# hello-robot/stretch_mujoco

Measured on AMD Instinct MI355X. Metric: env-steps/sec (whole node), 4096 parallel Stretch envs in total, higher is better.
Workload: dtype f32

## Files before the change

### stretch_mujoco_amd/csrc/smj_kernels.hip

```cpp
#define SMJ_BUILD_TAG step
#include "smj_step_tu.h"

__global__ __launch_bounds__(256) void smj_reset_kernel(const DevModel M, const DevState S, const uint8_t* mask) {
  const int e = blockIdx.x * blockDim.x + threadIdx.x;
  if (e >= S.B) return;
  if (mask && !mask[e]) return;
  for (int k = 0; k < M.nq_all; k++) S.qpos[k * S.ld + e] = M.qpos0[k];
  for (int k = 0; k < M.nv_all; k++) { S.qvel[k * S.ld + e] = 0.f; S.warm[k * S.ld + e] = 0.f; }
  for (int k = 0; k < M.nu; k++) S.ctrl[k * S.ld + e] = 0.f;
  if (S.bctl)
    for (int k = 0; k < SMJ_BC_ROWS; k++) S.bctl[k * S.ld + e] = 0.f;
  S.nstep[e] = 0;
  for (int k = 0; k < 4; k++) S.info[k * S.ld + e] = 0;
  if (S.pgsprev) S.pgsprev[(size_t)e * SMJ_PGSPREV_STRIDE] = 0.f;
  if (S.mcache)
    for (int k = 0; k < SMJ_MC_SLOTS; k++) S.mcache[((size_t)e * SMJ_MC_SLOTS + k) * SMJ_MC_WORDS] = 0.f;
  if (S.sepcache)
    for (int k = 0; k < SMJ_SEP_SLOTS; k++) S.sepcache[((size_t)e * SMJ_SEP_SLOTS + k) * 4 + 3] = 0.f;
}

__global__ __launch_bounds__(256) void smj_stage_kernel(const StagePlan P, float* stage, int stride, int B, long ld, int is_export) {
  __shared__ float tile[128][65];
  const int t = threadIdx.x, w = t >> 6, l = t & 63, env0 = blockIdx.x * 64, sg = blockIdx.y;
  float* arr = static_cast<float*>(P.seg[sg].ptr) + (long)P.row0[sg] * ld;
  const int nr = P.seg[sg].rows, off = P.seg[sg].off;
  if (!is_export) {
    for (int k = w; k < nr; k += 4) tile[k][l] = env0 + l < B ? arr[(long)k * ld + env0 + l] : 0.f;
    __syncthreads();
    for (int idx = t; idx < 64 * nr; idx += 256) {
      const int e = idx / nr, k = idx - e * nr;
      if (env0 + e < B) stage[(size_t)(env0 + e) * stride + off + k] = tile[k][e];
    }
  } else {
    for (int idx = t; idx < 64 * nr; idx += 256) {
      const int e = idx / nr, k = idx - e * nr;
      if (env0 + e < B) tile[k][e] = stage[(size_t)(env0 + e) * stride + off + k];
    }
    __syncthreads();
    for (int k = w; k < nr; k += 4)
      if (env0 + l < B) arr[(long)k * ld + env0 + l] = tile[k][l];
  }
}

__global__ __launch_bounds__(256) void smj_base_tick_kernel(const DevState S) {
  const int e = blockIdx.x * blockDim.x + threadIdx.x;
  if (e >= S.B || !S.bctl) return;
  const long ld = S.ld;
  const int mode = (int)S.bctl[SMJ_BC_MODE * ld + e];
  if (mode == 0) return;
  const float x = S.base[e], y = S.base[ld + e], th = S.base[2 * ld + e];
  const float inc = S.bctl[SMJ_BC_INC * ld + e], sign = inc > 0.f ? 1.f : -1.f;
  float v = 0.f, w = 0.f;
  int next = mode;
  if (mode == 1) {
    const float dx = x - S.bctl[SMJ_BC_X0 * ld + e], dy = y - S.bctl[SMJ_BC_Y0 * ld + e];
    if (!(sqrtf(dx * dx + dy * dy) <= fabsf(inc))) next = 0; else v = SMJ_BASE_X_VEL * sign;
  } else if (mode == 2) {
    if (!(fabsf(S.bctl[SMJ_BC_TH0 * ld + e] - th) <= fabsf(inc))) next = 0; else w = SMJ_BASE_R_VEL * sign;
  } else { v = S.bctl[SMJ_BC_V * ld + e]; w = S.bctl[SMJ_BC_W * ld + e]; }
  S.ctrl[e] = (v - (w * SMJ_WHEEL_SEPARATION / 2.f)) / SMJ_WHEEL_RADIUS;
  S.ctrl[ld + e] = (v + (w * SMJ_WHEEL_SEPARATION / 2.f)) / SMJ_WHEEL_RADIUS;
  S.bctl[SMJ_BC_MODE * ld + e] = (float)next;
}

__global__ __launch_bounds__(1024) void smj_order_kernel(const int* cost, int* order, int B) {
  __shared__ int hist[256], mx;
  const int t = threadIdx.x;
  if (t < 256) hist[t] = 0;
  if (t == 0) mx = 1;
  __syncthreads();
  int m = 1;
  for (int e = t; e < B; e += 1024) m = cost[e] > m ? cost[e] : m;
  atomicMax(&mx, m);
  __syncthreads();
  const float sc = 255.f / (float)mx;
  for (int e = t; e < B; e += 1024) atomicAdd(&hist[255 - (int)((float)(cost[e] > 0 ? cost[e] : 0) * sc)], 1);
  __syncthreads();
  if (t == 0) {
    int acc = 0;
    for (int k = 0; k < 256; k++) { const int n = hist[k]; hist[k] = acc; acc += n; }
  }
  __syncthreads();
  for (int e = t; e < B; e += 1024) order[atomicAdd(&hist[255 - (int)((float)(cost[e] > 0 ? cost[e] : 0) * sc)], 1)] = e;
}
void smj_launch_order(const int* cost, int* order, int B, hipStream_t stream) {
  hipLaunchKernelGGL(smj_order_kernel, dim3(1), dim3(1024), 0, stream, cost, order, B);
}
void smj_launch_stage(const StagePlan& plan, float* stage, int stride, int B, long ld, bool is_export, hipStream_t stream) {
  if (plan.nseg == 0) return;
  hipLaunchKernelGGL(smj_stage_kernel, dim3((B + 63) / 64, plan.nseg), dim3(256), 0, stream, plan, stage, stride, B, ld, is_export ? 1 : 0);
}
void smj_launch_base_tick(const DevState& s, hipStream_t stream) {
  hipLaunchKernelGGL(smj_base_tick_kernel, dim3((s.B + 255) / 256), dim3(256), 0, stream, s);
}
void smj_launch_reset(const DevModel& m, const DevState& s, const uint8_t* mask, hipStream_t stream) {
  hipLaunchKernelGGL(smj_reset_kernel, dim3((s.B + 255) / 256), dim3(256), 0, stream, m, s, mask);
}
```

### stretch_mujoco_amd/csrc/smj_kernels_mid.hip

```cpp
#define SMJ_BUILD_TAG mid
#include "smj_step_tu.h"
```

### stretch_mujoco_amd/csrc/smj_step_impl.h

```cpp
#pragma once
#ifndef SMJ_PROFILING
#define SMJ_PROFILING 1
#endif
#include <cstddef>
#include "smj_model.h"
#include "smj_wave.h"
#include "smj_sat_mem.h"

#define JS (NVS + 1)
#define MS (NVS + 1)
#define SMJ_MINVAL 1e-15f
#define SMJ_MINIMP 0.0001f
#define SMJ_MAXIMP 0.9999f

enum { JT_FREE = 0, JT_BALL = 1, JT_SLIDE = 2, JT_HINGE = 3 };
enum { GT_PLANE = 0, GT_SPHERE = 2, GT_CAPSULE = 3, GT_ELLIPSOID = 4, GT_CYLINDER = 5, GT_BOX = 6, GT_MESH = 7 };
enum { CT_EQUALITY = 0, CT_FRICTION = 1, CT_LIMIT = 3, CT_CONTACT_FRICTIONLESS = 5, CT_CONTACT_ELLIPTIC = 7, CT_NONE = -1 };

#if NSAT > 0
#define NCGS (NCG + 1)
#define NSURV 128
#else
#define NCGS NCG
#endif
// ... 149 lines not shown
#endif

template <int N>
SMJ_DEV int qcqp(float* res, const float* Ain, const float* bin, const float* dd, float r, float& la_io, bool exact, float* iters = nullptr) {
  float A[N * N], b[N], L[N * N], Li[N], la = exact ? 0.f : la_io;
#pragma unroll
  for (int i = 0; i < N; i++) {
    b[i] = bin[i] * dd[i];
#pragma unroll
    for (int j = 0; j <= i; j++) A[i * N + j] = Ain[i * N + j] * dd[i] * dd[j];
  }
  float dmin = A[0];
#pragma unroll
  for (int i = 1; i < N; i++) dmin = fminf(dmin, A[i * N + i]);
  const float r2 = r * r, vtol = exact ? 1e-10f : 1e-10f + 1e-5f * r2, dtol = exact ? 1e-10f : 1e-10f + 1e-5f * dmin, drel = exact ? 0.f : 1e-5f;
  for (int it = 0; it < 20; it++) {
    if (iters) *iters += 1.f;
    bool bad = false;
#pragma unroll
    for (int j = 0; j < N; j++) {
      float sd = A[j * N + j] + la;
#pragma unroll
      for (int k = 0; k < j; k++) sd -= L[j * N + k] * L[j * N + k];
      if (sd < 1e-10f) { bad = true; sd = 1e-10f; }
      const float li = fast_rsqrt(sd);
      Li[j] = li;
#pragma unroll
      for (int i = j + 1; i < N; i++) {
        float t = A[i * N + j];
#pragma unroll
        for (int k = 0; k < j; k++) t -= L[i * N + k] * L[j * N + k];
        L[i * N + j] = t * li;
      }
    }
    if (bad) {
#pragma unroll
      for (int i = 0; i < N; i++) res[i] = 0;
      return 0;
    }
    float x[N], nn = 0;
#pragma unroll
    for (int i = 0; i < N; i++) {
      float sv = -b[i];
#pragma unroll
      for (int k = 0; k < i; k++) sv -= L[i * N + k] * x[k];
      x[i] = sv * Li[i];
    }
#pragma unroll
    for (int i = N - 1; i >= 0; i--) {
      float sv = x[i];
#pragma unroll
      for (int k = i + 1; k < N; k++) sv -= L[k * N + i] * x[k];
      x[i] = sv * Li[i];
    }
#pragma unroll
    for (int i = 0; i < N; i++) { res[i] = x[i]; nn += x[i] * x[i]; }
    const float val = nn - r2;
    if (val < vtol && (exact || la == 0.f || val > -vtol)) break;
    float q = 0;
#pragma unroll
    for (int i = 0; i < N; i++) {
      float sv = res[i];
#pragma unroll
      for (int k = 0; k < i; k++) sv -= L[i * N + k] * x[k];
      x[i] = sv * Li[i];
      q += x[i] * x[i];
    }
    float delta;
    if (exact) {
      delta = val * fast_rcp(2.f * q);
      if (delta < dtol) break;
    } else {
      const float nrm = nn * fast_rsqrt(nn);
      delta = (nrm - r) * nn * fast_rcp(r * q);
      if (fabsf(delta) < dtol + drel * la) break;
      if (fabsf(delta) < 3e-3f * (la + dmin)) {
        const float lan = fmaxf(0.f, la + delta), d = lan - la;
#pragma unroll
        for (int i = N - 1; i >= 0; i--) {
          float sv = x[i];
#pragma unroll
          for (int k = i + 1; k < N; k++) sv -= L[k * N + i] * x[k];
          x[i] = sv * Li[i];
        }
#pragma unroll
        for (int i = 0; i < N; i++) res[i] -= d * x[i];
        la = lan;
        break;
      }
    }
    la = fmaxf(0.f, la + delta);
  }
#pragma unroll
  for (int i = 0; i < N; i++) res[i] *= dd[i];
  la_io = la;
  return la != 0;
}

SMJ_DEV float impedance(const float* solimp, float pos, float margin) {
  float dmin = fminf(SMJ_MAXIMP, fmaxf(SMJ_MINIMP, solimp[0])), dmax = fminf(SMJ_MAXIMP, fmaxf(SMJ_MINIMP, solimp[1]));
  float width = fmaxf(SMJ_MINVAL, solimp[2]), mid = fminf(SMJ_MAXIMP, fmaxf(SMJ_MINIMP, solimp[3])), power = fmaxf(1.0f, solimp[4]);
  if (dmin == dmax) return 0.5f * (dmin + dmax);
  float x = fabsf(pos - margin) / width, y;
  if (x >= 1) return dmax;
  if (x <= 0) return dmin;
  if (power == 1.0f) y = x;
  else if (power == 2.0f) y = (x <= mid) ? x * x / mid : 1 - (1 - x) * (1 - x) / (1 - mid);
  else if (x <= mid) y = powf(x, power) / powf(mid, power - 1);
  else y = 1 - powf(1 - x, power) / powf(1 - mid, power - 1);
  return dmin + y * (dmax - dmin);
}

#ifdef SMJ_EMUL
static long smj_emul_sep_skips = 0;
static long smj_emul_ext_steps = 0;
static long smj_emul_mc_hits = 0;
static long smj_emul_isl_total = 0, smj_emul_isl_swept = 0;
#endif
struct StepKernel {
  const DevModel& M;
  const DevState& S;
  Smem& s;
  int env;

  PL<float[6]> cdof, cdof_dot;
  PL<float> qvel_r, g_r, qacc_r;
  PL<float> f_r[NPS], r_r[NPS], ARinv_r[NPS];
  PL<float> qla_r;
  int nefc, ncon, niter, flags;
  float* ppc = nullptr;
  int step_base = 0;
  int pipe_chunk = 0;
  bool parked = false;
  bool split_on = false, rev = false;
  bool serial_redo = false;

  SMJ_DEV StepKernel(const DevModel& M_, const DevState& S_, Smem& s_, int env_) : M(M_), S(S_), s(s_), env(env_) {}

  SMJ_DEV static uint64_t mk64(int lo, int hi) { return (uint64_t)(uint32_t)lo | ((uint64_t)(uint32_t)hi << 32); }

  struct KinTab {
    PL<int> parent, level;
    PL<int[6]> jump;
    PL<float[3]> pos;
    PL<float[4]> quat;
    PL<int[2]> jtype, jqadr, jdadr;
    PL<float[2]> jq0;
    PL<float[6]> jaxis, jpos;
  };
  SMJ_DEV const int* lanerec(int ol, int off) const {
    return static_cast<const int*>(__builtin_assume_aligned(M.k_lanerec + ol * SMJ_LR_STRIDE + off, 16));
  }
  SMJ_DEV static float asf(int b) { return __builtin_bit_cast(float, b); }
  SMJ_DEV void load(KinTab& t) {
    LANES {
      const int* r = lanerec(opaque(lane), SMJ_LR_KIN);
      int v[35];
      for (int k = 0; k < 35; k++) v[k] = r[k];
      t.parent[lane] = v[0]; t.level[lane] = v[1];
      for (int q = 0; q < 6; q++) t.jump[lane][q] = v[2 + q];
      for (int k = 0; k < 3; k++) t.pos[lane][k] = asf(v[8 + k]);
      for (int k = 0; k < 4; k++) t.quat[lane][k] = asf(v[11 + k]);
      for (int u = 0; u < 2; u++) {
        t.jtype[lane][u] = v[15 + u]; t.jqadr[lane][u] = v[17 + u]; t.jdadr[lane][u] = v[19 + u]; t.jq0[lane][u] = asf(v[21 + u]);
      }
      for (int k = 0; k < 6; k++) { t.jaxis[lane][k] = asf(v[23 + k]); t.jpos[lane][k] = asf(v[29 + k]); }
    }
  }
  struct BodyTab {
    PL<int> root, subsize, parent, dofadr, dofnum;
    PL<int[6]> jump;
    PL<uint64_t> dofmask;
    PL<float[10]> inl;
  };
  SMJ_DEV void load(BodyTab& t) {
    LANES {
      const int* r = lanerec(opaque(lane), SMJ_LR_BODY);
      int v[23];
      for (int k = 0; k < 23; k++) v[k] = r[k];
      t.root[lane] = v[0]; t.subsize[lane] = v[1]; t.parent[lane] = v[2]; t.dofadr[lane] = v[3]; t.dofnum[lane] = v[4];
      for (int q = 0; q < 6; q++) t.jump[lane][q] = v[5 + q];
      t.dofmask[lane] = mk64(v[11], v[12]);
      for (int k = 0; k < 10; k++) t.inl[lane][k] = asf(v[13 + k]);
    }
  }
  struct DofTab {
    PL<int> body, jtype, qadr, first, bsub;
    PL<uint64_t> velmask;
    PL<float> damp, stiff, spring;
    PL<int[2]> act;
    PL<float[2]> actmom;
  };
  SMJ_DEV void load(DofTab& t) {
    LANES {
      const int* r = lanerec(opaque(lane), SMJ_LR_DOF);
      int v[14];
      for (int k = 0; k < 14; k++) v[k] = r[k];
      t.body[lane] = v[0]; t.jtype[lane] = v[1]; t.qadr[lane] = v[2]; t.first[lane] = v[3]; t.bsub[lane] = v[4];
      t.velmask[lane] = mk64(v[5], v[6]);
      t.damp[lane] = asf(v[7]); t.stiff[lane] = asf(v[8]); t.spring[lane] = asf(v[9]);
      for (int u = 0; u < 2; u++) { t.act[lane][u] = v[10 + u]; t.actmom[lane][u] = asf(v[12 + u]); }
    }
  }
  struct EntryTab {
    PL<int[NENT]> i, j, lact;
    PL<float[NENT]> arm, damp, dcoef, lcoef;
  };
  SMJ_DEV void load(EntryTab& t, bool implicit) {
    LANES {
      const int* r = lanerec(opaque(lane), SMJ_LR_ENT);
      for (int u = 0; u < NENT; u++) { t.i[lane][u] = r[u]; t.j[lane][u] = r[NENT + u]; t.arm[lane][u] = asf(r[2 * NENT + u]); }
      if (implicit)
        for (int u = 0; u < NENT; u++) {
          t.lact[lane][u] = r[3 * NENT + u]; t.damp[lane][u] = asf(r[4 * NENT + u]); t.dcoef[lane][u] = asf(r[5 * NENT + u]);
          t.lcoef[lane][u] = asf(r[6 * NENT + u]);
        }
    }
  }
  struct ActTab {
    PL<int[4]> dof, qadr;
    PL<float[4]> mom;
    PL<float[8]> prm;
    PL<int> flags;
    PL<int> gc_body, gc_mlo, gc_mhi;
    PL<float> gc_mass, gc_x, gc_y, gc_z;
  };
  SMJ_DEV void load(ActTab& t) {
    LANES {
      const int* r = lanerec(opaque(lane), SMJ_LR_ACT);
      int v[28];
      for (int k = 0; k < 28; k++) v[k] = r[k];
      for (int u = 0; u < 4; u++) { t.dof[lane][u] = v[u]; t.qadr[lane][u] = v[4 + u]; t.mom[lane][u] = asf(v[8 + u]); }
      for (int k = 0; k < 8; k++) t.prm[lane][k] = asf(v[12 + k]);
      t.flags[lane] = v[20]; t.gc_body[lane] = v[21]; t.gc_mlo[lane] = v[22]; t.gc_mhi[lane] = v[23];
      t.gc_mass[lane] = asf(v[24]); t.gc_x[lane] = asf(v[25]); t.gc_y[lane] = asf(v[26]); t.gc_z[lane] = asf(v[27]);
    }
  }

  SMJ_DEV void setup() {
    LANES {
      for (int k = lane; k < NVS * MS; k += 64) (&s.MM[0][0])[k] = 0.f;
      if (lane == 0) {
        s.xpos[0][0] = s.xpos[0][1] = s.xpos[0][2] = 0;
        s.xquat[0][0] = 1; s.xquat[0][1] = s.xquat[0][2] = s.xquat[0][3] = 0;
        for (int k = 0; k < 9; k++) s.xmat[0][k] = (k % 4 == 0) ? 1.f : 0.f;
      }
    }
    SYNC();
#if NSAT > 0
    LANES {
      for (int k = lane; k < (NDR + 1) * JS; k += 64) (&s.J[0][0])[k] = 0.f;
      if (lane == 0) { s.sat.cand_ok = 0; s.sat.ncand = 0; }
      for (int k = lane; k < NCG * 3; k += 64) (&s.sat.refcen[0][0])[k] = 0.f;
    }
#endif
    LANES { if (lane >= M.nv && lane < NVS) s.MM[lane][lane] = 1.f; }
    SYNC();
  }

  SMJ_DEV float* stage_row() const { return S.stage + (size_t)env * S.lay.stride; }
  SMJ_DEV void escalate(int st) {
#ifndef SMJ_EMUL
    float* row = stage_row();
    int* rowi = reinterpret_cast<int*>(row);
    LANES {
      for (int k = lane; k < M.nq; k += 64) st_coh(&row[S.lay.qpos + k], s.qpos[k]);
      if (lane < M.nv) { st_coh(&row[S.lay.qvel + lane], s.qvel[lane]); st_coh(&row[S.lay.warm + lane], s.warm[lane]); }
      if (lane < M.nu) st_coh(&row[S.lay.ctrl + lane], s.ctrl[lane]);
      if (lane < SMJ_BC_ROWS) st_coh(&row[S.lay.bctl + lane], s.bctl[lane]);
      if (lane == 0) {
        st_coh(&rowi[S.lay.nstep], ld_coh(&rowi[S.lay.nstep]) + st);
        st_coh(&S.done_steps[env], ld_coh(&S.done_steps[env]) + st);
      }
    }
#if NSAT > 0
    sat_store_state();
#endif
    coh_release();
    LANES {
      if (lane == 0) {
        st_coh(&S.progress[env], -(pipe_chunk + 1));
        asm volatile("s_waitcnt vmcnt(0)" ::: "memory");
        const int at = atomicAdd(&S.sched[SMJ_SCHED_COUNT], 1);
        st_coh(&S.redo[at], env);
      }
    }
#endif
    parked = true;
  }
  SMJ_DEV void load_state() {
    const long ld = S.ld;
    if (staged()) {
      const float* st = stage_row();
      LANES {
        for (int k = lane; k < M.nq; k += 64) s.qpos[k] = ld_coh(&st[S.lay.qpos + k]);
        if (lane < M.nv) { s.qvel[lane] = ld_coh(&st[S.lay.qvel + lane]); s.warm[lane] = ld_coh(&st[S.lay.warm + lane]); }
        if (lane < M.nu) s.ctrl[lane] = ld_coh(&st[S.lay.ctrl + lane]);
        if (lane < SMJ_BC_ROWS) s.bctl[lane] = ld_coh(&st[S.lay.bctl + lane]);
      }
    } else {
      LANES {
        for (int k = lane; k < M.nq; k += 64) s.qpos[k] = S.qpos[k * ld + env];
        if (lane < M.nv) { s.qvel[lane] = S.qvel[lane * ld + env]; s.warm[lane] = S.warm[lane * ld + env]; }
        if (lane < M.nu) s.ctrl[lane] = S.ctrl[lane * ld + env];
        if (lane < SMJ_BC_ROWS) s.bctl[lane] = S.bctl ? S.bctl[lane * ld + env] : 0.f;
      }
    }
    SYNC();
#if NSAT > 0
    sat_load_state();
#endif
  }
  SMJ_DEV void store_state(int nsteps) {
    const long ld = S.ld;
#if NSAT > 0
    sat_store_state();
#endif
    const int b = 1;
    const float bx = s.xpos[b][0], by = s.xpos[b][1], bth = atan2f(s.xmat[b][3], s.xmat[b][0]);
    if (staged()) {
      float* st = stage_row();
      int* sti = reinterpret_cast<int*>(st);
      LANES {
        for (int k = lane; k < M.nq; k += 64) st_coh(&st[S.lay.qpos + k], s.qpos[k]);
        if (lane < M.nv) { st_coh(&st[S.lay.qvel + lane], s.qvel[lane]); st_coh(&st[S.lay.warm + lane], s.warm[lane]); }
        if (lane < M.nu) { st_coh(&st[S.lay.ctrl + lane], s.ctrl[lane]); st_coh(&st[S.lay.actlen + lane], s.act_len[lane]); st_coh(&st[S.lay.actvel + lane], s.act_vel[lane]); }
        if (lane < SMJ_BC_ROWS) st_coh(&st[S.lay.bctl + lane], s.bctl[lane]);
        if (lane == 0) {
          st_coh(&sti[S.lay.nstep], ld_coh(&sti[S.lay.nstep]) + nsteps);
          if (S.done_steps) st_coh(&S.done_steps[env], ld_coh(&S.done_steps[env]) + nsteps);
          st_coh(&sti[S.lay.info + SMJ_INFO_NEFC], nefc); st_coh(&sti[S.lay.info + SMJ_INFO_NCON], ncon);
          st_coh(&sti[S.lay.info + SMJ_INFO_NITER], niter); st_coh(&sti[S.lay.info + SMJ_INFO_FLAGS], ld_coh(&sti[S.lay.info + SMJ_INFO_FLAGS]) | flags);
          st_coh(&st[S.lay.base], bx); st_coh(&st[S.lay.base + 1], by); st_coh(&st[S.lay.base + 2], bth);
        }
      }
    } else {
      LANES {
        for (int k = lane; k < M.nq; k += 64) S.qpos[k * ld + env] = s.qpos[k];
        if (lane < M.nv) { S.qvel[lane * ld + env] = s.qvel[lane]; S.warm[lane * ld + env] = s.warm[lane]; }
        if (lane < M.nu) { S.ctrl[lane * ld + env] = s.ctrl[lane]; S.act_len[lane * ld + env] = s.act_len[lane]; S.act_vel[lane * ld + env] = s.act_vel[lane]; }
        if (lane < SMJ_BC_ROWS && S.bctl) S.bctl[lane * ld + env] = s.bctl[lane];
        if (lane == 0) {
          S.nstep[env] += nsteps;
          S.info[SMJ_INFO_NEFC * ld + env] = nefc; S.info[SMJ_INFO_NCON * ld + env] = ncon;
          S.info[SMJ_INFO_NITER * ld + env] = niter; S.info[SMJ_INFO_FLAGS * ld + env] |= flags;
          S.base[0 * ld + env] = bx; S.base[1 * ld + env] = by; S.base[2 * ld + env] = bth;
        }
      }
    }
  }

  SMJ_DEV void base_controller() {
    const int mode = (int)uni(s.bctl[SMJ_BC_MODE]);
    if (mode == 0) return;
    const int b = 1;
    const float x = uni(s.xpos[b][0]), y = uni(s.xpos[b][1]), th = atan2f(uni(s.xmat[b][3]), uni(s.xmat[b][0]));
    const float inc = uni(s.bctl[SMJ_BC_INC]), sign = inc > 0.f ? 1.f : -1.f;
    float v = 0.f, w = 0.f;
    int next = mode;
    if (mode == 1) {
      const float dx = x - uni(s.bctl[SMJ_BC_X0]), dy = y - uni(s.bctl[SMJ_BC_Y0]);
      if (!(sqrtf(dx * dx + dy * dy) <= fabsf(inc))) next = 0; else v = SMJ_BASE_X_VEL * sign;
    } else if (mode == 2) {
      if (!(fabsf(uni(s.bctl[SMJ_BC_TH0]) - th) <= fabsf(inc))) next = 0; else w = SMJ_BASE_R_VEL * sign;
    } else { v = uni(s.bctl[SMJ_BC_V]); w = uni(s.bctl[SMJ_BC_W]); }
    const float wl = (v - (w * SMJ_WHEEL_SEPARATION / 2.f)) / SMJ_WHEEL_RADIUS, wr = (v + (w * SMJ_WHEEL_SEPARATION / 2.f)) / SMJ_WHEEL_RADIUS;
    LANES {
      if (lane == 0) { s.ctrl[0] = wl; s.ctrl[1] = wr; s.bctl[SMJ_BC_MODE] = (float)next; }
    }
    SYNC();
  }

  SMJ_DEV void kinematics() {
    const int nb = M.nbody;
    KinTab kt;
    load(kt);
    PL<float[3]> pl;
    PL<float[4]> ql;
    PL<float[6]> al, xl;
    LANES {
      float pos[3] = {0, 0, 0}, quat[4] = {1, 0, 0, 0};
      for (int k = 0; k < 6; k++) { al[lane][k] = 0.f; xl[lane][k] = 0.f; }
      if (lane > 0 && lane < nb) {
        if (kt.jtype[lane][0] == JT_FREE) {
          const int qa = kt.jqadr[lane][0];
          for (int k = 0; k < 3; k++) pos[k] = s.qpos[qa + k];
          for (int k = 0; k < 4; k++) quat[k] = s.qpos[qa + 3 + k];
        } else {
          for (int k = 0; k < 3; k++) pos[k] = kt.pos[lane][k];
          for (int k = 0; k < 4; k++) quat[k] = kt.quat[lane][k];
#pragma unroll
          for (int t = 0; t < 2; t++) {
            const int jt = kt.jtype[lane][t];
            if (jt < 0) continue;
            const float* ax = &kt.jaxis[lane][3 * t];
            const float* jp = &kt.jpos[lane][3 * t];
            float Rm[9], xa[3], a[3], anchor[3];
            quat2mat(Rm, quat);
            mulmat3vec(xa, Rm, ax);
            mulmat3vec(a, Rm, jp);
            for (int k = 0; k < 3; k++) { anchor[k] = pos[k] + a[k]; xl[lane][3 * t + k] = xa[k]; al[lane][3 * t + k] = anchor[k]; }
            const float q = s.qpos[kt.jqadr[lane][t]] - kt.jq0[lane][t];
            if (jt == JT_SLIDE) {
              for (int k = 0; k < 3; k++) pos[k] += xa[k] * q;
            } else {
              float sn, cs;
              sincosf(0.5f * q, &sn, &cs);
              const float dq[4] = {cs, ax[0] * sn, ax[1] * sn, ax[2] * sn};
              quat_mul(quat, quat, dq);
              quat2mat(Rm, quat);
              mulmat3vec(a, Rm, jp);
              for (int k = 0; k < 3; k++) pos[k] = anchor[k] - a[k];
            }
          }
        }
        quat_normalize(quat);
      }
      const bool mine = lane < NBP && (!SMJ_W2_FORWARD || lane < nb);
      for (int k = 0; k < 3; k++) { pl[lane][k] = pos[k]; if (mine) s.xpos[lane][k] = pos[k]; }
      for (int k = 0; k < 4; k++) { ql[lane][k] = quat[k]; if (mine) s.xquat[lane][k] = quat[k]; }
    }
    SYNC();
#pragma unroll
    for (int r = 0; r < 6; r++) {
      if (r >= M.njump) break;
      PL<float[3]> pa;
      PL<float[4]> qa;
      PL<int> anc;
      LANES {
        const int a = kt.jump[lane][r];
        anc[lane] = a;
        for (int k = 0; k < 3; k++) pa[lane][k] = s.xpos[a][k];
        for (int k = 0; k < 4; k++) qa[lane][k] = s.xquat[a][k];
      }
      SYNC();
      LANES {
        if (anc[lane] > 0) {
          float Rm[9], v[3], q[4];
          quat2mat(Rm, qa[lane]);
          mulmat3vec(v, Rm, pl[lane]);
          quat_mul(q, qa[lane], ql[lane]);
          for (int k = 0; k < 3; k++) { pl[lane][k] = pa[lane][k] + v[k]; s.xpos[lane][k] = pl[lane][k]; }
          for (int k = 0; k < 4; k++) { ql[lane][k] = q[k]; s.xquat[lane][k] = q[k]; }
        }
      }
      SYNC();
    }
    LANES {
      if (lane < nb) {
        float q[4] = {ql[lane][0], ql[lane][1], ql[lane][2], ql[lane][3]}, Rm[9];
        quat_normalize(q);
        quat2mat(Rm, q);
        for (int k = 0; k < 4; k++) s.xquat[lane][k] = q[k];
        for (int k = 0; k < 9; k++) s.xmat[lane][k] = Rm[k];
      }
    }
    SYNC();
    LANES {
      if (lane > 0 && lane < nb) {
        if (kt.jtype[lane][0] == JT_FREE) {
          const int da = kt.jdadr[lane][0];
          for (int d = 0; d < 6; d++)
            for (int k = 0; k < 3; k++) s.xanchor[da + d][k] = s.xpos[lane][k];
          for (int d = 0; d < 3; d++)
            for (int k = 0; k < 3; k++) {
              s.xaxis[da + d][k] = (d == k) ? 1.f : 0.f;
              s.xaxis[da + 3 + d][k] = s.xmat[lane][3 * k + d];
            }
        } else {
          const int p = kt.parent[lane];
#pragma unroll
          for (int t = 0; t < 2; t++) {
            if (kt.jtype[lane][t] < 0) continue;
            const int da = kt.jdadr[lane][t];
            float xa[3], an[3];
            mulmat3vec(xa, s.xmat[p], &xl[lane][3 * t]);
            mulmat3vec(an, s.xmat[p], &al[lane][3 * t]);
            for (int k = 0; k < 3; k++) { s.xaxis[da][k] = xa[k]; s.xanchor[da][k] = s.xpos[p][k] + an[k]; }
          }
        }
      }
    }
    SYNC();
  }

  SMJ_DEV void com_crb() {
    const int nb = M.nbody, nv = M.nv;
    BodyTab bt;
    DofTab dt;
    EntryTab et;
    load(bt); load(dt); load(et, false);
    PL<float> mx, my, mz;
    PL<float[3]> xip;
    LANES {
      const int b = lane;
      float t[3] = {0, 0, 0};
      if (b > 0 && b < nb) {
        mulmat3vec(t, s.xmat[b], &bt.inl[lane][6]);
        for (int k = 0; k < 3; k++) t[k] += s.xpos[b][k];
      }
      for (int k = 0; k < 3; k++) xip[lane][k] = t[k];
    }
    for (int r = 0; r < nroot(); r++) {
      const int root = uni(M.k_root_list[r]);
      LANES {
        const bool in = lane > 0 && lane < nb && bt.root[lane] == root;
        const float m = in ? bt.inl[lane][9] : 0.f;
        mx[lane] = m * xip[lane][0]; my[lane] = m * xip[lane][1]; mz[lane] = m * xip[lane][2];
      }
      const float inv = 1.0f / M.body_subtreemass[root];
      const float cx = wave_sum(mx) * inv, cy = wave_sum(my) * inv, cz = wave_sum(mz) * inv;
      LANES {
        if (lane < nb && bt.root[lane] == root) { s.com[lane][0] = cx; s.com[lane][1] = cy; s.com[lane][2] = cz; }
      }
    }
    SYNC();
    LANES {
      const int b = lane;
      if (b > 0 && b < nb) {
        const float* R = s.xmat[b];
        const float* I = bt.inl[lane];
        float Il[9] = {I[0], I[3], I[4], I[3], I[1], I[5], I[4], I[5], I[2]}, RI[9], T[9], Rt[9];
        mulmat3(RI, R, Il);
        for (int i = 0; i < 3; i++)
          for (int j = 0; j < 3; j++) Rt[3 * i + j] = R[3 * j + i];
        mulmat3(T, RI, Rt);
        float dif[3] = {xip[lane][0] - s.com[b][0], xip[lane][1] - s.com[b][1], xip[lane][2] - s.com[b][2]};
        const float mass = I[9], dd = dot3(dif, dif);
        float* c = s.u.t.cinert[b];
        c[0] = T[0] + mass * (dd - dif[0] * dif[0]); c[1] = T[4] + mass * (dd - dif[1] * dif[1]);
        c[2] = T[8] + mass * (dd - dif[2] * dif[2]); c[3] = T[1] - mass * dif[0] * dif[1];
        c[4] = T[2] - mass * dif[0] * dif[2]; c[5] = T[5] - mass * dif[1] * dif[2];
        c[6] = mass * dif[0]; c[7] = mass * dif[1]; c[8] = mass * dif[2]; c[9] = mass;
      }
      if (lane < nv) {
        const int d = lane, b = dt.body[lane];
        float off[3] = {s.com[b][0] - s.xanchor[d][0], s.com[b][1] - s.xanchor[d][1], s.com[b][2] - s.xanchor[d][2]};
        float* c = cdof[lane];
        const int jt = dt.jtype[lane], k = d - dt.first[lane];
        if (jt == JT_SLIDE || (jt == JT_FREE && k < 3)) {
          c[0] = c[1] = c[2] = 0;
          for (int x = 0; x < 3; x++) c[3 + x] = s.xaxis[d][x];
        } else {
          for (int x = 0; x < 3; x++) c[x] = s.xaxis[d][x];
          cross3(c + 3, s.xaxis[d], off);
        }
        for (int x = 0; x < 6; x++) s.u.t.cdof[d][x] = c[x];
        qvel_r[lane] = s.qvel[d];
      } else {
        for (int x = 0; x < 6; x++) cdof[lane][x] = 0;
        qvel_r[lane] = 0;
      }
    }
    SYNC();
    LANES {
      if (lane < nv)
        for (int x = 0; x < 6; x++) s.u.t.buf[lane][x] = cdof[lane][x] * qvel_r[lane];
    }
    SYNC();
    PL<float[6]> cvb;
    LANES {
      float sv[6] = {0, 0, 0, 0, 0, 0};
      if (lane > 0 && lane < nb) {
        const int da = bt.dofadr[lane], dn = bt.dofnum[lane];
#pragma unroll
        for (int u = 0; u < 6; u++) {
          const float on = u < dn ? 1.f : 0.f;
          const int a = da + (u < dn ? u : 0);
          for (int x = 0; x < 6; x++) sv[x] += on * s.u.t.buf[dn > 0 ? a : 0][x];
        }
      }
      for (int x = 0; x < 6; x++) { cvb[lane][x] = sv[x]; if (lane < NBP) s.u.t.cvel[lane][x] = sv[x]; }
    }
    SYNC();
#pragma unroll
    for (int r = 0; r < 6; r++) {
      if (r >= M.njump) break;
      PL<float[6]> up;
      PL<int> anc;
      LANES {
        const int a = bt.jump[lane][r];
        anc[lane] = a;
        for (int x = 0; x < 6; x++) up[lane][x] = s.u.t.cvel[a][x];
      }
      SYNC();
      LANES {
        if (anc[lane] > 0)
          for (int x = 0; x < 6; x++) { cvb[lane][x] += up[lane][x]; s.u.t.cvel[lane][x] = cvb[lane][x]; }
      }
      SYNC();
    }
    LANES {
      if (lane < nv) {
        const int b = dt.body[lane], pb = M.body_parentid[b], da = M.body_dofadr[b];
        float cv[6];
        for (int x = 0; x < 6; x++) cv[x] = s.u.t.cvel[pb][x];
        const uint64_t mk = dt.velmask[lane];
#pragma unroll
        for (int u = 0; u < 5; u++) {
          const int a = da + u;
          const float on = (a < lane && ((mk >> a) & 1)) ? 1.f : 0.f;
          for (int x = 0; x < 6; x++) cv[x] += on * s.u.t.buf[a < lane ? a : lane][x];
        }
        const int jt = dt.jtype[lane], k = lane - dt.first[lane];
        if (jt == JT_FREE && k < 3) { for (int x = 0; x < 6; x++) cdof_dot[lane][x] = 0; }
        else cross_motion(cdof_dot[lane], cv, cdof[lane]);
        for (int x = 0; x < 6; x++) s.u.t.cdof_dot[lane][x] = cdof_dot[lane][x];
      } else {
        for (int x = 0; x < 6; x++) cdof_dot[lane][x] = 0;
      }
    }
    {
      PL<float[10]> cr;
      LANES { for (int k = 0; k < 10; k++) cr[lane][k] = 0.f; }
      for (int x0 = 0; x0 < M.maxsubtree; x0 += 4) {
        LANES {
          if (lane > 0 && lane < nb) {
            const int sub = bt.subsize[lane];
#pragma unroll
            for (int u = 0; u < 4; u++) {
              const bool in = x0 + u < sub;
              const int x = lane + (in ? x0 + u : 0);
              const float on = in ? 1.f : 0.f;
              for (int k = 0; k < 10; k++) cr[lane][k] += on * s.u.t.cinert[x][k];
            }
          }
        }
      }
      LANES {
        if (lane < nb)
          for (int k = 0; k < 10; k++) s.u.t.crb[lane][k] = cr[lane][k];
      }
    }
    SYNC();
    LANES {
      if (lane < nv) {
        float bf[6];
        mul_inert_vec(bf, s.u.t.crb[dt.body[lane]], cdof[lane]);
        for (int x = 0; x < 6; x++) s.u.t.buf[lane][x] = bf[x];
      }
    }
    SYNC();
    LANES {
      for (int t = 0; t < NENT; t++) {
        const int i = et.i[lane][t], j = et.j[lane][t];
        if (i < 0) continue;
        float v = 0;
        for (int x = 0; x < 6; x++) v += s.u.t.cdof[j][x] * s.u.t.buf[i][x];
        if (i == j) { v += et.arm[lane][t]; s.Mdiag[i] = v; }
        s.MM[i][j] = v;
        if (i != j) s.MM[j][i] = v;
      }
    }
    SYNC();
  }

  SMJ_DEV void factor() {
    const int nv = M.nv;
    EntryTab et;
    load(et, false);
    for (int k = nv - 1; k >= 0; k--) {
      const float dkk = s.MM[k][k], dinv = 1.0f / dkk;
      LANES {
        for (int t = 0; t < NENT; t++) {
          const int i = et.i[lane][t], j = et.j[lane][t];
          if (i < 0 || i >= k) continue;
          const float a = s.MM[k][i];
          if (a != 0.f) s.MM[i][j] -= a * s.MM[k][j] * dinv;
        }
      }
      SYNC();
      LANES {
        if (lane < k) s.MM[k][lane] *= dinv;
        if (lane == k) s.Dinv[k] = dinv;
      }
      SYNC();
    }
  }
  SMJ_DEV void solve_LT(PL<float>& x) {
    for (int i = M.nv - 1; i > 0; i--) {
      const float xi = wave_read(x, i);
      LANES { if (lane < i) x[lane] -= s.MM[i][lane] * xi; }
    }
  }
  SMJ_DEV void solve_L(PL<float>& x) {
    for (int j = 0; j < M.nv - 1; j++) {
      const float xj = wave_read(x, j);
      LANES { if (lane > j && lane < M.nv) x[lane] -= s.MM[lane][j] * xj; }
    }
  }

  SMJ_DEV void smooth_forces(bool dbg) {
    const int nb = M.nbody, nv = M.nv, nu = M.nu;
    PL<float> frc_passive, frc_bias, frc_act;
    DofTab dt;
    ActTab at;
    load(dt); load(at);
    LANES {
      float f = 0;
      if (lane < nv) {
        f = -dt.damp[lane] * s.qvel[lane];
        if (dt.stiff[lane] != 0.f) f -= dt.stiff[lane] * (s.qpos[dt.qadr[lane]] - dt.spring[lane]);
      }
      frc_passive[lane] = f;
    }
    BodyTab bt;
    load(bt);
    LANES {
      if (lane < 16) {
        float off[3] = {0, 0, 0}, F[3] = {0, 0, 0};
        int mlo = 0, mhi = 0;
        if (lane < M.ngc) {
          const int b = at.gc_body[lane];
          const float gm = at.gc_mass[lane];
          const float lp[3] = {at.gc_x[lane], at.gc_y[lane], at.gc_z[lane]};
          float pt[3];
          mulmat3vec(pt, s.xmat[b], lp);
          for (int k = 0; k < 3; k++) { off[k] = pt[k] + s.xpos[b][k] - s.com[b][k]; F[k] = -M.gravity[k] * gm; }
          mlo = at.gc_mlo[lane]; mhi = at.gc_mhi[lane];
        }
        float* o = s.u.t.buf[lane];
        for (int k = 0; k < 3; k++) { o[k] = off[k]; o[3 + k] = F[k]; }
        s.u.t.cfrc[lane][0] = __builtin_bit_cast(float, mlo); s.u.t.cfrc[lane][1] = __builtin_bit_cast(float, mhi);
      }
    }
    SYNC();
    LANES {
      if (lane < nv) {
        float acc = 0;
#pragma unroll
        for (int t = 0; t < 16; t++) {
          const uint64_t mk = mk64(__builtin_bit_cast(int, s.u.t.cfrc[t][0]), __builtin_bit_cast(int, s.u.t.cfrc[t][1]));
          const float* o = s.u.t.buf[t];
          float tv[3];
          cross3(tv, cdof[lane], o);
          const float v = (cdof[lane][3] + tv[0]) * o[3] + (cdof[lane][4] + tv[1]) * o[4] + (cdof[lane][5] + tv[2]) * o[5];
          acc += ((mk >> lane) & 1) ? v : 0.f;
        }
        frc_passive[lane] += acc;
      }
    }
    SYNC();
    LANES {
      if (lane < nv)
        for (int x = 0; x < 6; x++) s.u.t.buf[lane][x] = s.u.t.cdof_dot[lane][x] * s.qvel[lane];
    }
    SYNC();
    PL<float[6]> ca;
    LANES {
      float sv[6] = {0, 0, 0, 0, 0, 0};
      if (lane > 0 && lane < nb) {
        const int da = bt.dofadr[lane], dn = bt.dofnum[lane];
#pragma unroll
        for (int u = 0; u < 6; u++) {
          const float on = u < dn ? 1.f : 0.f;
          const int a = dn > 0 ? da + (u < dn ? u : 0) : 0;
          for (int x = 0; x < 6; x++) sv[x] += on * s.u.t.buf[a][x];
        }
      }
      for (int x = 0; x < 6; x++) { ca[lane][x] = sv[x]; if (lane < NBP) s.u.t.cfrc[lane][x] = sv[x]; }
    }
    SYNC();
#pragma unroll
    for (int r = 0; r < 6; r++) {
      if (r >= M.njump) break;
      PL<float[6]> up;
      PL<int> anc;
      LANES {
        const int a = bt.jump[lane][r];
        anc[lane] = a;
        for (int x = 0; x < 6; x++) up[lane][x] = s.u.t.cfrc[a][x];
      }
      SYNC();
      LANES {
        if (anc[lane] > 0)
          for (int x = 0; x < 6; x++) { ca[lane][x] += up[lane][x]; s.u.t.cfrc[lane][x] = ca[lane][x]; }
      }
      SYNC();
    }
    LANES {
      if (lane < nb) {
        const int b = lane;
        float t1[6] = {0, 0, 0, 0, 0, 0}, cf[6] = {0, 0, 0, 0, 0, 0};
        if (b > 0) {
          const float a[6] = {ca[lane][0], ca[lane][1], ca[lane][2], ca[lane][3] - M.gravity[0], ca[lane][4] - M.gravity[1], ca[lane][5] - M.gravity[2]};
          float t2[6];
          mul_inert_vec(t1, s.u.t.cinert[b], a);
          mul_inert_vec(t2, s.u.t.cinert[b], s.u.t.cvel[b]);
          cross_force(cf, s.u.t.cvel[b], t2);
        }
        for (int x = 0; x < 6; x++) s.u.t.cfrc[b][x] = t1[x] + cf[x];
      }
    }
    SYNC();
    {
      PL<float[6]> cfs;
      LANES { for (int k = 0; k < 6; k++) cfs[lane][k] = 0.f; }
      for (int x0 = 0; x0 < M.maxsubtree; x0 += 4) {
        LANES {
          if (lane < nv) {
            const int b = dt.body[lane], sub = dt.bsub[lane];
#pragma unroll
            for (int u = 0; u < 4; u++) {
              const bool in = x0 + u < sub;
              const int x = b + (in ? x0 + u : 0);
              const float on = in ? 1.f : 0.f;
              for (int k = 0; k < 6; k++) cfs[lane][k] += on * s.u.t.cfrc[x][k];
            }
          }
        }
      }
      LANES {
        float v = 0;
        if (lane < nv)
          for (int k = 0; k < 6; k++) v += cdof[lane][k] * cfs[lane][k];
        frc_bias[lane] = v;
      }
    }
    LANES {
      if (lane < nu) {
        const int a = lane;
        float len = 0, vel = 0;
#pragma unroll
        for (int t = 0; t < 4; t++) {
          const int dd = at.dof[lane][t];
          if (dd >= 0) { vel += at.mom[lane][t] * s.qvel[dd]; len += at.mom[lane][t] * s.qpos[at.qadr[lane][t]]; }
        }
        const float* pr = at.prm[lane];
        const int fl = at.flags[lane];
        float ctrl = s.ctrl[a];
        if (fl & 1) ctrl = fminf(pr[5], fmaxf(pr[4], ctrl));
        float f = pr[0] * ctrl;
        if (fl & 4) f += pr[1] + pr[2] * len + pr[3] * vel;
        bool clamped = false;
        if (fl & 2) { clamped = (f <= pr[6] || f >= pr[7]); f = fminf(pr[7], fmaxf(pr[6], f)); }
        s.act_force[a] = f; s.act_len[a] = len; s.act_vel[a] = vel;
        s.act_free[a] = clamped ? 0.f : 1.f;
      }
    }
    SYNC();
    LANES {
      float v = 0;
      if (lane < nv) {
#pragma unroll
        for (int t = 0; t < 2; t++) {
          const int a = dt.act[lane][t];
          if (a >= 0) v += dt.actmom[lane][t] * s.act_force[a];
        }
      }
      frc_act[lane] = v;
      g_r[lane] = frc_passive[lane] - frc_bias[lane] + frc_act[lane];
      if (lane < nv) s.g[lane] = g_r[lane];
      if (dbg && debug_bound() && lane < nv) {
        S.debug[(SMJ_DBG_QFRC_BIAS + lane) * S.ld + env] = frc_bias[lane];
        S.debug[(SMJ_DBG_QFRC_PASSIVE + lane) * S.ld + env] = frc_passive[lane];
        S.debug[(SMJ_DBG_QFRC_ACT + lane) * S.ld + env] = frc_act[lane];
        S.debug[(SMJ_DBG_G + lane) * S.ld + env] = g_r[lane];
      }
    }
    SYNC();
  }

  SMJ_DEV void geom_pose(int g, float* pos, float* mat) const {
    const int b = M.geom_bodyid[g];
    float lp[3] = {M.geom_pos[3 * g], M.geom_pos[3 * g + 1], M.geom_pos[3 * g + 2]};
    mulmat3vec(pos, s.xmat[b], lp);
    for (int k = 0; k < 3; k++) pos[k] += s.xpos[b][k];
    float lm[9];
    for (int k = 0; k < 9; k++) lm[k] = M.k_geom_mat[9 * g + k];
    mulmat3(mat, s.xmat[b], lm);
  }
  SMJ_DEV void pose_from(int b, const float* lp, const float* lm, float* pos, float* mat) const {
    mulmat3vec(pos, s.xmat[b], lp);
    for (int k = 0; k < 3; k++) pos[k] += s.xpos[b][k];
    mulmat3(mat, s.xmat[b], lm);
  }
  SMJ_DEV static void make_frame(float* fr) {
    normalize3(fr);
    if (fr[1] > -0.5f && fr[1] < 0.5f) { fr[3] = 0; fr[4] = 1; fr[5] = 0; } else { fr[3] = 0; fr[4] = 0; fr[5] = 1; }
    const float t = dot3(fr, fr + 3);
    for (int k = 0; k < 3; k++) fr[3 + k] -= t * fr[k];
    normalize3(fr + 3);
    cross3(fr + 6, fr, fr + 3);
  }
  SMJ_DEV int cslot(int c) const { return (SMJ_SPLIT_COLLIDE && rev) ? NCON - 1 - c : c; }
  SMJ_DEV float (*mcs())[3] {
#if SMJ_SPLIT_COLLIDE
    return rev ? s.u.c.mc2 : s.u.c.mc;
#else
    return s.u.c.mc;
#endif
  }
  SMJ_DEV bool con_claim(int n) {
#if SMJ_SPLIT_COLLIDE
    if (split_on) {
      if (ncon + n > NCON) return false;
      int old = 0;
      LANES { if (lane == 0) old = lds_atomic_add(&s.u.c.contotal, n); }
      return uni(old) + n <= NCON;
    }
#endif
    return ncon + n <= NCON;
  }
  SMJ_DEV void write_contact(int c_, const int* r, float dist, const float* pos, const float* n) {
    const int c = cslot(c_);
    s.cdist[c] = dist;
    float fr[9] = {n[0], n[1], n[2], 0, 0, 0, 0, 0, 0};
    make_frame(fr);
    for (int k = 0; k < 9; k++) s.cframe[c][k] = fr[k];
    for (int k = 0; k < 3; k++) s.cpos[c][k] = pos[k];
    for (int k = 0; k < 5; k++) { s.cfric[c][k] = asf(r[SMJ_CP_FRIC + k]); s.csolimp[c][k] = asf(r[SMJ_CP_SOLIMP + k]); }
    s.csolref[c][0] = asf(r[SMJ_CP_SOLREF]); s.csolref[c][1] = asf(r[SMJ_CP_SOLREF + 1]);
    s.cmargin[c] = asf(r[SMJ_CP_MG]);
    s.cdim[c] = r[SMJ_CP_CONDIM]; s.cgeom1[c] = r[SMJ_CP_G1]; s.cgeom2[c] = r[SMJ_CP_G2]; s.cefc[c] = -1;
#if NSAT > 0
    s.cpair[c] = r[SMJ_CP_PAIR];
#endif
  }
  SMJ_DEV void add_contact(const int* r, float dist, const float* pos, const float* n) {
    if (!con_claim(1)) { flags |= SMJ_FLAG_CON_OVERFLOW | 0x4000; return; }
    const int c = ncon++;
    LANES { if (lane == 0) write_contact(c, r, dist, pos, n); }
  }

  SMJ_DEV void collision() {
    ncon = 0;
    for (int base = 0; base < M.nplanepair; base += 64) {
      PL<int> hull, cv;
      LANES {
        int cnt = 0, hl = 0;
        const int t = base + lane;
        if (t < M.nplanepair) {
          const int* r = static_cast<const int*>(__builtin_assume_aligned(M.k_pprec + opaque(t) * SMJ_PP_STRIDE, 16));
          int v[SMJ_PP_CONDIM];
          for (int k = 0; k < SMJ_PP_CONDIM; k++) v[k] = r[k];
          const int b1 = v[SMJ_PP_B1], b2 = v[SMJ_PP_B2];
          float lp1[3], lm1[9], pp[3], pm[9];
          for (int k = 0; k < 3; k++) lp1[k] = asf(v[SMJ_PP_POS1 + k]);
          for (int k = 0; k < 9; k++) lm1[k] = asf(v[SMJ_PP_MAT1 + k]);
          pose_from(b1, lp1, lm1, pp, pm);
          float c2[3], lc[3] = {asf(v[SMJ_PP_BCEN2]), asf(v[SMJ_PP_BCEN2 + 1]), asf(v[SMJ_PP_BCEN2 + 2])};
          mulmat3vec(c2, s.xmat[b2], lc);
          const float n[3] = {pm[2], pm[5], pm[8]};
          const float dif[3] = {c2[0] + s.xpos[b2][0] - pp[0], c2[1] + s.xpos[b2][1] - pp[1], c2[2] + s.xpos[b2][2] - pp[2]};
          const float margin = asf(v[SMJ_PP_MARGIN]);
          if (dot3(dif, n) - asf(v[SMJ_PP_RBOUND2]) <= margin) {
            const int t2 = v[SMJ_PP_T2];
            if (t2 == GT_MESH) {
              float lp2[3], lm2[9], gp[3], gm[9], bc[3], wc[3];
              for (int k = 0; k < 3; k++) { lp2[k] = asf(v[SMJ_PP_POS2 + k]); bc[k] = asf(r[SMJ_PP_BOX2 + k]); }
              for (int k = 0; k < 9; k++) lm2[k] = asf(v[SMJ_PP_MAT2 + k]);
              pose_from(b2, lp2, lm2, gp, gm);
              mulmat3vec(wc, gm, bc);
              float low = (gp[0] + wc[0] - pp[0]) * n[0] + (gp[1] + wc[1] - pp[1]) * n[1] + (gp[2] + wc[2] - pp[2]) * n[2];
              for (int k = 0; k < 3; k++) low -= fabsf(n[0] * gm[k] + n[1] * gm[3 + k] + n[2] * gm[6 + k]) * (asf(r[SMJ_PP_BOX2 + 3 + k]) + 1e-5f);
              hl = low <= margin + 1e-6f;
            } else {
              float lp2[3], lm2[9], size[3];
              for (int k = 0; k < 3; k++) { lp2[k] = asf(v[SMJ_PP_POS2 + k]); size[k] = asf(v[SMJ_PP_SIZE2 + k]); }
              for (int k = 0; k < 9; k++) lm2[k] = asf(v[SMJ_PP_MAT2 + k]);
              cnt = plane_prim(b2, lp2, lm2, size, t2, pp, n, margin, s.u.p.dist[lane], s.u.p.pos[lane]);
            }
            for (int k = 0; k < 3; k++) s.u.p.nrm[lane][k] = n[k];
            s.u.p.pair[lane] = t;
          }
        }
        s.u.p.cnt[lane] = cnt;
        hull[lane] = hl;
      }
      uint64_t hm = wave_ballot(hull);
      if (hm) {
        SYNC();
        while (hm) {
          const int l = ffs64(hm);
          hm &= hm - 1;
          narrow_plane_hull(uni(M.k_planepair[base + l]), l);
        }
        SYNC();
      }
      PL<int> bit;
      LANES { cv[lane] = s.u.p.cnt[lane]; bit[lane] = cv[lane] & 1; }
      const uint64_t m0 = wave_ballot(bit);
      LANES { bit[lane] = cv[lane] & 2; }
      const uint64_t m1 = wave_ballot(bit);
      LANES { bit[lane] = cv[lane] & 4; }
      const uint64_t m2 = wave_ballot(bit);
      const int total = popc64(m0) + 2 * popc64(m1) + 4 * popc64(m2);
      if (total) {
        LANES {
          const int c = cv[lane];
          if (c) {
            const uint64_t lt = (1ull << lane) - 1;
            const int off = ncon + popc64(m0 & lt) + 2 * popc64(m1 & lt) + 4 * popc64(m2 & lt);
            const int* r = static_cast<const int*>(__builtin_assume_aligned(M.k_pprec + s.u.p.pair[lane] * SMJ_PP_STRIDE, 16));
            const int g1 = r[SMJ_PP_G1], g2 = r[SMJ_PP_G2];
            float fr[9] = {s.u.p.nrm[lane][0], s.u.p.nrm[lane][1], s.u.p.nrm[lane][2], 0, 0, 0, 0, 0, 0};
            make_frame(fr);
            float fric[5], simp[5];
            for (int k = 0; k < 5; k++) { fric[k] = asf(r[SMJ_PP_FRIC + k]); simp[k] = asf(r[SMJ_PP_SOLIMP + k]); }
            const float sr0 = asf(r[SMJ_PP_SOLREF]), sr1 = asf(r[SMJ_PP_SOLREF + 1]), mg = asf(r[SMJ_PP_MG]);
            const int cd = r[SMJ_PP_CONDIM];
#pragma unroll
            for (int k = 0; k < 4; k++) {
              const int ci = off + k;
              if (k < c && ci < NCON) {
                s.cdist[ci] = s.u.p.dist[lane][k];
                for (int x = 0; x < 9; x++) s.cframe[ci][x] = fr[x];
                for (int x = 0; x < 3; x++) s.cpos[ci][x] = s.u.p.pos[lane][k][x];
                for (int x = 0; x < 5; x++) { s.cfric[ci][x] = fric[x]; s.csolimp[ci][x] = simp[x]; }
                s.csolref[ci][0] = sr0; s.csolref[ci][1] = sr1;
                s.cmargin[ci] = mg;
                s.cdim[ci] = cd; s.cgeom1[ci] = g1; s.cgeom2[ci] = g2; s.cefc[ci] = -1;
#if NSAT > 0
                s.cpair[ci] = r[SMJ_PP_PAIR];
#endif
              }
            }
          }
        }
        if (ncon + total > NCON) { flags |= SMJ_FLAG_CON_OVERFLOW; ncon = NCON; }
        else ncon += total;
      }
    }
    SYNC();
  }

  SMJ_DEV int plane_prim(int b2, const float* lp2, const float* lm2, const float* size, int t2, const float* pp, const float* n,
                         float margin, float* cdist, float (*cpos)[3]) const {
    float gp[3], gm[9];
    pose_from(b2, lp2, lm2, gp, gm);
    int cnt = 0;
#define put(d, q) do { cdist[cnt] = (d); cpos[cnt][0] = (q)[0]; cpos[cnt][1] = (q)[1]; cpos[cnt][2] = (q)[2]; cnt++; } while (0)
    if (t2 == GT_SPHERE) {
      const float dif[3] = {gp[0] - pp[0], gp[1] - pp[1], gp[2] - pp[2]};
      const float dist = dot3(dif, n) - size[0];
      if (dist <= margin) {
        float pos[3];
        for (int k = 0; k < 3; k++) pos[k] = gp[k] - n[k] * (size[0] + 0.5f * dist);
        put(dist, pos);
      }
    } else if (t2 == GT_CYLINDER) {
      float axis[3] = {gm[2], gm[5], gm[8]};
      float prjaxis = dot3(n, axis);
      if (prjaxis > 0) { for (int k = 0; k < 3; k++) axis[k] = -axis[k]; prjaxis = -prjaxis; }
      float vec[3] = {gp[0] - pp[0], gp[1] - pp[1], gp[2] - pp[2]};
      const float dist0 = dot3(vec, n);
      for (int k = 0; k < 3; k++) vec[k] = axis[k] * prjaxis - n[k];
      const float len2 = dot3(vec, vec);
      if (len2 >= 1e-9f) { const float sc = size[0] / sqrtf(len2); for (int k = 0; k < 3; k++) vec[k] *= sc; }
      else { vec[0] = gm[0] * size[0]; vec[1] = gm[3] * size[0]; vec[2] = gm[6] * size[0]; }
      const float prjvec = dot3(vec, n);
      for (int k = 0; k < 3; k++) axis[k] *= size[1];
      prjaxis *= size[1];
      if (dist0 + prjaxis + prjvec <= margin) {
        float pos[3], dist = dist0 + prjaxis + prjvec;
        for (int k = 0; k < 3; k++) pos[k] = gp[k] + vec[k] + axis[k] - n[k] * dist * 0.5f;
        put(dist, pos);
        if (dist0 - prjaxis + prjvec <= margin) {
          dist = dist0 - prjaxis + prjvec;
          for (int k = 0; k < 3; k++) pos[k] = gp[k] + vec[k] - axis[k] - n[k] * dist * 0.5f;
          put(dist, pos);
        }
        const float prjvec1 = -prjvec * 0.5f;
        if (dist0 + prjaxis + prjvec1 <= margin) {
          float vec1[3];
          cross3(vec1, vec, axis);
          normalize3(vec1);
          for (int k = 0; k < 3; k++) vec1[k] *= size[0] * 0.8660254037844386f;
          dist = dist0 + prjaxis + prjvec1;
          for (int sg = 0; sg < 2 && cnt < 4; sg++) {
            const float sgn = sg ? -1.f : 1.f;
            for (int k = 0; k < 3; k++) pos[k] = gp[k] + sgn * vec1[k] + axis[k] - vec[k] * 0.5f - n[k] * dist * 0.5f;
            put(dist, pos);
          }
        }
      }
    } else if (t2 == GT_CAPSULE) {
#pragma unroll
      for (int e = 0; e < 2; e++) {
        const float sg = e ? -1.f : 1.f;
        const float c[3] = {gp[0] + sg * size[1] * gm[2], gp[1] + sg * size[1] * gm[5], gp[2] + sg * size[1] * gm[8]};
        const float dif[3] = {c[0] - pp[0], c[1] - pp[1], c[2] - pp[2]};
        const float dist = dot3(dif, n) - size[0];
        if (dist <= margin) {
          float pos[3];
          for (int k = 0; k < 3; k++) pos[k] = c[k] - n[k] * (size[0] + 0.5f * dist);
          put(dist, pos);
        }
// ... 380 lines not shown
#pragma unroll
      for (int i = 0; i < 3; i++) {
        const float v1 = P[1].v[i], v2 = P[2].v[i], a1 = P[1].a[i], a2 = P[2].a[i], b1 = P[1].b[i], b2 = P[2].b[i];
        P[1].v[i] = sw ? v2 : v1; P[2].v[i] = sw ? v1 : v2;
        P[1].a[i] = sw ? a2 : a1; P[2].a[i] = sw ? a1 : a2;
        P[1].b[i] = sw ? b2 : b1; P[2].b[i] = sw ? b1 : b2;
        dir[i] = sw ? -dir[i] : dir[i];
      }
    }
    for (int it = 0;; it++) {
      if (it > 100) return false;
      mpr_support(A, Bs, dir, P[3]);
      dot = dot3(P[3].v, dir);
      if (ccd_zero(dot) || dot < 0) { SMJ_SEP_OUT() return false; }
      bool cont = false;
      cross3(va, P[1].v, P[3].v);
      dot = dot3(va, P[0].v);
      if (dot < 0 && !ccd_zero(dot)) { const MprPt q = P[3]; portal_set<2>(P, q, true); cont = true; }
      if (!cont) {
        cross3(va, P[3].v, P[2].v);
        dot = dot3(va, P[0].v);
        if (dot < 0 && !ccd_zero(dot)) { const MprPt q = P[3]; portal_set<1>(P, q, true); cont = true; }
      }
      if (!cont) break;
      for (int i = 0; i < 3; i++) { va[i] = P[1].v[i] - P[0].v[i]; vb[i] = P[2].v[i] - P[0].v[i]; }
      cross3(dir, va, vb);
      normalize3(dir);
    }
    for (int it = 0;; it++) {
      portal_dir(P, dir);
      dot = dot3(dir, P[1].v);
      if (ccd_zero(dot) || dot > 0) break;
      mpr_support(A, Bs, dir, v4);
      dot = dot3(v4.v, dir);
      if (!(ccd_zero(dot) || dot > 0)) { SMJ_SEP_OUT() return false; }
      if (reach_tolerance(P, v4, dir, tol) || it > maxit) return false;
      expand_portal(P, v4);
    }
    for (int it = 0;; it++) {
      portal_dir(P, dir);
      mpr_support(A, Bs, dir, v4);
      if (reach_tolerance(P, v4, dir, tol) || it > maxit) {
        bool inside;
        depth = sqrtf(fmaxf(0.f, origin_tri_dist2(P[1].v, P[2].v, P[3].v, pdir, &inside)));
        if (ccd_zero(pdir[0]) && ccd_zero(pdir[1]) && ccd_zero(pdir[2])) { pdir[0] = dir[0]; pdir[1] = dir[1]; pdir[2] = dir[2]; }
        normalize3(pdir);
        if (SMJ_PORTAL_NORMAL && inside && dot3(pdir, dir) > 0.9995f) {
          float ea[3], eb[3], ec[3], cr[3];
          for (int i = 0; i < 3; i++) { ea[i] = P[2].v[i] - P[1].v[i]; eb[i] = P[3].v[i] - P[1].v[i]; ec[i] = P[3].v[i] - P[2].v[i]; }
          cross3(cr, ea, eb);
          const float emax2 = fmaxf(dot3(ea, ea), fmaxf(dot3(eb, eb), dot3(ec, ec)));
          if (dot3(cr, cr) > 16.f * depth * depth * emax2) { pdir[0] = dir[0]; pdir[1] = dir[1]; pdir[2] = dir[2]; }
        }
        float b[4], vec[3], sum;
        cross3(vec, P[1].v, P[2].v); b[0] = dot3(vec, P[3].v);
        cross3(vec, P[3].v, P[2].v); b[1] = dot3(vec, P[0].v);
        cross3(vec, P[0].v, P[1].v); b[2] = dot3(vec, P[3].v);
        cross3(vec, P[2].v, P[1].v); b[3] = dot3(vec, P[0].v);
        sum = b[0] + b[1] + b[2] + b[3];
        if (ccd_zero(sum) || sum < 0) {
          b[0] = 0;
          cross3(vec, P[2].v, P[3].v); b[1] = dot3(vec, dir);
          cross3(vec, P[3].v, P[1].v); b[2] = dot3(vec, dir);
          cross3(vec, P[1].v, P[2].v); b[3] = dot3(vec, dir);
          sum = b[1] + b[2] + b[3];
        }
        if (!(fabsf(sum) > 1e-30f)) { b[0] = 0; b[1] = b[2] = b[3] = 1; sum = 3; }
#pragma unroll
        for (int i = 0; i < 3; i++) {
          const float p1 = b[0] * P[0].a[i] + b[1] * P[1].a[i] + b[2] * P[2].a[i] + b[3] * P[3].a[i];
          const float p2 = b[0] * P[0].b[i] + b[1] * P[1].b[i] + b[2] * P[2].b[i] + b[3] * P[3].b[i];
          pos[i] = 0.5f * (p1 + p2) / sum;
        }
        return true;
      }
      expand_portal(P, v4);
    }
#undef SMJ_SEP_OUT
  }

  SMJ_DEV bool sphere_box(const float* spos, float r, const Shape& bx, float margin, float& dist_out, float* dir, float* pos) {
    const float tmp[3] = {spos[0] - bx.pos[0], spos[1] - bx.pos[1], spos[2] - bx.pos[2]};
    float cen[3], cl[3], dif[3], nl[3], pl[3];
    mulmat3Tvec(cen, bx.mat, tmp);
    for (int i = 0; i < 3; i++) { cl[i] = fminf(bx.size[i], fmaxf(-bx.size[i], cen[i])); dif[i] = cl[i] - cen[i]; }
    const float dist = sqrtf(dot3(dif, dif));
    if (dist - r > margin) return false;
    if (dist <= SMJ_MINVAL) {
      float closest = 2.f * fmaxf(bx.size[0], fmaxf(bx.size[1], bx.size[2]));
      int k = 0;
      for (int i = 0; i < 6; i++) {
        const float cd = fabsf(((i & 1) ? 1.f : -1.f) * bx.size[i >> 1] - cen[i >> 1]);
        if (cd < closest) { closest = cd; k = i; }
      }
      for (int i = 0; i < 3; i++) nl[i] = (i == (k >> 1)) ? ((k & 1) ? -1.f : 1.f) : 0.f;
      for (int i = 0; i < 3; i++) pl[i] = cen[i] + nl[i] * (r - closest) * 0.5f;
      dist_out = -closest - r;
    } else {
      const float inv = 1.f / dist;
      for (int i = 0; i < 3; i++) { nl[i] = dif[i] * inv; pl[i] = 0.5f * (cl[i] + cen[i] + dif[i] * (r * inv)); }
      dist_out = dist - r;
    }
    mulmat3vec(dir, bx.mat, nl);
    mulmat3vec(pos, bx.mat, pl);
    for (int i = 0; i < 3; i++) pos[i] += bx.pos[i];
    return true;
  }
  SMJ_DEV bool sphere_sphere(const float* p1, float r1, const float* p2, float r2, float margin, float& dist_out, float* dir, float* pos) {
    float dif[3] = {p2[0] - p1[0], p2[1] - p1[1], p2[2] - p1[2]};
    const float cdist = sqrtf(dot3(dif, dif));
    if (cdist - r1 - r2 > margin) return false;
    if (cdist < SMJ_MINVAL) { dif[0] = 1; dif[1] = dif[2] = 0; } else { const float inv = 1.f / cdist; for (int i = 0; i < 3; i++) dif[i] *= inv; }
    dist_out = cdist - r1 - r2;
    for (int i = 0; i < 3; i++) { dir[i] = dif[i]; pos[i] = p1[i] + dif[i] * (r1 + 0.5f * dist_out); }
    return true;
  }
  SMJ_DEV bool sphere_capsule(const float* p1, float r1, const Shape& cp, float margin, float& dist_out, float* dir, float* pos) {
    const float ax[3] = {cp.mat[2], cp.mat[5], cp.mat[8]}, vec[3] = {p1[0] - cp.pos[0], p1[1] - cp.pos[1], p1[2] - cp.pos[2]};
    const float x = fmaxf(-cp.size[1], fminf(cp.size[1], dot3(ax, vec)));
    const float q[3] = {cp.pos[0] + ax[0] * x, cp.pos[1] + ax[1] * x, cp.pos[2] + ax[2] * x};
    return sphere_sphere(p1, r1, q, cp.size[0], margin, dist_out, dir, pos);
  }
  SMJ_DEV void capsule_capsule(const int* r, const Shape& A, const Shape& Bs, float margin) {
    const float a1[3] = {A.mat[2] * A.size[1], A.mat[5] * A.size[1], A.mat[8] * A.size[1]};
    const float a2[3] = {Bs.mat[2] * Bs.size[1], Bs.mat[5] * Bs.size[1], Bs.mat[8] * Bs.size[1]};
    const float dif[3] = {A.pos[0] - Bs.pos[0], A.pos[1] - Bs.pos[1], A.pos[2] - Bs.pos[2]};
    const float ma = dot3(a1, a1), mb = -dot3(a1, a2), mc = dot3(a2, a2), u = -dot3(a1, dif), v = dot3(a2, dif);
    float c[3], c1[3], c2[3];
    cross3(c, a1, a2); cross3(c2, a2, dif); cross3(c1, a1, dif);
    const float det = dot3(c, c);
    float v1[3], v2[3], depth, dir[3], pos[3];
    if (det >= 1e-12f * ma * mc) {
      float x1 = dot3(c, c2) / det, x2 = dot3(c, c1) / det;
      if (x1 > 1) { x1 = 1; x2 = (v - mb) / mc; }
      else if (x1 < -1) { x1 = -1; x2 = (v + mb) / mc; }
      if (x2 > 1) { x2 = 1; x1 = fmaxf(-1.f, fminf(1.f, (u - mb) / ma)); }
      else if (x2 < -1) { x2 = -1; x1 = fmaxf(-1.f, fminf(1.f, (u + mb) / ma)); }
      for (int i = 0; i < 3; i++) { v1[i] = A.pos[i] + a1[i] * x1; v2[i] = Bs.pos[i] + a2[i] * x2; }
      if (sphere_sphere(v1, A.size[0], v2, Bs.size[0], margin, depth, dir, pos)) add_contact(r, depth, pos, dir);
      return;
    }
    int n = 0;
    for (int e = 0; e < 2; e++) {
      const float sg = e ? -1.f : 1.f, x2 = fmaxf(-1.f, fminf(1.f, (v - sg * mb) / mc));
      for (int i = 0; i < 3; i++) { v1[i] = A.pos[i] + sg * a1[i]; v2[i] = Bs.pos[i] + a2[i] * x2; }
      if (sphere_sphere(v1, A.size[0], v2, Bs.size[0], margin, depth, dir, pos)) { add_contact(r, depth, pos, dir); n++; }
    }
    for (int e = 0; e < 2 && n < 2; e++) {
      const float sg = e ? -1.f : 1.f, x1 = fmaxf(-1.f, fminf(1.f, (u - sg * mb) / ma));
      for (int i = 0; i < 3; i++) { v1[i] = A.pos[i] + a1[i] * x1; v2[i] = Bs.pos[i] + sg * a2[i]; }
      if (sphere_sphere(v1, A.size[0], v2, Bs.size[0], margin, depth, dir, pos)) { add_contact(r, depth, pos, dir); n++; }
    }
  }
  SMJ_DEV void load_shape(Shape& sh, int g, int slot, float* cen) {
    (void)g;
    const unsigned meta = (unsigned)uni(s.u.c.meta[slot]);
    sh.type = (int)(meta & 15u); sh.nvert = (int)((meta >> 4) & 4095u);
    sh.verts = M.k_hull_vert4 + 4 * (int)(meta >> 16);
    for (int k = 0; k < 3; k++) { sh.pos[k] = uni(s.u.c.pos[slot][k]); sh.size[k] = uni(s.u.c.size[slot][k]); cen[k] = uni(s.u.c.ccen[slot][k]); }
    for (int k = 0; k < 9; k++) sh.mat[k] = uni(s.u.c.mat[slot][k]);
    if (sh.type == GT_MESH) {
      const Vec4* verts = reinterpret_cast<const Vec4*>(sh.verts);
      const int nvert = sh.nvert;
      LANES {
#pragma unroll
        for (int u = 0; u < 4; u++) {
          const int id = lane + 64 * u < nvert ? lane + 64 * u : (nvert > 0 ? nvert - 1 : 0);
          const Vec4 v = verts[id];
          sh.vc[lane][3 * u] = v.x; sh.vc[lane][3 * u + 1] = v.y; sh.vc[lane][3 * u + 2] = v.z;
        }
      }
    }
  }


  SMJ_DEV void ccol(float* o, int slot, int i) const {
    o[0] = uni(s.u.c.mat[slot][i]); o[1] = uni(s.u.c.mat[slot][3 + i]); o[2] = uni(s.u.c.mat[slot][6 + i]);
  }
  SMJ_DEV void box_box(const int* rec, int slot1, int slot2, float margin) {
    float p1[3], p2[3], A[3], B[3], R1[9], R2[9];
#pragma unroll
    for (int k = 0; k < 3; k++) { p1[k] = uni(s.u.c.pos[slot1][k]); p2[k] = uni(s.u.c.pos[slot2][k]); A[k] = uni(s.u.c.size[slot1][k]); B[k] = uni(s.u.c.size[slot2][k]); }
#pragma unroll
    for (int k = 0; k < 9; k++) { R1[k] = uni(s.u.c.mat[slot1][k]); R2[k] = uni(s.u.c.mat[slot2][k]); }
    const float p[3] = {p2[0] - p1[0], p2[1] - p1[1], p2[2] - p1[2]};
    float R[3][3], Q[3][3], pp[3], pq[3];
#pragma unroll
    for (int i = 0; i < 3; i++) {
      const float ai[3] = {R1[i], R1[3 + i], R1[6 + i]}, bi[3] = {R2[i], R2[3 + i], R2[6 + i]};
      pp[i] = dot3(p, ai); pq[i] = dot3(p, bi);
#pragma unroll
      for (int j = 0; j < 3; j++) { const float bj[3] = {R2[j], R2[3 + j], R2[6 + j]}; R[i][j] = dot3(ai, bj); Q[i][j] = fabsf(R[i][j]); }
    }
    float best = -3.0e38f, en[3] = {0, 0, 0};
    int code = -1;
    bool sep = false;
#pragma unroll
    for (int i = 0; i < 3; i++) {
      const float sv = fabsf(pp[i]) - (A[i] + B[0] * Q[i][0] + B[1] * Q[i][1] + B[2] * Q[i][2]);
      sep = sep || sv > margin;
      if (sv > best) { best = sv; code = i; }
    }
#pragma unroll
    for (int j = 0; j < 3; j++) {
      const float sv = fabsf(pq[j]) - (B[j] + A[0] * Q[0][j] + A[1] * Q[1][j] + A[2] * Q[2][j]);
      sep = sep || sv > margin;
      if (sv > best) { best = sv; code = 3 + j; }
    }
#pragma unroll
    for (int i = 0; i < 3; i++)
#pragma unroll
      for (int j = 0; j < 3; j++) {
        const int i1 = (i + 1) % 3, i2 = (i + 2) % 3, j1 = (j + 1) % 3, j2 = (j + 2) % 3;
        const float l = sqrtf(fmaxf(0.f, 1.f - R[i][j] * R[i][j]));
        if (l >= 2e-3f) {
          const float e = pp[i2] * R[i1][j] - pp[i1] * R[i2][j];
          const float sv = (fabsf(e) - (A[i1] * Q[i2][j] + A[i2] * Q[i1][j] + B[j1] * Q[i][j2] + B[j2] * Q[i][j1])) / l;
          sep = sep || sv > margin;
          if (sv * 1.05f > best && sv > best) {
            best = sv; code = 6 + 3 * i + j;
            const float ai[3] = {R1[i], R1[3 + i], R1[6 + i]}, bj[3] = {R2[j], R2[3 + j], R2[6 + j]};
            cross3(en, ai, bj);
            for (int k = 0; k < 3; k++) en[k] /= l;
          }
        }
      }
#ifdef SMJ_EMUL
    if (getenv("SMJ_BOXBOX_TRACE")) { fprintf(stderr, "box_box: code %d best %.9g sep %d R:", code, best, (int)sep); for (int i = 0; i < 3; i++) for (int j = 0; j < 3; j++) fprintf(stderr, " %.9g", R[i][j]); fprintf(stderr, " pp %.9g %.9g %.9g\n", pp[0], pp[1], pp[2]); }
#endif
    if (sep) return;
    if (code >= 6) {
      float n[3] = {en[0], en[1], en[2]};
      if (dot3(n, p) < 0) for (int k = 0; k < 3; k++) n[k] = -n[k];
      const int i = (code - 6) / 3, j = (code - 6) % 3;
      float pa[3] = {p1[0], p1[1], p1[2]}, pb[3] = {p2[0], p2[1], p2[2]};
#pragma unroll
      for (int k = 0; k < 3; k++) {
        const float ak[3] = {R1[k], R1[3 + k], R1[6 + k]}, bk[3] = {R2[k], R2[3 + k], R2[6 + k]};
        const float sa = dot3(n, ak) > 0 ? 1.f : -1.f, sb = dot3(n, bk) > 0 ? -1.f : 1.f;
        for (int x = 0; x < 3; x++) { pa[x] += sa * A[k] * ak[x]; pb[x] += sb * B[k] * bk[x]; }
      }
      float ua[3], ub[3];
      ccol(ua, slot1, i); ccol(ub, slot2, j);
      const float dd[3] = {pb[0] - pa[0], pb[1] - pa[1], pb[2] - pa[2]};
      const float uaub = dot3(ua, ub), q1 = dot3(ua, dd), q2 = -dot3(ub, dd), den = 1.f - uaub * uaub;
      float al = 0, be = 0;
      if (den > 1e-12f) { al = (q1 + uaub * q2) / den; be = (uaub * q1 + q2) / den; }
      float pos[3];
      for (int x = 0; x < 3; x++) pos[x] = 0.5f * ((pa[x] + al * ua[x]) + (pb[x] + be * ub[x]));
      add_contact(rec, best, pos, n);
      return;
    }
    const bool swap = code >= 3;
    const int ia = swap ? code - 3 : code, sa = swap ? slot2 : slot1, sb = swap ? slot1 : slot2;
    float pa[3], pb[3], n[3], u[3], v[3];
    for (int k = 0; k < 3; k++) { pa[k] = uni(s.u.c.pos[sa][k]); pb[k] = uni(s.u.c.pos[sb][k]); }
    ccol(n, sa, ia);
    const float ab[3] = {pb[0] - pa[0], pb[1] - pa[1], pb[2] - pa[2]};
    if (dot3(n, ab) < 0) for (int k = 0; k < 3; k++) n[k] = -n[k];
    const int ja = (ia + 1) % 3, ka = (ia + 2) % 3;
    ccol(u, sa, ja); ccol(v, sa, ka);
    const float hu = uni(s.u.c.size[sa][ja]), hv = uni(s.u.c.size[sa][ka]), hn = uni(s.u.c.size[sa][ia]);
    float cA[3];
    for (int k = 0; k < 3; k++) cA[k] = pa[k] + n[k] * hn;
    int ib = 0;
    float bd = -1.f;
#pragma unroll
    for (int k = 0; k < 3; k++) { float bk[3]; ccol(bk, sb, k); const float t = fabsf(dot3(bk, n)); if (t > bd) { bd = t; ib = k; } }
    float nb[3], pv[3], qv[3];
    ccol(nb, sb, ib);
    if (dot3(nb, n) > 0) for (int k = 0; k < 3; k++) nb[k] = -nb[k];
    const int jb = (ib + 1) % 3, kb = (ib + 2) % 3;
    ccol(pv, sb, jb); ccol(qv, sb, kb);
    const float hp = uni(s.u.c.size[sb][jb]), hq = uni(s.u.c.size[sb][kb]), hbn = uni(s.u.c.size[sb][ib]);
    float cB[3];
    for (int k = 0; k < 3; k++) cB[k] = pb[k] + nb[k] * hbn;
    const float nnb = dot3(n, nb);
    PL<int> okv;
    PL<float> dv, px, py, pz;
    LANES {
      const int cand = lane;
      int ok = 0;
      float x[3] = {0, 0, 0};
#define SG0(c) (((c) == 1 || (c) == 2) ? 1.f : -1.f)
#define SG1(c) ((c) >= 2 ? 1.f : -1.f)
      if (cand < 4) {
        float d[3];
        for (int k = 0; k < 3; k++) { x[k] = cB[k] + SG0(cand) * hp * pv[k] + SG1(cand) * hq * qv[k]; d[k] = x[k] - cA[k]; }
        ok = fabsf(dot3(d, u)) <= hu * (1.f + 2e-6f) && fabsf(dot3(d, v)) <= hv * (1.f + 2e-6f);
      } else if (cand < 8) {
        const int c = cand - 4;
        float r[3], d[3];
        for (int k = 0; k < 3; k++) { r[k] = cA[k] + SG0(c) * hu * u[k] + SG1(c) * hv * v[k]; d[k] = cB[k] - r[k]; }
        const float t = dot3(d, nb) / nnb;
        for (int k = 0; k < 3; k++) { x[k] = r[k] + t * n[k]; d[k] = x[k] - cB[k]; }
        ok = fabsf(dot3(d, pv)) <= hp * (1.f + 2e-6f) && fabsf(dot3(d, qv)) <= hq * (1.f + 2e-6f);
      } else if (cand < 24) {
        const int e = (cand - 8) >> 2, r = (cand - 8) & 3, c0 = e, c1 = (e + 1) & 3;
        float w0[3], w1[3], d0[3], d1[3];
        for (int k = 0; k < 3; k++) {
          w0[k] = cB[k] + SG0(c0) * hp * pv[k] + SG1(c0) * hq * qv[k]; w1[k] = cB[k] + SG0(c1) * hp * pv[k] + SG1(c1) * hq * qv[k];
          d0[k] = w0[k] - cA[k]; d1[k] = w1[k] - cA[k];
        }
        const float u0 = dot3(d0, u), v0 = dot3(d0, v), u1 = dot3(d1, u), v1 = dot3(d1, v);
        const bool along_u = r < 2;
        const float lim = ((r & 1) ? 1.f : -1.f) * (along_u ? hu : hv);
        const float a0 = along_u ? u0 : v0, a1 = along_u ? u1 : v1, b0 = along_u ? v0 : u0, b1 = along_u ? v1 : u1;
        const float den = a1 - a0;
        if (fabsf(den) > 1e-12f) {
          const float t = (lim - a0) / den, o = b0 + t * (b1 - b0);
          ok = t > 0 && t < 1 && fabsf(o) < (along_u ? hv : hu);
          for (int k = 0; k < 3; k++) x[k] = w0[k] + t * (w1[k] - w0[k]);
        }
      }
#undef SG0
#undef SG1
      const float d[3] = {x[0] - cA[0], x[1] - cA[1], x[2] - cA[2]};
      const float depth = -dot3(d, n);
      if (-depth > margin) ok = 0;
      okv[lane] = ok; dv[lane] = -depth;
      px[lane] = x[0] + 0.5f * depth * n[0]; py[lane] = x[1] + 0.5f * depth * n[1]; pz[lane] = x[2] + 0.5f * depth * n[2];
    }
    uint64_t mask = wave_ballot(okv);
    if (mask == 0) return;
// ... 234 lines not shown
      rotate_point(m.apos, p0l, Rp); rotate_point(m.bpos, p0l, Rn); rotate_point(ca, p0l, Rp); rotate_point(cb, p0l, Rn);
      mulmat3(m.amat, Rp, mA); mulmat3(m.bmat, Rn, mB);
      for (int i = 0; i < 3; i++) { m.P[0].a[i] = ca[i]; m.P[0].b[i] = cb[i]; m.P[0].v[i] = ca[i] - cb[i]; }
      if (ccd_zero(m.P[0].v[0]) && ccd_zero(m.P[0].v[1]) && ccd_zero(m.P[0].v[2])) m.P[0].v[0] += 10.f * CCD_EPS;
      for (int i = 0; i < 3; i++) m.dir[i] = -m.P[0].v[i];
      normalize3(m.dir);
      m.phase = MQ_W1; m.it = 0; m.ok = 0; m.depth = 0;
      for (int i = 0; i < 3; i++) { m.pdir[i] = 0; m.pos[i] = 0; }
    }
    int round = 0;
    for (; round < 256; round++) {
      PL<int> need;
      LANES {
        MprLane& m = st[lane];
        if (m.phase == MQ_W3 && m.it > 100) m.phase = MQ_DONE;
        if (m.phase == MQ_R1 || m.phase == MQ_R2) {
          portal_dir(m.P, m.dir);
          const float dot = dot3(m.dir, m.P[1].v);
          if (m.phase == MQ_R1 && (ccd_zero(dot) || dot > 0)) { m.phase = MQ_R2; m.it = 0; }
        }
        need[lane] = m.phase != MQ_DONE;
      }
      if (wave_ballot(need) == 0) break;
      PL<float[3]> sa, sb;
      shape_support4(A, st, false, sa);
      shape_support4(Bs, st, true, sb);
      LANES {
        MprLane& m = st[lane];
        MprPt np;
        for (int i = 0; i < 3; i++) { np.a[i] = sa[lane][i]; np.b[i] = sb[lane][i]; np.v[i] = np.a[i] - np.b[i]; }
        float va[3], vb[3];
        if (m.phase == MQ_W1) {
          m.P[1] = np;
          float dot = dot3(m.P[1].v, m.dir);
          if (ccd_zero(dot) || dot < 0) m.phase = MQ_DONE;
          else {
            cross3(m.dir, m.P[0].v, m.P[1].v);
            if (ccd_zero(dot3(m.dir, m.dir))) {
              if (ccd_zero(m.P[1].v[0]) && ccd_zero(m.P[1].v[1]) && ccd_zero(m.P[1].v[2])) { m.depth = 0; m.pdir[0] = m.pdir[1] = m.pdir[2] = 0; }
              else {
                m.depth = sqrtf(dot3(m.P[1].v, m.P[1].v));
                for (int i = 0; i < 3; i++) m.pdir[i] = m.P[1].v[i];
                normalize3(m.pdir);
              }
              for (int i = 0; i < 3; i++) m.pos[i] = 0.5f * (m.P[1].a[i] + m.P[1].b[i]);
              m.ok = 1; m.phase = MQ_DONE;
            } else { normalize3(m.dir); m.phase = MQ_W2; }
          }
        } else if (m.phase == MQ_W2) {
          m.P[2] = np;
          const float dot = dot3(m.P[2].v, m.dir);
          if (ccd_zero(dot) || dot < 0) m.phase = MQ_DONE;
          else {
            for (int i = 0; i < 3; i++) { va[i] = m.P[1].v[i] - m.P[0].v[i]; vb[i] = m.P[2].v[i] - m.P[0].v[i]; }
            cross3(m.dir, va, vb);
            normalize3(m.dir);
            const bool sw = dot3(m.dir, m.P[0].v) > 0;
#pragma unroll
            for (int i = 0; i < 3; i++) {
              const float v1 = m.P[1].v[i], v2 = m.P[2].v[i], a1 = m.P[1].a[i], a2 = m.P[2].a[i], b1 = m.P[1].b[i], b2 = m.P[2].b[i];
              m.P[1].v[i] = sw ? v2 : v1; m.P[2].v[i] = sw ? v1 : v2;
              m.P[1].a[i] = sw ? a2 : a1; m.P[2].a[i] = sw ? a1 : a2;
              m.P[1].b[i] = sw ? b2 : b1; m.P[2].b[i] = sw ? b1 : b2;
              m.dir[i] = sw ? -m.dir[i] : m.dir[i];
            }
            m.phase = MQ_W3; m.it = 0;
          }
        } else if (m.phase == MQ_W3) {
          m.P[3] = np;
          float dot = dot3(m.P[3].v, m.dir);
          if (ccd_zero(dot) || dot < 0) m.phase = MQ_DONE;
          else {
            bool cont = false;
            cross3(va, m.P[1].v, m.P[3].v);
            dot = dot3(va, m.P[0].v);
            if (dot < 0 && !ccd_zero(dot)) { const MprPt q = m.P[3]; portal_set<2>(m.P, q, true); cont = true; }
            if (!cont) {
              cross3(va, m.P[3].v, m.P[2].v);
              dot = dot3(va, m.P[0].v);
              if (dot < 0 && !ccd_zero(dot)) { const MprPt q = m.P[3]; portal_set<1>(m.P, q, true); cont = true; }
            }
            if (cont) {
              for (int i = 0; i < 3; i++) { va[i] = m.P[1].v[i] - m.P[0].v[i]; vb[i] = m.P[2].v[i] - m.P[0].v[i]; }
              cross3(m.dir, va, vb);
              normalize3(m.dir);
              m.it++;
            } else { m.phase = MQ_R1; m.it = 0; }
          }
        } else if (m.phase == MQ_R1 || m.phase == MQ_R2) {
          m.v4 = np;
          const float dot = dot3(m.v4.v, m.dir);
          const bool behind = m.phase == MQ_R1 && !(ccd_zero(dot) || dot > 0);
          if (behind || reach_tolerance(m.P, m.v4, m.dir, tolm) || m.it > maxit) { m.ok = m.phase == MQ_R2 ? 2 : 0; m.phase = MQ_DONE; }
          else { expand_portal(m.P, m.v4); m.it++; }
        }
      }
    }
    LANES {
      MprLane& m = st[lane];
      if (m.ok == 2) { mpr_finish(m); m.ok = 1; }
    }
    PL<int> okp;
    PL<float> dpp, drx, dry, drz, psx, psy, psz;
    LANES {
      const MprLane& m = st[lane];
      okp[lane] = m.ok; dpp[lane] = m.depth; drx[lane] = m.pdir[0]; dry[lane] = m.pdir[1]; drz[lane] = m.pdir[2];
      psx[lane] = m.pos[0]; psy[lane] = m.pos[1]; psz[lane] = m.pos[2];
    }
    LANES { if (lane == 0) for (int k = 0; k < 3; k++) mcs()[0][k] = pos0[k]; }
    SYNC();
    int n = 1;
#pragma nounroll
    for (int q = 0; q < 4; q++) {
      const int l = 16 * q;
      if (!wave_read(okp, l)) continue;
      const float dp = wave_read(dpp, l);
      const float dr[3] = {wave_read(drx, l), wave_read(dry, l), wave_read(drz, l)}, ps[3] = {wave_read(psx, l) + org[0], wave_read(psy, l) + org[1], wave_read(psz, l) + org[2]};
      if (-dp > margin || dot3(dr, dr) < 0.5f) continue;
      bool dup = false;
#pragma nounroll
      for (int k = 0; k < n; k++) {
        const float e[3] = {ps[0] - uni(mcs()[k][0]), ps[1] - uni(mcs()[k][1]), ps[2] - uni(mcs()[k][2])};
        dup = dup || dot3(e, e) < tol * tol;
      }
      if (dup) continue;
      LANES { if (lane == 0) for (int k = 0; k < 3; k++) mcs()[n][k] = ps[k]; }
      SYNC();
      n++;
      add_contact(rec, -dp, ps, dir0);
    }
    return round;
  }

  SMJ_DEV static void smj_mc_motion(const float* x0, const float* q0, const float* x1, const float* q1, float* dx, float* dth) {
    for (int k = 0; k < 3; k++) dx[k] = x1[k] - x0[k];
    const float sw = q1[0] * q0[0] + q1[1] * q0[1] + q1[2] * q0[2] + q1[3] * q0[3];
    const float sg = sw < 0.f ? -2.f : 2.f;
    dth[0] = sg * (q0[0] * q1[1] - q1[0] * q0[1] - (q1[2] * q0[3] - q1[3] * q0[2]));
    dth[1] = sg * (q0[0] * q1[2] - q1[0] * q0[2] - (q1[3] * q0[1] - q1[1] * q0[3]));
    dth[2] = sg * (q0[0] * q1[3] - q1[0] * q0[3] - (q1[1] * q0[2] - q1[2] * q0[1]));
  }
  SMJ_DEV static void smj_mc_carry(const float* xa, const float* dxa, const float* dta, const float* xb, const float* dxb, const float* dtb, const float* n,
                                   float& dist, float* p) {
    const float ra[3] = {p[0] - xa[0], p[1] - xa[1], p[2] - xa[2]}, rb[3] = {p[0] - xb[0], p[1] - xb[1], p[2] - xb[2]};
    const float ua[3] = {dxa[0] + dta[1] * ra[2] - dta[2] * ra[1], dxa[1] + dta[2] * ra[0] - dta[0] * ra[2], dxa[2] + dta[0] * ra[1] - dta[1] * ra[0]};
    const float ub[3] = {dxb[0] + dtb[1] * rb[2] - dtb[2] * rb[1], dxb[1] + dtb[2] * rb[0] - dtb[0] * rb[2], dxb[2] + dtb[0] * rb[1] - dtb[1] * rb[0]};
    dist += n[0] * (ub[0] - ua[0]) + n[1] * (ub[1] - ua[1]) + n[2] * (ub[2] - ua[2]);
    for (int k = 0; k < 3; k++) p[k] += 0.5f * (ua[k] + ub[k]);
  }
  SMJ_DEV float* mc_entry(int tag) const {
    const unsigned slot = (((unsigned)tag >> 30) & 1u) << SMJ_MC_LOG2 | (((unsigned)tag * 2654435761u) >> (32 - SMJ_MC_LOG2));
    return S.mcache + ((size_t)env * SMJ_MC_SLOTS + slot) * SMJ_MC_WORDS;
  }
  SMJ_DEV void narrow_pair(const int* r, int s1, int s2, float* sepslot, int septag, bool sep_hit, const float* sd, float* pc, bool prof, bool lookup = true) {
    const int g1 = uni(r[SMJ_CP_G1]), g2 = uni(r[SMJ_CP_G2]);
    const int ta0 = uni(s.u.c.meta[s1]) & 15, tb0 = uni(s.u.c.meta[s2]) & 15;
    float* mc = nullptr;
    const int ncon0 = ncon;
    if (mcache_bound() && manifold_cache() && ta0 != GT_SPHERE && tb0 != GT_SPHERE && !(ta0 == GT_CAPSULE && tb0 == GT_CAPSULE)) {
      mc = mc_entry(septag);
      const int b1 = uni(r[SMJ_CP_B1]), b2 = uni(r[SMJ_CP_B2]);
      PL<float> w;
      PL<int> moved;
      if (lookup) LANES {
        w[lane] = lane < SMJ_MC_WORDS ? mc[lane] : 0.f;
        float cur = w[lane];
        if (lane >= 1 && lane < 15) {
          const int b = lane < 8 ? b1 : b2, k = lane < 8 ? lane - 1 : lane - 8;
          cur = k < 3 ? s.xpos[b][k] : s.xquat[b][k - 3];
        }
        moved[lane] = !(fabsf(cur - w[lane]) <= SMJ_MC_EPS);
      }
      if (lookup && __builtin_bit_cast(int, wave_read(w, 0)) == septag && wave_ballot(moved) == 0) {
        const int n = (int)wave_read(w, 15);
        const float nrm[3] = {wave_read(w, 16), wave_read(w, 17), wave_read(w, 18)};
        float x0a[3], q0a[4], x0b[3], q0b[4], x1a[3], q1a[4], x1b[3], q1b[4], dxa[3], dta[3], dxb[3], dtb[3];
        for (int k = 0; k < 3; k++) { x0a[k] = wave_read(w, 1 + k); x0b[k] = wave_read(w, 8 + k); x1a[k] = uni(s.xpos[b1][k]); x1b[k] = uni(s.xpos[b2][k]); }
        for (int k = 0; k < 4; k++) { q0a[k] = wave_read(w, 4 + k); q0b[k] = wave_read(w, 11 + k); q1a[k] = uni(s.xquat[b1][k]); q1b[k] = uni(s.xquat[b2][k]); }
        smj_mc_motion(x0a, q0a, x1a, q1a, dxa, dta);
        smj_mc_motion(x0b, q0b, x1b, q1b, dxb, dtb);
        for (int k = 0; k < n && k < 5; k++) {
          float p3[3] = {wave_read(w, 20 + 4 * k), wave_read(w, 21 + 4 * k), wave_read(w, 22 + 4 * k)};
          float dist = wave_read(w, 19 + 4 * k);
          smj_mc_carry(x0a, dxa, dta, x0b, dxb, dtb, nrm, dist, p3);
          add_contact(r, dist, p3, nrm);
        }
#ifdef SMJ_EMUL
        smj_emul_mc_hits++;
#endif
        return;
      }
    }
    narrow_pair_run(r, g1, g2, s1, s2, sepslot, septag, sep_hit, sd, pc, prof);
    if (mc && ncon > ncon0 && ncon - ncon0 <= 5 && !(flags & SMJ_FLAG_CON_OVERFLOW)) {
      const int b1 = uni(r[SMJ_CP_B1]), b2 = uni(r[SMJ_CP_B2]), n = ncon - ncon0;
      SYNC();
      LANES {
        if (lane < SMJ_MC_WORDS) {
          float v = 0.f;
          if (lane == 0) v = asf(septag);
          else if (lane < 15) { const int b = lane < 8 ? b1 : b2, k = lane < 8 ? lane - 1 : lane - 8; v = k < 3 ? s.xpos[b][k] : s.xquat[b][k - 3]; }
          else if (lane == 15) v = (float)n;
          else if (lane < 19) v = s.cframe[cslot(ncon0)][lane - 16];
          else if (lane < 19 + 4 * n) { const int k = (lane - 19) >> 2, q = (lane - 19) & 3; v = q == 0 ? s.cdist[cslot(ncon0 + k)] : s.cpos[cslot(ncon0 + k)][q - 1]; }
          mc[lane] = v;
        }
      }
    }
  }
  SMJ_DEV void narrow_pair_run(const int* r, int g1, int g2, int s1, int s2, float* sepslot, int septag, bool sep_hit, const float* sd, float* pc, bool prof) {
    Shape A, Bs;
    float c0[3], c1[3], depth, dir[3], pos[3];
    load_shape(A, g1, s1, c0);
    load_shape(Bs, g2, s2, c1);
    const float margin = asf(uni(r[SMJ_CP_MARGIN]));
    if (A.type == GT_SPHERE && Bs.type == GT_SPHERE) {
      if (sphere_sphere(A.pos, A.size[0], Bs.pos, Bs.size[0], margin, depth, dir, pos)) add_contact(r, depth, pos, dir);
      return;
    }
    if (A.type == GT_SPHERE && Bs.type == GT_BOX) {
      if (sphere_box(A.pos, A.size[0], Bs, margin, depth, dir, pos)) add_contact(r, depth, pos, dir);
      return;
    }
    if (A.type == GT_BOX && Bs.type == GT_SPHERE) {
      if (sphere_box(Bs.pos, Bs.size[0], A, margin, depth, dir, pos)) {
        for (int k = 0; k < 3; k++) dir[k] = -dir[k];
        add_contact(r, depth, pos, dir);
      }
      return;
    }
    if (A.type == GT_SPHERE && Bs.type == GT_CAPSULE) {
      if (sphere_capsule(A.pos, A.size[0], Bs, margin, depth, dir, pos)) add_contact(r, depth, pos, dir);
      return;
    }
    if (A.type == GT_CAPSULE && Bs.type == GT_SPHERE) {
      if (sphere_capsule(Bs.pos, Bs.size[0], A, margin, depth, dir, pos)) {
        for (int k = 0; k < 3; k++) dir[k] = -dir[k];
        add_contact(r, depth, pos, dir);
      }
      return;
    }
    if (A.type == GT_CAPSULE && Bs.type == GT_CAPSULE) { capsule_capsule(r, A, Bs, margin); return; }
    if (A.type == GT_BOX && Bs.type == GT_BOX && M.multiccd) {
      const long long tb = prof ? smj_clock() : 0;
      box_box(r, s1, s2, margin);
      if (prof) pc[SMJ_PROF_C_TBOXBOX] += (float)(smj_clock() - tb);
      return;
    }
    const long long tm = prof ? smj_clock() : 0;
    float org[3];
    {
      const float ha = uni(s.u.c.half[s1][0]) + uni(s.u.c.half[s1][1]) + uni(s.u.c.half[s1][2]), hb = uni(s.u.c.half[s2][0]) + uni(s.u.c.half[s2][1]) + uni(s.u.c.half[s2][2]);
      for (int k = 0; k < 3; k++) org[k] = SMJ_MPR_LOCAL ? (ha <= hb ? c0[k] : c1[k]) : 0.f;
      for (int k = 0; k < 3; k++) { A.pos[k] -= org[k]; Bs.pos[k] -= org[k]; c0[k] -= org[k]; c1[k] -= org[k]; }
    }
    float sep[3];
    bool pen = false, skipped = false;
    if (sep_hit) {
      MprPt q;
      mpr_support(A, Bs, sd, q);
      skipped = dot3(q.v, sd) < -1e-6f;
#ifdef SMJ_EMUL
      if (skipped) smj_emul_sep_skips++;
#endif
    }
    if (!skipped) {
      pen = mpr_penetration(A, Bs, c0, c1, depth, dir, pos, sep);
      if (sepslot && !pen && (sep[0] != 0.f || sep[1] != 0.f || sep[2] != 0.f)) {
        LANES { if (lane == 0) *reinterpret_cast<Vec4*>(sepslot) = Vec4{sep[0], sep[1], sep[2], asf(septag)}; }
      }
    }
    if (prof) pc[SMJ_PROF_C_TMPR1] += (float)(smj_clock() - tm);
    if (!pen) return;
    if (-depth > margin || dot3(dir, dir) < 0.5f) return;
    for (int k = 0; k < 3; k++) pos[k] += org[k];
    add_contact(r, -depth, pos, dir);
    if (prof) pc[SMJ_PROF_C_NHIT] += 1.f;
    if (prof && M.multiccd && A.type != GT_SPHERE && Bs.type != GT_SPHERE) pc[SMJ_PROF_C_NMULTI] += 1.f;
    if (M.multiccd && A.type != GT_SPHERE && Bs.type != GT_SPHERE) {
#ifdef SMJ_EMUL
      if (M.multi_serial) { convex_multi(r, A, Bs, s1, s2, pos, dir, margin, 1e-3f * asf(uni(r[SMJ_CP_RBMIN])), org); return; }
#endif
      const long long t4 = prof ? smj_clock() : 0;
      const int rounds = convex_multi4(r, A, Bs, s1, s2, pos, dir, margin, 1e-3f * asf(uni(r[SMJ_CP_RBMIN])), org);
      if (prof) { pc[SMJ_PROF_C_TMULTI] += (float)(smj_clock() - t4); pc[SMJ_PROF_C_ROUNDS] += (float)rounds; }
    }
  }

  SMJ_DEV void collision_convex(float* pc, bool prof) {
    if (!M.convex_pairs || (M.nconvpair == 0 && (NSAT == 0 || M.nsgeom == 0))) return;
    long long tc = prof ? smj_clock() : 0;
#define CTICK(slot) if (prof) { const long long t1 = smj_clock(); pc[slot] += (float)(t1 - tc); tc = t1; }
    for (int c0 = 0; c0 < M.ncgeom; c0 += 64) {
      LANES {
        const int c = c0 + lane;
        if (c < M.ncgeom) {
          const int* r = static_cast<const int*>(__builtin_assume_aligned(M.k_cgrec + opaque(c) * SMJ_CG_STRIDE, 16));
          int v[SMJ_CG_STRIDE];
          for (int k = 0; k < SMJ_CG_STRIDE; k++) v[k] = r[k];
          float lp[3], lm[9], pos[3], mat[9], cw[3];
          for (int k = 0; k < 3; k++) lp[k] = asf(v[SMJ_CG_POS + k]);
          for (int k = 0; k < 9; k++) lm[k] = asf(v[SMJ_CG_MAT + k]);
          pose_from(v[SMJ_CG_BODY], lp, lm, pos, mat);
          const float lc[3] = {asf(v[SMJ_CG_LCEN]), asf(v[SMJ_CG_LCEN + 1]), asf(v[SMJ_CG_LCEN + 2])};
          mulmat3vec(cw, mat, lc);
          for (int k = 0; k < 3; k++) { s.u.c.pos[c][k] = pos[k]; s.u.c.cen[c][k] = pos[k] + cw[k]; s.u.c.half[c][k] = asf(v[SMJ_CG_HALF + k]); }
          for (int k = 0; k < 9; k++) s.u.c.mat[c][k] = mat[k];
          const float lcc[3] = {asf(v[SMJ_CG_CCEN]), asf(v[SMJ_CG_CCEN + 1]), asf(v[SMJ_CG_CCEN + 2])};
          float wc[3];
          mulmat3vec(wc, mat, lcc);
          for (int k = 0; k < 3; k++) { s.u.c.ccen[c][k] = pos[k] + wc[k]; s.u.c.size[c][k] = asf(v[SMJ_CG_SIZE + k]); }
          s.u.c.meta[c] = v[SMJ_CG_META];
        }
      }
    }
    SYNC();
    CTICK(SMJ_PROF_C_POSE)
#if SMJ_SPLIT_COLLIDE
    if (!serial_redo) {
      LANES {
        if (lane == 0) { s.mbox[0] = W2_COLLIDE; s.mbox[1] = env; s.u.c.contotal = ncon; }
      }
      WG_BARRIER();
      split_on = true;
    }
    collision_static(pc, prof);
    split_on = false;
    CTICK(SMJ_PROF_C_NARROW)
    if (serial_redo) {
      collision_moving(pc, prof);
      SYNC();
      return;
    }
    WG_BARRIER();
    {
      const int nh = uni(s.mbox[2]);
      flags |= uni(s.mbox[3]);
      if (nh > 0 && ncon + nh <= NCON) {
        PL<float[31]> w;
        LANES {
          if (lane < nh) {
            const int c = NCON - 1 - lane;
            float* v = w[lane];
            v[0] = s.cdist[c]; v[1] = s.cmargin[c];
            for (int k = 0; k < 9; k++) v[2 + k] = s.cframe[c][k];
            for (int k = 0; k < 3; k++) v[11 + k] = s.cpos[c][k];
            for (int k = 0; k < 5; k++) { v[14 + k] = s.cfric[c][k]; v[19 + k] = s.csolimp[c][k]; }
            v[24] = s.csolref[c][0]; v[25] = s.csolref[c][1];
            v[26] = __builtin_bit_cast(float, (int)s.cdim[c]); v[27] = __builtin_bit_cast(float, (int)s.cgeom1[c]);
            v[28] = __builtin_bit_cast(float, (int)s.cgeom2[c]); v[29] = __builtin_bit_cast(float, (int)s.cefc[c]);
            v[30] = __builtin_bit_cast(float, (int)s.cpair[c]);
          }
        }
        SYNC();
        LANES {
          if (lane < nh) {
            const int c = ncon + lane;
            const float* v = w[lane];
            s.cdist[c] = v[0]; s.cmargin[c] = v[1];
            for (int k = 0; k < 9; k++) s.cframe[c][k] = v[2 + k];
            for (int k = 0; k < 3; k++) s.cpos[c][k] = v[11 + k];
            for (int k = 0; k < 5; k++) { s.cfric[c][k] = v[14 + k]; s.csolimp[c][k] = v[19 + k]; }
            s.csolref[c][0] = v[24]; s.csolref[c][1] = v[25];
            s.cdim[c] = __builtin_bit_cast(int, v[26]); s.cgeom1[c] = (unsigned short)__builtin_bit_cast(int, v[27]);
            s.cgeom2[c] = (unsigned short)__builtin_bit_cast(int, v[28]); s.cefc[c] = __builtin_bit_cast(int, v[29]);
            s.cpair[c] = __builtin_bit_cast(int, v[30]);
          }
        }
        ncon += nh;
      } else if (nh > 0) flags |= SMJ_FLAG_CON_OVERFLOW | 0x4000;
    }
    SYNC();
    CTICK(SMJ_PROF_C_SPHERE)
#undef CTICK
  }
  enum { W2_COLLIDE = 1, W2_EXIT = 2, W2_SAT_NEWTON = 3, W2_SAT_FORWARD = 4, W2_SAT_INTEGRATE = 5 };
  SMJ_DEV void helper() {
    rev = true;
    split_on = true;
    for (int cmd = uni(s.mbox[0]);;) {
      if (cmd == W2_COLLIDE) {
        ncon = 0;
        flags = 0;
        collision_moving(nullptr, false);
        LANES { if (lane == 0) { s.mbox[2] = ncon; s.mbox[3] = flags; } }
      } else if (cmd == W2_SAT_NEWTON) {
        const uint64_t conemask = mk64(uni(s.mbox[1]), uni(s.mbox[2]));
        sat_hessian(conemask);
        SYNC();
        sat_solve_own();
      } else if (cmd == W2_SAT_FORWARD) {
        env = uni(s.mbox[1]);
        sat_forward();
      } else if (cmd == W2_SAT_INTEGRATE) {
        PL<int> bad;
        LANES { bad[lane] = 0; }
        sat_integrate(bad);
        const int anybad = wave_ballot(bad) != 0;
        LANES { if (lane == 0) s.mbox[2] = anybad; }
      }
      WG_BARRIER();
      WG_BARRIER();
      cmd = uni(s.mbox[0]);
      if (cmd == W2_EXIT) return;
    }
  }
  SMJ_DEV void fork2(int cmd, int w1 = 0, int w2 = 0) {
    LANES { if (lane == 0) { s.mbox[0] = cmd; s.mbox[1] = w1; s.mbox[2] = w2; } }
    WG_BARRIER();
  }
  SMJ_DEV void collision_moving(float* pc, bool prof) {
    long long tc = prof ? smj_clock() : 0;
#define CTICK(slot) if (prof) { const long long t1 = smj_clock(); pc[slot] += (float)(t1 - tc); tc = t1; }
#else
#if NSAT > 0
    collision_static(pc, prof);
    CTICK(SMJ_PROF_C_NARROW)
#endif
#endif
    int nsurv = 0;
    const int ncp = M.nconvpair;
    const int* const pair_ss = M.k_convpair_ss;
    const float* const pair_rr = M.k_convpair_rsum;
    for (int g0 = 0; g0 < ncp; g0 += 512) {
      PL<int> ssv[8];
      PL<float> rrv[8];
      LANES {
#pragma unroll
        for (int j = 0; j < 8; j++) {
          int t = g0 + 64 * j + lane;
          t = t < ncp ? t : ncp;
          ssv[j][lane] = pair_ss[t];
          rrv[j][lane] = pair_rr[t];
        }
      }
      PL<int> hit[8];
      LANES {
#pragma unroll
        for (int j = 0; j < 8; j++) {
          const int ss = ssv[j][lane], s1 = ss & 255, s2 = ss >> 8;
          const float rr = rrv[j][lane];
          const float dv[3] = {s.u.c.cen[s2][0] - s.u.c.cen[s1][0], s.u.c.cen[s2][1] - s.u.c.cen[s1][1], s.u.c.cen[s2][2] - s.u.c.cen[s1][2]};
          hit[j][lane] = rr >= 0.f && dot3(dv, dv) <= rr * rr;
        }
      }
#pragma unroll
      for (int j = 0; j < 8; j++) {
        const int base = g0 + 64 * j;
        if (base < ncp) {
          const uint64_t mask = wave_ballot(hit[j]);
          LANES {
            if (hit[j][lane]) {
              const int at = nsurv + popc64(mask & ((1ull << lane) - 1));
              if (at < 1024) s.u.c.list[at] = (unsigned short)(base + lane);
            }
          }
          nsurv += popc64(mask);
        }
      }
    }
    if (nsurv > 1024) { nsurv = 1024; flags |= SMJ_FLAG_CON_OVERFLOW; }
    SYNC();
    CTICK(SMJ_PROF_C_SPHERE)
    if (prof) pc[SMJ_PROF_C_NSPHERE] += (float)nsurv;
    for (int base = 0; base < nsurv; base += 64) {
      PL<int> hit;
      PL<int> tt;
      LANES {
        int h = 0, t = 0;
        if (base + lane < nsurv) {
          t = s.u.c.list[base + lane];
          const int ss = M.k_convpair_ss[t], s1 = ss & 255, s2 = ss >> 8;
          const float dv[3] = {s.u.c.cen[s2][0] - s.u.c.cen[s1][0], s.u.c.cen[s2][1] - s.u.c.cen[s1][1], s.u.c.cen[s2][2] - s.u.c.cen[s1][2]};
          float Ra[9], Rb[9], ha[3], hb[3], Rm[3][3], ta[3], tb[3];
#pragma unroll
          for (int k = 0; k < 9; k++) { Ra[k] = s.u.c.mat[s1][k]; Rb[k] = s.u.c.mat[s2][k]; }
#pragma unroll
          for (int k = 0; k < 3; k++) { ha[k] = s.u.c.half[s1][k]; hb[k] = s.u.c.half[s2][k]; }
#pragma unroll
          for (int i = 0; i < 3; i++) {
            ta[i] = Ra[i] * dv[0] + Ra[3 + i] * dv[1] + Ra[6 + i] * dv[2];
            tb[i] = Rb[i] * dv[0] + Rb[3 + i] * dv[1] + Rb[6 + i] * dv[2];
#pragma unroll
            for (int j = 0; j < 3; j++) Rm[i][j] = fabsf(Ra[i] * Rb[j] + Ra[3 + i] * Rb[3 + j] + Ra[6 + i] * Rb[6 + j]);
          }
          h = 1;
#pragma unroll
          for (int k = 0; k < 3; k++) {
            if (fabsf(ta[k]) > ha[k] + (Rm[k][0] * hb[0] + Rm[k][1] * hb[1] + Rm[k][2] * hb[2])) h = 0;
            if (fabsf(tb[k]) > hb[k] + (Rm[0][k] * ha[0] + Rm[1][k] * ha[1] + Rm[2][k] * ha[2])) h = 0;
          }
        }
        hit[lane] = h;
        tt[lane] = t;
      }
      uint64_t mask = wave_ballot(hit);
      PL<float> sdx, sdy, sdz;
      PL<int> stag;
      float* const sepbase = (S.sepcache && M.sep_cache) ? S.sepcache + (size_t)env * (SMJ_SEP_SLOTS * 4) : nullptr;
      LANES {
        Vec4 e = {0.f, 0.f, 0.f, 0.f};
        if (sepbase && hit[lane]) e = *reinterpret_cast<const Vec4*>(sepbase + 4 * (tt[lane] & (SMJ_SEP_SLOTS / 2 - 1)));
        sdx[lane] = e.x; sdy[lane] = e.y; sdz[lane] = e.z; stag[lane] = __builtin_bit_cast(int, e.w);
      }
      CTICK(SMJ_PROF_C_OBB)
      if (prof) pc[SMJ_PROF_C_NOBB] += (float)popc64(mask);
      while (mask) {
        const int l = ffs64(mask);
        mask &= mask - 1;
        const int t = wave_read(tt, l);
        const int* r = static_cast<const int*>(__builtin_assume_aligned(M.k_cprec + t * SMJ_CP_STRIDE, 16));
        const float sd[3] = {wave_read(sdx, l), wave_read(sdy, l), wave_read(sdz, l)};
        narrow_pair(r, uni(r[SMJ_CP_S1]), uni(r[SMJ_CP_S2]), sepbase ? sepbase + 4 * (t & (SMJ_SEP_SLOTS / 2 - 1)) : nullptr, t + 1,
                    sepbase && wave_read(stag, l) == t + 1, sd, pc, prof);
      }
      CTICK(SMJ_PROF_C_NARROW)
    }
    SYNC();
#undef CTICK
  }

  SMJ_DEV void make_constraint() {
    const int nv = M.nv, neq = M.neq, nfric = M.nfric, nlimit = M.nlimit;
    ROWPASS(rb, nefc) LANES {
      const int row = lane + rb;
      static_assert((64 * JS) % 4 == 0 && ((NEFC % 64) * JS) % 4 == 0, "row blocks are whole float4s");
      const int nrow = NEFC - rb < 64 ? NEFC - rb : 64, nf4 = nrow * JS / 4;
      Vec4* jz = reinterpret_cast<Vec4*>(&s.J[rb][0]);
      for (int k = lane; k < nf4; k += 64) jz[k] = Vec4{0.f, 0.f, 0.f, 0.f};
      if (row < NEFC) {
        s.etype[row] = CT_NONE; s.efloss[row] = 0; s.eid[row] = 0; s.epos[row] = 0; s.emargin[row] = 0; s.ediag[row] = 0;
      }
    }
    SYNC();
    int cap = newton() ? NEFC : M.pgs_cap > 0 ? M.pgs_cap : NEFC_P;
    if (M.row_limit > 0 && M.row_limit < cap) cap = M.row_limit;
    const int nstat = neq + nfric;
    PL<int> act, lrow[5];
    PL<float> lq;
    LANES {
      const int ol = opaque(lane);
      if (lane < nstat) {
        const int* r = static_cast<const int*>(__builtin_assume_aligned(M.k_rowrec + ol * SMJ_RR_STRIDE, 16));
        int v[SMJ_RR_SOLREF];
        for (int k = 0; k < SMJ_RR_SOLREF; k++) v[k] = r[k];
        const int e = lane, d1 = v[SMJ_RR_D1];
        if (v[SMJ_RR_TYPE] == CT_EQUALITY) {
          const int d2 = v[SMJ_RR_D2];
          float pos = s.qpos[v[SMJ_RR_Q1]] - asf(v[SMJ_RR_V1]), deriv = 0;
          const float a[5] = {asf(v[SMJ_RR_DATA]), asf(v[SMJ_RR_DATA + 1]), asf(v[SMJ_RR_DATA + 2]), asf(v[SMJ_RR_DATA + 3]), asf(v[SMJ_RR_DATA + 4])};
          if (d2 >= 0) {
            const float dif = s.qpos[v[SMJ_RR_Q2]] - asf(v[SMJ_RR_V2]);
            pos -= a[0] + dif * (a[1] + dif * (a[2] + dif * (a[3] + dif * a[4])));
            deriv = a[1] + dif * (2 * a[2] + dif * (3 * a[3] + dif * 4 * a[4]));
            s.J[e][d2] = -deriv;
          } else pos -= a[0];
          s.J[e][d1] = 1.f;
          s.etype[e] = CT_EQUALITY; s.eid[e] = v[SMJ_RR_ID]; s.epos[e] = pos; s.emargin[e] = 0; s.ediag[e] = asf(v[SMJ_RR_DIAG]);
        } else {
          s.J[e][d1] = 1.f;
          s.etype[e] = CT_FRICTION; s.eid[e] = v[SMJ_RR_ID]; s.efloss[e] = asf(v[SMJ_RR_FLOSS]); s.ediag[e] = asf(v[SMJ_RR_DIAG]);
        }
      }
      int a = 0;
      float q = 0;
      for (int k = 0; k < 5; k++) lrow[k][lane] = 0;
      if (lane < 2 * nlimit) {
        const int* r = static_cast<const int*>(__builtin_assume_aligned(M.k_rowrec + (nstat + ol) * SMJ_RR_STRIDE, 16));
        int v[SMJ_RR_DIAG + 1];
        for (int k = 0; k < SMJ_RR_DIAG + 1; k++) v[k] = r[k];
        const int side = v[SMJ_RR_D2];
        q = s.qpos[v[SMJ_RR_Q1]];
        const float dist = side * (asf(v[SMJ_RR_V1]) - q);
        a = dist < asf(v[SMJ_RR_V2]);
        lrow[0][lane] = v[SMJ_RR_D1]; lrow[1][lane] = side; lrow[2][lane] = v[SMJ_RR_V1]; lrow[3][lane] = v[SMJ_RR_V2]; lrow[4][lane] = v[SMJ_RR_DIAG];
      }
      act[lane] = a; lq[lane] = q;
    }
    const uint64_t lm = wave_ballot(act);
    int row0 = nstat;
    LANES {
      if (act[lane]) {
        const int r = row0 + popc64(lm & ((1ull << lane) - 1));
        if (r < cap) {
          const int side = lrow[1][lane];
          s.J[r][lrow[0][lane]] = (float)(-side);
          s.etype[r] = CT_LIMIT; s.eid[r] = lane;
          s.epos[r] = side * (asf(lrow[2][lane]) - lq[lane]);
          s.emargin[r] = asf(lrow[3][lane]); s.ediag[r] = asf(lrow[4][lane]);
        }
      }
    }
    row0 += popc64(lm);
    if (row0 > cap) { row0 = cap; flags |= SMJ_FLAG_EFC_OVERFLOW; }
    SYNC();
    PL<int> cact, cdimv, crow;
    PL<float> ctran, crot;
    LANES {
      int act = 0, dim = 0;
      float tran = 0, rot = 0;
      if (lane < ncon) {
        const int c = lane;
        dim = s.cdim[c];
        act = s.cdist[c] < s.cmargin[c];
        const int g1 = s.cgeom1[c], g2 = s.cgeom2[c], b1 = M.geom_bodyid[g1], b2 = M.geom_bodyid[g2];
        s.u.k.b1[c] = b1; s.u.k.b2[c] = b2;
        s.u.k.m1lo[c] = M.k_body_dofmask_lo[b1]; s.u.k.m1hi[c] = M.k_body_dofmask_hi[b1];
        s.u.k.m2lo[c] = M.k_body_dofmask_lo[b2]; s.u.k.m2hi[c] = M.k_body_dofmask_hi[b2];
        tran = M.geom_invweight0[2 * g1] + M.geom_invweight0[2 * g2];
        rot = M.geom_invweight0[2 * g1 + 1] + M.geom_invweight0[2 * g2 + 1];
      }
      cact[lane] = act; cdimv[lane] = dim; ctran[lane] = tran; crot[lane] = rot; crow[lane] = -1;
      if (lane < NVP)
        for (int x = 0; x < 6; x++) s.u.k.cd[lane][x] = lane < nv ? cdof[lane][x] : 0.f;
    }
    for (int c = 0; c < ncon; c++) {
      int d = wave_read(cdimv, c);
      if (!wave_read(cact, c)) continue;
      if (row0 + d > cap) {
        flags |= SMJ_FLAG_EFC_OVERFLOW;
        if (d > 3 && row0 + 3 <= cap) d = 3;
        else if (row0 + 1 <= cap) d = 1;
        else continue;
        LANES { if (lane == c) { cdimv[lane] = d; s.cdim[c] = d; } }
      }
      LANES { if (lane == c) crow[lane] = row0; }
      row0 += d;
    }
    LANES {
      if (lane < ncon) {
        const int c = lane, r0 = crow[lane], dim = cdimv[lane];
        s.cefc[c] = r0;
        if (r0 >= 0) {
#pragma unroll
          for (int r = 0; r < 6; r++)
            if (r < dim) {
              s.etype[r0 + r] = dim == 1 ? CT_CONTACT_FRICTIONLESS : CT_CONTACT_ELLIPTIC;
              s.eid[r0 + r] = c; s.epos[r0 + r] = s.cdist[c]; s.emargin[r0 + r] = s.cmargin[c];
              s.ediag[r0 + r] = r < 3 ? ctran[lane] : crot[lane];
            }
        }
      }
    }
    SYNC();
    constexpr int CPP = 64 / NVP;
    for (int c0 = 0; c0 < ncon; c0 += CPP) {
      LANES {
        const int c = c0 + lane / NVP, d = lane % NVP;
        if (c < ncon && d < nv) {
          const int r0 = s.cefc[c];
          if (r0 >= 0) {
            const int dim = s.cdim[c], b1 = s.u.k.b1[c], b2 = s.u.k.b2[c];
            const uint64_t m1 = mk64(s.u.k.m1lo[c], s.u.k.m1hi[c]), m2 = mk64(s.u.k.m2lo[c], s.u.k.m2hi[c]);
            const int in1 = (int)((m1 >> d) & 1), in2 = (int)((m2 >> d) & 1);
            const float sg = (float)(in2 - in1);
            if (sg != 0.f) {
              const int bb = in2 ? b2 : b1;
              const float off[3] = {s.cpos[c][0] - s.com[bb][0], s.cpos[c][1] - s.com[bb][1], s.cpos[c][2] - s.com[bb][2]};
              float cd[6], tv[3];
              for (int x = 0; x < 6; x++) cd[x] = s.u.k.cd[d][x];
              cross3(tv, cd, off);
              const float jp[3] = {cd[3] + tv[0], cd[4] + tv[1], cd[5] + tv[2]};
#pragma unroll
              for (int r = 0; r < 6; r++) {
                if (r < dim) {
                  const float* ax = s.cframe[c] + 3 * (r < 3 ? r : r - 3);
                  s.J[r0 + r][d] = sg * (r < 3 ? dot3(ax, jp) : dot3(ax, cd));
// ... 783 lines not shown
#ifdef SMJ_EMUL
      LANES {
        hrow[lane][J] -= mult[lane] * h0; hrow[lane][J + 1] -= mult[lane] * h1;
        hrow[lane][J + 2] -= mult[lane] * h2; hrow[lane][J + 3] -= mult[lane] * h3;
      }
#else
      LANES {
        typedef float f2 __attribute__((ext_vector_type(2)));
        const f2 m = {mult[lane], mult[lane]}, p = {h0, h1}, q = {h2, h3};
        f2 a = {hrow[lane][J], hrow[lane][J + 1]}, b = {hrow[lane][J + 2], hrow[lane][J + 3]};
        a = a - m * p; b = b - m * q;
        hrow[lane][J] = a.x; hrow[lane][J + 1] = a.y; hrow[lane][J + 2] = b.x; hrow[lane][J + 3] = b.y;
      }
#endif
      gj_pair<K, J + 4, N>(hrow, mult);
    } else if constexpr (J + 1 < N) {
      PL<float> c0, c1;
      LANES { c0[lane] = hrow[lane][J]; c1[lane] = hrow[lane][J + 1]; }
      const float h0 = wave_read(c0, K), h1 = wave_read(c1, K);
#ifdef SMJ_EMUL
      LANES { hrow[lane][J] -= mult[lane] * h0; hrow[lane][J + 1] -= mult[lane] * h1; }
#else
      LANES {
        typedef float f2 __attribute__((ext_vector_type(2)));
        const f2 m = {mult[lane], mult[lane]}, p = {h0, h1};
        f2 h = {hrow[lane][J], hrow[lane][J + 1]};
        h = h - m * p;
        hrow[lane][J] = h.x; hrow[lane][J + 1] = h.y;
      }
#endif
      gj_pair<K, J + 2, N>(hrow, mult);
    } else if constexpr (J < N) {
      PL<float> cj;
      LANES { cj[lane] = hrow[lane][J]; }
      const float hkj = wave_read(cj, K);
      LANES { hrow[lane][J] -= mult[lane] * hkj; }
    }
  }
  template <int K, int N>
  SMJ_DEV void gj_cols(PL<float[NVS]>& hrow, PL<float>& x, PL<float>& pinv, const PL<int>& ol) {
    if constexpr (K < N) {
      PL<float> col, mult;
      LANES { col[lane] = hrow[lane][K]; }
      const float rp = fast_rcp(fmaxf(wave_read(col, K), 1e-30f));
      LANES {
        mult[lane] = ol[lane] == K ? 0.f : col[lane] * rp;
        if (ol[lane] == K) pinv[lane] = rp;
      }
      gj_pair<K, K + 1, N>(hrow, mult);
      const float xk = wave_read(x, K);
      LANES { x[lane] -= mult[lane] * xk; }
      gj_cols<K + 1, N>(hrow, x, pinv, ol);
    }
  }
  template <int N>
  SMJ_DEV void gj_solve(PL<float>& x) {
    PL<float[NVS]> hrow;
    PL<float> pinv;
    PL<int> ol;
    LANES { ol[lane] = opaque(lane); }
    LANES {
      const int i = NVS == 32 ? (lane & 31) : (lane < NVS ? lane : NVS - 1);
#pragma unroll
      for (int k = 0; k < N; k++) hrow[lane][k] = s.u.n.H[i][k];
      pinv[lane] = 0.f;
      if (lane >= N) x[lane] = 0.f;
    }
    gj_cols<0, N>(hrow, x, pinv, ol);
    LANES { x[lane] *= pinv[lane]; }
  }
  SMJ_DEV void gj_solve_lds(PL<float>& x) {
    const int n = M.nv;
    LANES { if (lane < NVS) s.u.n.H[lane][NVS] = lane < n ? x[lane] : 0.f; }
    SYNC();
    for (int k = 0; k < n; k++) {
      const float rp = fast_rcp(fmaxf(uni(s.u.n.H[k][k]), 1e-30f));
      LANES {
        if (lane < n && lane != k) {
          float* row = s.u.n.H[lane];
          const float* piv = s.u.n.H[k];
          const float mult = row[k] * rp;
          int j = k + 1;
          for (; j + 8 <= n; j += 8) {
            float a[8], b[8];
#pragma unroll
            for (int u = 0; u < 8; u++) { a[u] = row[j + u]; b[u] = piv[j + u]; }
#pragma unroll
            for (int u = 0; u < 8; u++) row[j + u] = a[u] - mult * b[u];
          }
          for (; j < n; j++) row[j] -= mult * piv[j];
          row[NVS] -= mult * piv[NVS];
        }
      }
      SYNC();
    }
    LANES { x[lane] = lane < n ? s.u.n.H[lane][NVS] * fast_rcp(fmaxf(s.u.n.H[lane][lane], 1e-30f)) : 0.f; }
    SYNC();
  }
  SMJ_DEV void solve_H(PL<float>& x, bool rare = false) {
#if NVP == 32
    if (M.nv <= 26) gj_solve<26>(x);
    else gj_solve<NVP>(x);
#else
    if (rare || M.nv > 50) gj_solve_lds(x);
#if NVS >= 50
    else if (M.nv > 38) gj_solve<50>(x);
#endif
    else gj_solve<38>(x);
#endif
  }

  SMJ_DEV float ls_eval(NRow& nr0, const float* qg, float a, float& d1, float& d2) {
    const int ne = nefc;
    PL<float> p0, p1, p2;
    LANES { p0[lane] = 0.f; p1[lane] = 0.f; p2[lane] = 0.f; }
    ROWS_BEGIN(rb, ne) LANES {
      float c0 = 0, c1 = 0, c2 = 0;
      if (lane + rb < ne) {
        const int t = nr.type[lane];
        const float x = nr.jar[lane] + a * nr.jv[lane];
        if (t == CT_EQUALITY) { c0 = nr.q0[lane]; c1 = nr.q1[lane]; c2 = nr.q2[lane]; }
        else if (t == CT_FRICTION) {
          const float fl = nr.fl[lane], rf = nr.R[lane] * fl;
          if (x <= -rf) { c0 = fl * (-0.5f * rf - nr.jar[lane]); c1 = -fl * nr.jv[lane]; }
          else if (x >= rf) { c0 = fl * (-0.5f * rf + nr.jar[lane]); c1 = fl * nr.jv[lane]; }
          else { c0 = nr.q0[lane]; c1 = nr.q1[lane]; c2 = nr.q2[lane]; }
        } else if (t == CT_LIMIT || t == CT_CONTACT_FRICTIONLESS) {
          if (x < 0) { c0 = nr.q0[lane]; c1 = nr.q1[lane]; c2 = nr.q2[lane]; }
        } else if (nr.c0[lane] >= 0) {
          const float* k = nr.cq[lane];
          const float mu = k[6], Dm = k[5], N = k[0] + a * k[1], Tsq = k[2] + a * (2 * k[3] + a * k[4]);
          if (Tsq <= 0) { if (N < 0) { c0 = nr.q0[lane]; c1 = nr.q1[lane]; c2 = nr.q2[lane]; } }
          else {
            const float Ti = fast_rsqrt(Tsq), T = Tsq * Ti;
            if (N >= mu * T) {}
            else if (mu * N + T <= 0) { c0 = nr.q0[lane]; c1 = nr.q1[lane]; c2 = nr.q2[lane]; }
            else {
              const float w = k[3] + a * k[4], N1 = k[1], T1 = w * Ti, T2 = k[4] * Ti - w * w * Ti * Ti * Ti;
              const float NT = N - mu * T, NT1 = N1 - mu * T1;
              const float v = 0.5f * Dm * NT * NT, g = Dm * NT * NT1, h = Dm * (NT1 * NT1 - NT * mu * T2);
              c2 = 0.5f * h; c1 = g - h * a; c0 = v - a * g + 0.5f * h * a * a;
            }
          }
        }
      }
      p0[lane] += c0; p1[lane] += c1; p2[lane] += c2;
    } ROWS_END_RO()
    const float q0 = qg[0] + wave_sum(p0), q1 = qg[1] + wave_sum(p1), q2 = qg[2] + wave_sum(p2);
    d1 = 2 * a * q2 + q1;
    d2 = 2 * q2;
    return a * a * q2 + a * q1 + q0;
  }

  SMJ_DEV void solve_newton(bool dbg, float* pc, long long& t0, bool prof) {
#define TICK(slot) if (prof) { const long long t1 = smj_clock(); pc[slot] += (float)(t1 - t0); t0 = t1; }
    const int nv = M.nv, ne = nefc;
    NRow nr0;
    PL<float> qacc, Ma, Mv, grad, search, tmpv;
    if (ne == 0) {
      build_dense(false);
      LANES { qacc[lane] = lane < nv ? g_r[lane] : 0.f; }
      solve_H(qacc, true);
      LANES {
        qacc_r[lane] = lane < nv ? qacc[lane] : 0.f;
        if (lane < nv) { s.qacc[lane] = qacc[lane]; s.warm[lane] = qacc[lane]; s.tmp[lane] = g_r[lane]; }
#if NSAT > 0
        if (lane >= 32 && lane - 32 < M.nsat) {
          const int si = lane - 32;
          float A[21], x[6];
          for (int k = 0; k < 21; k++) A[k] = s.sat.Mb[si][k];
          for (int k = 0; k < 6; k++) { x[k] = s.sat.x[SX_G][si][k]; s.sat.x[SX_TMP][si][k] = x[k]; }
          sat_solve6(A, x);
          for (int k = 0; k < 6; k++) s.sat.x[SX_QA][si][k] = k < s.sat.ndof[si] ? x[k] : 0.f;
        }
#endif
      }
      niter = 0;
      SYNC();
      return;
    }
    ROWS_BEGIN_(rb, ne, false) LANES {
      const int row = lane + rb;
      float vel = 0;
      const bool on = row < ne;
      if (on) {
        const float* jr = jrow(row);
        for (int k = 0; k < nv; k++) vel += jr[k] * s.qvel[k];
#if NSAT > 0
        vel += sat_jdot(row, SX_V);
#endif
      }
      nr.type[lane] = on ? s.etype[row] : CT_NONE;
      nr.R[lane] = on ? s.eR[row] : 1.f;
      nr.D[lane] = on ? 1.0f / s.eR[row] : 0.f;
      nr.fl[lane] = on ? s.efloss[row] : 0.f;
      nr.aref[lane] = on ? -s.eBv[row] * vel - s.eK[row] * s.eimp[row] * (s.epos[row] - s.emargin[row]) : 0.f;
      int c0 = -1;
      if (on && s.etype[row] == CT_CONTACT_ELLIPTIC && s.cefc[s.eid[row]] == row) c0 = s.eid[row];
      nr.c0[lane] = c0;
      nr.state[lane] = 0; nr.jar[lane] = 0.f; nr.jv[lane] = 0.f; nr.force[lane] = 0.f; nr.q0[lane] = 0.f; nr.q1[lane] = 0.f; nr.q2[lane] = 0.f;
      for (int k = 0; k < 7; k++) nr.cq[lane][k] = 0.f;
      if (c0 >= 0) {
        const float mu = contact_mu(c0);
        nr.cq[lane][6] = mu;
        nr.cq[lane][5] = (1.0f / s.eR[row]) / fmaxf(mu * mu * (1 + mu * mu), SMJ_MINVAL);
      }
      if (dbg && row < NEFC) s.earef[row] = nr.aref[lane];
    } ROWS_END_RW(rb)
#if NSAT > 0
    const int nvt = M.nv_all;
#else
    const int nvt = nv;
#endif
    const float scale = 1.0f / (M.meaninertia * (float)(nvt > 1 ? nvt : 1));
    LANES { qacc[lane] = (lane < nv && M.warmstart) ? s.warm[lane] : 0.f; }
    mat_M(Ma, qacc);
#if NSAT > 0
    if (!M.warmstart) { LANES { if (lane >= 32 && lane - 32 < M.nsat) for (int k = 0; k < 6; k++) s.sat.x[SX_QA][lane - 32][k] = 0.f; } }
    sat_matM(SX_MA, SX_QA);
    SYNC();
#endif
    ROWS_BEGIN(rb, ne) mat_J_exact(nr.jar, qacc, nr.aref, rb); ROWS_END_RW(rb)
    float cost = 0;
    TICK(SMJ_PROF_WARM)
    int iter = 0;
    bool at_update = false;
    for (; iter < M.iterations;) {
      TICK(SMJ_PROF_PGS)
      cost = newton_update(nr0, true);
      float gauss;
      {
        PL<float> gs;
        LANES {
          gs[lane] = lane < nv ? qacc[lane] * (0.5f * Ma[lane] - g_r[lane]) : 0.f;
#if NSAT > 0
          if (lane >= 32 && lane - 32 < M.nsat)
            for (int k = 0; k < 6; k++) gs[lane] += s.sat.x[SX_QA][lane - 32][k] * (0.5f * s.sat.x[SX_MA][lane - 32][k] - s.sat.x[SX_G][lane - 32][k]);
#endif
        }
        gauss = wave_sum(gs);
      }
      cost += gauss;
      (void)cost;
      TICK(SMJ_PROF_N_UPDATE)
      matT_J(tmpv, nr0);
#if NSAT > 0
      sat_JTf();
#endif
      PL<float> g2;
      PL<int> gsig;
      LANES {
        grad[lane] = lane < nv ? Ma[lane] - g_r[lane] - tmpv[lane] : 0.f; g2[lane] = grad[lane] * grad[lane];
        gsig[lane] = fabsf(grad[lane]) > M.grad_noise * (fabsf(Ma[lane]) + fabsf(g_r[lane]) + fabsf(tmpv[lane]));
#if NSAT > 0
        if (lane >= 32 && lane - 32 < M.nsat) {
          const int si = lane - 32;
          for (int k = 0; k < 6; k++) {
            const float ma = s.sat.x[SX_MA][si][k], gg = s.sat.x[SX_G][si][k], jf = s.sat.x[SX_TMP][si][k], gr = k < s.sat.ndof[si] ? ma - gg - jf : 0.f;
            s.sat.x[SX_GRAD][si][k] = gr;
            g2[lane] += gr * gr;
            gsig[lane] |= fabsf(gr) > M.grad_noise * (fabsf(ma) + fabsf(gg) + fabsf(jf));
          }
        }
#endif
      }
      const float gnorm = sqrtf(wave_sum(g2));
      if (iter > 0 && (scale * gnorm < M.tolerance || wave_ballot(gsig) == 0)) { at_update = true; break; }
      TICK(SMJ_PROF_N_GRAD)
      ROWS_BEGIN(rb, ne) LANES {
        const int row = lane + rb;
        if (row < NEFC) s.ediag[row] = (row < ne && nr.state[lane] == 1) ? nr.D[lane] : 0.f;
      } ROWS_END_RO()
      uint64_t conemask;
      {
        PL<int> cz;
#if NSAT > 0
        SYNC();
#endif
        LANES {
          int z = 0;
          if (lane < ncon) {
            const int r0 = s.cefc[lane];
            z = r0 >= 0 && s.cdim[lane] >= 3 && s.estate[r0 >= 0 ? r0 : 0] == 4;
#if NSAT > 0
            if (z && s.sat.chs[lane] < 0) {
              for (int j = 0; j < s.cdim[lane]; j++) s.ediag[r0 + j] = 1.0f / s.eR[r0 + j];
              z = 0;
            }
#endif
          }
          cz[lane] = z;
        }
        conemask = wave_ballot(cz);
      }
      SYNC();
      TICK(SMJ_PROF_N_XA)
#if SMJ_W2_NEWTON
      fork2(W2_SAT_NEWTON, (int)(uint32_t)conemask, (int)(uint32_t)(conemask >> 32));
#endif
      {
        constexpr int NT = (NVS + 15) / 16, NTRI = NT * (NT + 1) / 2, KB = NVP == 32 ? 16 : 8;
        const int ksteps = (ndense() + 3) >> 2;
        PL<F4v> acc[NTRI];
        LANES {
#pragma unroll
          for (int t = 0; t < NTRI; t++)
            for (int r = 0; r < 4; r++) acc[t][lane].r[r] = 0.f;
        }
#pragma unroll
// ... 119 lines not shown
      PL<float> sq;
      LANES {
        search[lane] = lane < nv ? -search[lane] : 0.f; sq[lane] = search[lane] * search[lane];
#if NSAT > 0
        if (lane >= 32 && lane - 32 < M.nsat)
          for (int k = 0; k < 6; k++) sq[lane] += s.sat.x[SX_SRCH][lane - 32][k] * s.sat.x[SX_SRCH][lane - 32][k];
#endif
      }
      const float snorm = sqrtf(wave_sum(sq));
      TICK(SMJ_PROF_N_SOLVE)
      mat_M(Mv, search);
#if NSAT > 0
      sat_matM(SX_MV, SX_SRCH);
      SYNC();
      ROWS_BEGIN(rb, ne) {
        mat_J(nr.jv, search, rb);
        LANES { if (lane + rb < ne) nr.jv[lane] += sat_jdot(lane + rb, SX_SRCH); }
      } ROWS_END_RW(rb)
#else
      ROWS_BEGIN(rb, ne) mat_J(nr.jv, search, rb); ROWS_END_RW(rb)
#endif
      float qg[3];
      {
        PL<float> a1, a2;
        LANES {
          a1[lane] = lane < nv ? search[lane] * (Ma[lane] - g_r[lane]) : 0.f;
          a2[lane] = lane < nv ? 0.5f * search[lane] * Mv[lane] : 0.f;
#if NSAT > 0
          if (lane >= 32 && lane - 32 < M.nsat) {
            const int si = lane - 32;
            for (int k = 0; k < 6; k++) {
              a1[lane] += s.sat.x[SX_SRCH][si][k] * (s.sat.x[SX_MA][si][k] - s.sat.x[SX_G][si][k]);
              a2[lane] += 0.5f * s.sat.x[SX_SRCH][si][k] * s.sat.x[SX_MV][si][k];
            }
          }
#endif
        }
        qg[0] = gauss; qg[1] = wave_sum(a1); qg[2] = wave_sum(a2);
      }
      ROWS_BEGIN(rb, ne) LANES {
        const int row = lane + rb;
        const float D = nr.D[lane], ja = nr.jar[lane], jv = nr.jv[lane];
        nr.q0[lane] = 0.5f * D * ja * ja; nr.q1[lane] = D * ja * jv; nr.q2[lane] = 0.5f * D * jv * jv;
        if (row < NEFC) { s.eb[row] = ja; s.ef[row] = jv; s.earef[row] = nr.q0[lane]; s.eK[row] = nr.q1[lane]; s.eBv[row] = nr.q2[lane]; }
      } ROWS_END_RW(rb)
      SYNC();
      ROWS_BEGIN(rb, ne) LANES {
        const int c = nr.c0[lane];
        if (c >= 0) {
          const int i = lane + rb, dim = s.cdim[c];
          float a0 = 0, a1 = 0, a2 = 0, uu = 0, uv = 0, vv = 0;
#pragma unroll
          for (int j = 1; j < 6; j++) {
            const int jj = j < dim ? j : 1;
            const float on = j < dim ? 1.f : 0.f;
            a0 += on * s.earef[i + jj]; a1 += on * s.eK[i + jj]; a2 += on * s.eBv[i + jj];
            const float fr = on * s.cfric[c][jj - 1], u = s.eb[i + jj] * fr, v = s.ef[i + jj] * fr;
            uu += u * u; uv += u * v; vv += v * v;
          }
          nr.q0[lane] += a0; nr.q1[lane] += a1; nr.q2[lane] += a2;
          const float mu = nr.cq[lane][6];
          nr.cq[lane][0] = nr.jar[lane] * mu; nr.cq[lane][1] = nr.jv[lane] * mu;
          nr.cq[lane][2] = uu; nr.cq[lane][3] = uv; nr.cq[lane][4] = vv;
        }
      } ROWS_END_RW(rb)
      TICK(SMJ_PROF_N_PREP)
      float alpha = 0, d10 = 0;
      {
        const float gtol = M.tolerance * M.ls_tolerance * snorm * M.meaninertia * (float)(nvt > 1 ? nvt : 1);
        float d1, d2, lo = 0, hi = -1;
        {
          PL<float> gs;
          LANES {
            gs[lane] = lane < nv ? grad[lane] * search[lane] : 0.f;
#if NSAT > 0
            if (lane >= 32 && lane - 32 < M.nsat)
              for (int k = 0; k < 6; k++) gs[lane] += s.sat.x[SX_GRAD][lane - 32][k] * s.sat.x[SX_SRCH][lane - 32][k];
#endif
          }
          d1 = wave_sum(gs); d2 = -d1;
        }
        d10 = d1;
        float bestd = fabsf(d1), a = 0;
        if (d1 < 0 && d2 > 0) {
          a = -d1 / d2;
          for (int it = 0; it < M.ls_iterations; it++) {
            ls_eval(nr0, qg, a, d1, d2);
            if (prof) pc[SMJ_PROF_N_LSEVALS] += 1.f;
            if (fabsf(d1) < bestd) { bestd = fabsf(d1); alpha = a; }
            if (fabsf(d1) < gtol || fabsf(d1) < 1e-4f * fabsf(d10)) break;
            if (d1 < 0) lo = a; else hi = a;
            float an = (d2 > 0) ? a - d1 / d2 : -1.f;
            if (hi < 0) { if (an <= lo) an = 2 * a + 1e-12f; }
            else if (!(an > lo && an < hi)) an = 0.5f * (lo + hi);
            if (hi >= 0 && hi - lo < 1e-6f * fmaxf(1.f, hi)) break;
            if (fabsf(an - a) <= 1e-7f * fabsf(a)) break;
            a = an;
          }
        }
      }
      TICK(SMJ_PROF_N_LS)
      iter++;
      if (alpha == 0.f) break;
      LANES {
        qacc[lane] += alpha * search[lane]; Ma[lane] += alpha * Mv[lane];
#if NSAT > 0
        if (lane >= 32 && lane - 32 < M.nsat)
          for (int k = 0; k < 6; k++) { s.sat.x[SX_QA][lane - 32][k] += alpha * s.sat.x[SX_SRCH][lane - 32][k]; s.sat.x[SX_MA][lane - 32][k] += alpha * s.sat.x[SX_MV][lane - 32][k]; }
#endif
      }
#if NSAT > 0
      SYNC();
#endif
      if (NSAT > 0 || nroot() > 1) {
        PL<float> qn;
        LANES { qn[lane] = qacc[lane]; }
        ROWS_BEGIN(rb, ne) mat_J_exact(nr.jar, qn, nr.aref, rb); ROWS_END_RW(rb)
      } else {
        ROWS_BEGIN(rb, ne) LANES { nr.jar[lane] += alpha * nr.jv[lane]; } ROWS_END_RW(rb)
      }
      if (scale * (-0.5f * alpha * d10) < M.tolerance) break;
    }
    niter = iter;
    TICK(SMJ_PROF_PGS)
    if (!at_update) {
      newton_update(nr0, false);
      matT_J(tmpv, nr0);
#if NSAT > 0
      SYNC();
      sat_JTf();
#endif
    }
    LANES {
      qacc_r[lane] = lane < nv ? qacc[lane] : 0.f;
      if (lane < nv) { s.qacc[lane] = qacc[lane]; s.warm[lane] = qacc[lane]; s.tmp[lane] = g_r[lane] + tmpv[lane]; }
#if NSAT > 0
      if (lane >= 32 && lane - 32 < M.nsat)
        for (int k = 0; k < 6; k++) s.sat.x[SX_TMP][lane - 32][k] += s.sat.x[SX_G][lane - 32][k];
#endif
    }
    SYNC();
    if (dbg && debug_bound()) {
      LANES {
        if (lane < nv) S.debug[(SMJ_DBG_QACC + lane) * S.ld + env] = qacc[lane];
        const NRow& nr = nr0;
        S.debug[(SMJ_DBG_EFC_FORCE + lane) * S.ld + env] = lane < ne ? nr.force[lane] : 0.f;
        S.debug[(SMJ_DBG_EFC_R + lane) * S.ld + env] = lane < ne ? nr.R[lane] : 0.f;
        S.debug[(SMJ_DBG_EFC_AREF + lane) * S.ld + env] = lane < ne ? nr.aref[lane] : 0.f;
      }
    }
#undef TICK
  }

  SMJ_DEV void build_dense(bool implicit) {
    const float h = M.timestep;
    EntryTab et;
    load(et, implicit);
    LANES {
      for (int k = lane; k < NVS * (NVS + 1); k += 64) {
        const int r = k / (NVS + 1), c = k - r * (NVS + 1);
#if NSAT > 0
        s.u.n.H[r][c] = (r == c && r >= M.nv) ? 1.f : 0.f;
#else
        (&s.u.n.H[0][0])[k] = (r == c && r >= M.nv) ? 1.f : 0.f;
#endif
      }
    }
    SYNC();
    LANES {
      for (int t = 0; t < NENT; t++) {
        const int i = et.i[lane][t], j = et.j[lane][t];
        if (i < 0) continue;
        float v = (i == j) ? s.Mdiag[i] : s.MM[j][i];
        if (implicit) {
          float d = et.damp[lane][t] - et.dcoef[lane][t];
          const int la = et.lact[lane][t];
          if (la >= 0) d -= et.lcoef[lane][t] * s.act_free[la];
          v += h * d;
        }
        s.u.n.H[i][j] = v;
        s.u.n.H[j][i] = v;
      }
    }
    SYNC();
  }

  SMJ_DEV void integrate() {
    const int nv = M.nv;
    const float h = M.timestep;
#if SMJ_W2_INTEGRATE
    fork2(W2_SAT_INTEGRATE);
#endif
    build_dense(true);
    PL<float> x;
    LANES { x[lane] = lane < nv ? s.tmp[lane] : 0.f; }
    solve_H(x);
    LANES {
      if (lane < nv) s.qvel[lane] += h * x[lane];
    }
    SYNC();
    LANES {
      if (lane < M.njnt) {
        const int j = lane, qa = M.jnt_qposadr[j], da = M.jnt_dofadr[j];
        if (M.jnt_type[j] == JT_FREE) {
          for (int k = 0; k < 3; k++) s.qpos[qa + k] += h * s.qvel[da + k];
          float wv[3] = {s.qvel[da + 3], s.qvel[da + 4], s.qvel[da + 5]};
          const float nrm = sqrtf(dot3(wv, wv)), ang = nrm * h;
          float q[4] = {s.qpos[qa + 3], s.qpos[qa + 4], s.qpos[qa + 5], s.qpos[qa + 6]};
          if (ang > 0) {
            const float sn = sinf(0.5f * ang) / nrm, dq[4] = {cosf(0.5f * ang), wv[0] * sn, wv[1] * sn, wv[2] * sn};
            quat_mul(q, q, dq);
          }
          quat_normalize(q);
          for (int k = 0; k < 4; k++) s.qpos[qa + 3 + k] = q[k];
        } else s.qpos[qa] += h * s.qvel[da];
      }
    }
    SYNC();
    PL<int> bad;
    LANES {
      int b = 0;
      for (int k = lane; k < M.nq; k += 64) { const float q = s.qpos[k]; b |= !(fabsf(q) < 1e10f); }
      if (lane < nv) { const float v = s.qvel[lane]; b |= !(fabsf(v) < 1e10f); }
      bad[lane] = b;
    }
#if SMJ_W2_INTEGRATE
    WG_BARRIER();
    LANES { bad[lane] |= s.mbox[2]; }
#elif NSAT > 0
    sat_integrate(bad);
#endif
    if (wave_ballot(bad) != 0) {
      flags |= SMJ_FLAG_BAD_STATE;
      LANES {
        for (int k = lane; k < M.nq; k += 64) s.qpos[k] = M.qpos0[k];
        if (lane < nv) { s.qvel[lane] = 0.f; s.warm[lane] = 0.f; }
      }
#if NSAT > 0
      sat_reset_state();
#endif
      SYNC();
    }
  }

  SMJ_DEV void imu() {
    if (M.imu_site < 0 || (!S.gyro && !staged())) return;
    const int sid = M.imu_site, b = M.site_bodyid[sid];
    const uint64_t mk = mk64(M.k_body_dofmask_lo[b], M.k_body_dofmask_hi[b]);
    float cv[6], ca[6];
    for (int x = 0; x < 6; x++) {
      PL<float> tv, ta;
      LANES {
        const bool in = (mk >> lane) & 1;
        tv[lane] = in ? cdof[lane][x] * qvel_r[lane] : 0.f;
        ta[lane] = in ? cdof_dot[lane][x] * qvel_r[lane] + cdof[lane][x] * qacc_r[lane] : 0.f;
      }
      cv[x] = wave_sum(tv); ca[x] = wave_sum(ta);
    }
    for (int k = 0; k < 3; k++) ca[3 + k] -= M.gravity[k];
    float lp[3] = {M.site_pos[3 * sid], M.site_pos[3 * sid + 1], M.site_pos[3 * sid + 2]}, sp[3], lm[9], R[9];
    mulmat3vec(sp, s.xmat[b], lp);
    for (int k = 0; k < 9; k++) lm[k] = M.k_site_mat[9 * sid + k];
    mulmat3(R, s.xmat[b], lm);
    const float off[3] = {sp[0] + s.xpos[b][0] - s.com[b][0], sp[1] + s.xpos[b][1] - s.com[b][1], sp[2] + s.xpos[b][2] - s.com[b][2]};
    float t[3], vlin[3], alin[3], c2[3], gy[3], ac[3];
    cross3(t, cv, off);
    for (int k = 0; k < 3; k++) vlin[k] = cv[3 + k] + t[k];
    cross3(t, ca, off);
    for (int k = 0; k < 3; k++) alin[k] = ca[3 + k] + t[k];
    cross3(c2, cv, vlin);
    for (int k = 0; k < 3; k++) alin[k] += c2[k];
    mulmat3Tvec(gy, R, cv);
    mulmat3Tvec(ac, R, alin);
    if (staged()) {
      float* st = stage_row();
      LANES { if (lane < 3) { st[S.lay.gyro + lane] = gy[lane]; st[S.lay.accel + lane] = ac[lane]; } }
    } else {
      LANES { if (lane < 3) { S.gyro[lane * S.ld + env] = gy[lane]; S.accel[lane * S.ld + env] = ac[lane]; } }
    }
  }

  SMJ_DEV void dump_poses() {
    if (staged()) {
      float* st = stage_row() + S.lay.xpose;
      LANES {
        for (int k = lane; k < 12 * (M.nbody + M.nsat); k += 64) {
          const int b = k / 12, c = k - 12 * b;
          st[k] = c < 3 ? s.xpos[b][c] : s.xmat[b][c - 3];
        }
      }
      return;
    }
    if (!S.xpose) return;
    LANES {
      if (lane < M.nbody + M.nsat) {
        for (int k = 0; k < 3; k++) S.xpose[(long)(12 * lane + k) * S.ld + env] = s.xpos[lane][k];
        for (int k = 0; k < 9; k++) S.xpose[(long)(12 * lane + 3 + k) * S.ld + env] = s.xmat[lane][k];
      }
    }
  }
  SMJ_DEV void dump_debug() {
    if (!debug_bound()) return;
    LANES {
      for (int i = 0; i < NVP; i++)
        if (lane < NVP) {
          float v = 0;
          if (i < M.nv && lane < M.nv) v = (i == lane) ? s.Mdiag[i] : (i < lane ? s.MM[i][lane] : s.MM[lane][i]);
          S.debug[(SMJ_DBG_QM + i * NVP + lane) * S.ld + env] = v;
        }
      if (lane < NBP)
        for (int k = 0; k < 3; k++) S.debug[(SMJ_DBG_XPOS + 3 * lane + k) * S.ld + env] = lane < M.nbody ? s.xpos[lane][k] : 0.f;
    }
  }
  SMJ_DEV void contact_geom(int c, float* v) const {
    v[SMJ_CR_DIST] = s.cdist[c];
    for (int k = 0; k < 3; k++) v[SMJ_CR_POS + k] = s.cpos[c][k];
    for (int k = 0; k < 9; k++) v[SMJ_CR_FRAME + k] = s.cframe[c][k];
  }
  SMJ_DEV void dump_contacts() {
    if (!debug_bound()) return;
    LANES {
      if (lane < NCON) {
        const int c = lane;
        float v[SMJ_CR_FORCE] = {};
        float code = 0.f;
        if (c < ncon) {
          contact_geom(c, v);
          code = (float)(s.cdim[c] + 16 * s.cgeom1[c] + 16 * 1024 * s.cgeom2[c]);
        }
        for (int k = 0; k < 7; k++) S.debug[(SMJ_DBG_CON + 8 * c + k) * S.ld + env] = v[k];
        S.debug[(SMJ_DBG_CON + 8 * c + 7) * S.ld + env] = code;
      }
    }
  }
  SMJ_DEV void dump_contact_records() {
    if (!S.contacts) return;
    float* const out = S.contacts + (size_t)env * (size_t)S.con_cap * SMJ_CR_WORDS;
    LANES {
      const int c = lane;
      if (c < ncon) {
        float v[SMJ_CR_WORDS];
        contact_geom(c, v);
        const int r0 = s.cefc[c], dim = s.cdim[c];
        for (int k = 0; k < 6; k++) v[SMJ_CR_FORCE + k] = (r0 >= 0 && k < dim) ? s.ef[r0 + k] : 0.f;
        v[SMJ_CR_GEOM1] = __builtin_bit_cast(float, (int)s.cgeom1[c]);
        v[SMJ_CR_GEOM2] = __builtin_bit_cast(float, (int)s.cgeom2[c]);
        v[SMJ_CR_DIM] = __builtin_bit_cast(float, dim);
        v[SMJ_CR_EFC] = __builtin_bit_cast(float, r0);
        v[SMJ_CR_WORDS - 1] = 0.f;
        for (int k = 0; k < SMJ_CR_WORDS; k++) out[SMJ_CR_WORDS * c + k] = v[k];
      }
    }
  }

#if NSAT > 0
#include "smj_sat.h"
#endif

#if defined(SMJ_ONLY_NEWTON)
  SMJ_DEV bool newton() const { return true; }
#elif defined(SMJ_ONLY_PGS)
  SMJ_DEV bool newton() const { return false; }
#else
  SMJ_DEV bool newton() const { return M.solver == 2; }
#endif
#if defined(SMJ_LEAN)
  SMJ_DEV bool mcache_bound() const { return false; }
  SMJ_DEV bool manifold_cache() const { return false; }
  SMJ_DEV bool debug_bound() const { return false; }
  SMJ_DEV bool staged() const { return true; }
  SMJ_DEV int nroot() const { return 1; }
#else
  SMJ_DEV bool mcache_bound() const { return S.mcache != nullptr; }
  SMJ_DEV bool manifold_cache() const { return M.manifold_cache != 0; }
  SMJ_DEV bool debug_bound() const { return S.debug != nullptr; }
  SMJ_DEV bool staged() const { return S.stage != nullptr; }
  SMJ_DEV int nroot() const { return M.nroot; }
#endif
  SMJ_DEV void run(int nsteps, unsigned read_flags) {
    const int want_imu = read_flags & 1;
    flags = 0; nefc = NEFC; ncon = 0; niter = 0;
    float pc[SMJ_PROF_SLOTS];
    for (int k = 0; k < SMJ_PROF_SLOTS; k++) pc[k] = 0.f;
    const bool prof = SMJ_PROFILING && S.prof != nullptr;
    const long long tlaunch = S.cost ? smj_clock() : 0;
    long long t0 = prof ? smj_clock() : 0, tstart = t0;
#define TICK(slot) if (prof) { const long long t1 = smj_clock(); pc[slot] += (float)(t1 - t0); t0 = t1; }
    setup();
    load_state();
    TICK(SMJ_PROF_SETUP)
    for (int st = 0; st < nsteps; st++) {
      const bool last = st == nsteps - 1;
#if SMJ_W2_FORWARD
      fork2(W2_SAT_FORWARD, env);
      kinematics();
      WG_BARRIER();
#else
      kinematics();
#if NSAT > 0
      sat_forward();
#endif
#endif
      if (last && (read_flags & 4)) dump_poses();
      TICK(SMJ_PROF_KIN)
      com_crb();
      if (last) dump_debug();
      TICK(SMJ_PROF_COMCRB)
      smooth_forces(last);
      TICK(SMJ_PROF_SMOOTH)
      if (!newton()) factor();
      TICK(SMJ_PROF_FACTOR)

      collision();
      {
        const int ncon_planes = ncon;
        const unsigned flags_planes = flags;
#pragma nounroll
        for (int pass = 0; pass < 2; pass++) {
          collision_convex(pc, prof && pass == 0);
          if (pass || !((flags & ~flags_planes) & SMJ_FLAG_CON_OVERFLOW) || !(SMJ_SPLIT_COLLIDE || (mcache_bound() && manifold_cache()))) break;
          static_assert(SMJ_MC_SLOTS <= 64, "the redo clears the env's kept manifolds in ONE pass of the 64 lanes (SMJ_MC_LOG2 above 5 needs a loop here)");
          if (S.mcache) {
            LANES { if (lane < SMJ_MC_SLOTS) S.mcache[((size_t)env * SMJ_MC_SLOTS + lane) * SMJ_MC_WORDS] = 0.f; }
          }
          SYNC();
          ncon = ncon_planes;
          flags = flags_planes;
          serial_redo = true;
        }
        serial_redo = false;
      }
      if (last) dump_contacts();
      TICK(SMJ_PROF_COLLISION)
#if NSAT > 0
      make_constraint_sat(pc, prof);
#else
      if (!newton()) nefc = NEFC;
      make_constraint();
#endif
      TICK(SMJ_PROF_MAKECON)
      if (S.redo && !S.redo_worker && (flags & (SMJ_FLAG_EFC_OVERFLOW | SMJ_FLAG_CON_OVERFLOW))) {
        escalate(st);
        if (S.cost) { const int cst = (int)((smj_clock() - tlaunch) >> 6); LANES { if (lane == 0) st_coh(&S.cost[env], step_base ? ld_coh(&S.cost[env]) + cst : cst); } }
        return;
      }
#if NSAT > 0
      if (newton()) solve_newton(last, pc, t0, prof);
      else solve_pgs_sat(last, pc, t0, prof);
      if (last && debug_bound()) {
        LANES {
          if (lane >= 32 && lane - 32 < M.nsat)
            for (int k = 0; k < 6; k++) S.debug[(SMJ_DBG_SATQACC + 6 * (lane - 32) + k) * S.ld + env] = s.sat.x[SX_QA][lane - 32][k];
        }
      }
#else
      if (newton()) solve_newton(last, pc, t0, prof);
      else if (nefc > NEFP) solve<true>(last, pc, t0, prof);
      else solve<false>(last, pc, t0, prof);
#endif
      if (last && want_imu) imu();
      TICK(SMJ_PROF_POST)
      integrate();
      base_controller();
      TICK(SMJ_PROF_INTEGRATE)
      pc[SMJ_PROF_PGS_SWEEPS] += (float)niter;
    }
    if (read_flags & SMJ_READ_CR) dump_contact_records();
    store_state(nsteps);
    if (S.cost) {
      const int cst = (int)((smj_clock() - tlaunch) >> 6);
      LANES { if (lane == 0) st_coh(&S.cost[env], (S.redo_worker || step_base) ? ld_coh(&S.cost[env]) + cst : cst); }
    }
    if (prof) {
      pc[SMJ_PROF_TOTAL] = (float)(smj_clock() - tstart);
      LANES { if (lane < SMJ_PROF_SLOTS) S.prof[lane * S.ld + env] = pc[lane]; }
    }
#undef TICK
  }
};
```

### stretch_mujoco_amd/csrc/smj_wave.h

```cpp
#pragma once
#include <math.h>
#include <stdint.h>
#include <string.h>

#ifdef SMJ_EMUL
#define SMJ_DEV
#define LANES for (int lane = 0; lane < 64; ++lane)
#define SYNC() ((void)0)
template <class T>
struct PL {
  T v[64];
#ifdef SMJ_EMUL_POISON
  PL() { memset(v, SMJ_EMUL_POISON, sizeof v); }
#endif
  T& operator[](int l) { return v[l]; }
  const T& operator[](int l) const { return v[l]; }
};
static inline float wave_sum(const PL<float>& x) {
  float t[64];
  for (int i = 0; i < 64; i++) t[i] = x.v[i];
  for (int off = 32; off >= 1; off >>= 1) {
    float u[64];
    for (int i = 0; i < 64; i++) u[i] = t[i] + t[i ^ off];
    for (int i = 0; i < 64; i++) t[i] = u[i];
  }
  return t[0];
}
template <int G>
static inline void wave_group_sum(PL<float>& x) {
  for (int off = 1; off < G; off <<= 1) {
    float u[64];
    for (int i = 0; i < 64; i++) u[i] = x.v[i] + x.v[i ^ off];
    for (int i = 0; i < 64; i++) x.v[i] = u[i];
  }
}
static inline float wave_min(const PL<float>& x) {
  float m = x.v[0];
  for (int i = 1; i < 64; i++) m = fminf(m, x.v[i]);
  return m;
}
static inline float wave_max(const PL<float>& x) {
  float m = x.v[0];
  for (int i = 1; i < 64; i++) m = fmaxf(m, x.v[i]);
  return m;
}
static inline uint64_t wave_ballot(const PL<int>& p) {
  uint64_t b = 0;
  for (int i = 0; i < 64; i++)
    if (p.v[i]) b |= 1ull << i;
  return b;
}
template <class T>
static inline T wave_read(const PL<T>& x, int l) { return x.v[l]; }
static inline int popc64(uint64_t x) { return __builtin_popcountll(x); }
template <int N>
static inline float wave_bcast16(const PL<float>& x, int lane) { return x.v[(lane & ~15) + N]; }
static inline int ffs64(uint64_t x) { return __builtin_ffsll((long long)x) - 1; }
static inline long long smj_clock() { return 0; }
static inline int opaque(int x) { return x; }
static inline float ld_coh(const float* p) { return *p; }
static inline int ld_coh(const int* p) { return *p; }
static inline void st_coh(float* p, float v) { *p = v; }
static inline void st_coh(int* p, int v) { *p = v; }
static inline int uni(int x) { return x; }
static inline float uni(float x) { return x; }
static inline float fast_rcp(float x) { return 1.0f / x; }
static inline float fast_rsqrt(float x) { return 1.0f / sqrtf(x); }
static inline int lds_atomic_inc(int* p) { const int v = *p; *p = v + 1; return v; }
static inline int lds_atomic_add(int* p, int n) { const int v = *p; *p = v + n; return v; }
#else
#include <hip/hip_runtime.h>
#define SMJ_DEV __device__ __forceinline__
#ifdef SMJ_TWO_WAVES
#define LANES for (int lane = (int)(threadIdx.x & 63u), _k = 0; _k < 1; ++_k)
#define SYNC() do { __builtin_amdgcn_fence(__ATOMIC_ACQ_REL, "workgroup"); __builtin_amdgcn_wave_barrier(); } while (0)
#define WG_BARRIER() do { __builtin_amdgcn_fence(__ATOMIC_RELEASE, "workgroup"); __builtin_amdgcn_s_barrier(); __builtin_amdgcn_fence(__ATOMIC_ACQUIRE, "workgroup"); } while (0)
#else
#define LANES for (int lane = (int)threadIdx.x, _k = 0; _k < 1; ++_k)
#define SYNC() __syncthreads()
#endif
template <class T>
struct PL {
  T v;
  __device__ __forceinline__ T& operator[](int) { return v; }
  __device__ __forceinline__ const T& operator[](int) const { return v; }
};
template <int CTRL, int ROWMASK>
__device__ __forceinline__ float smj_dpp(float ident, float v) {
  return __builtin_bit_cast(float, __builtin_amdgcn_update_dpp(__builtin_bit_cast(int, ident), __builtin_bit_cast(int, v), CTRL,
                                                                ROWMASK, 0xF, false));
}
#define SMJ_WAVE_REDUCE(OP, IDENT)                \
  t = OP(t, smj_dpp<0xB1, 0xF>(IDENT, t));        \
  t = OP(t, smj_dpp<0x4E, 0xF>(IDENT, t));        \
  t = OP(t, smj_dpp<0x141, 0xF>(IDENT, t));       \
  t = OP(t, smj_dpp<0x140, 0xF>(IDENT, t));       \
  t = OP(t, smj_dpp<0x142, 0xA>(IDENT, t));       \
  t = OP(t, smj_dpp<0x143, 0xC>(IDENT, t));       \
  return __builtin_bit_cast(float, __builtin_amdgcn_readlane(__builtin_bit_cast(int, t), 63));
__device__ __forceinline__ float smj_addf(float a, float b) { return a + b; }
__device__ __forceinline__ float wave_sum(const PL<float>& x) {
  float t = x.v;
  SMJ_WAVE_REDUCE(smj_addf, 0.0f)
}
template <int G>
__device__ __forceinline__ void wave_group_sum(PL<float>& x) {
  x.v += smj_dpp<0xB1, 0xF>(0.0f, x.v);
  if (G > 2) x.v += smj_dpp<0x4E, 0xF>(0.0f, x.v);
}
__device__ __forceinline__ float wave_min(const PL<float>& x) {
  float t = x.v;
  SMJ_WAVE_REDUCE(fminf, __builtin_inff())
}
__device__ __forceinline__ float wave_max(const PL<float>& x) {
  float t = x.v;
  SMJ_WAVE_REDUCE(fmaxf, -__builtin_inff())
}
#undef SMJ_WAVE_REDUCE
template <int N>
__device__ __forceinline__ float wave_bcast16(const PL<float>& x, int) {
  return __builtin_bit_cast(float, __builtin_amdgcn_update_dpp(0, __builtin_bit_cast(int, x.v), 0x150 + N, 0xF, 0xF, false));
}
__device__ __forceinline__ uint64_t wave_ballot(const PL<int>& p) { return __ballot(p.v != 0); }
__device__ __forceinline__ float wave_read(const PL<float>& x, int l) {
  return __builtin_bit_cast(float, __builtin_amdgcn_readlane(__builtin_bit_cast(int, x.v), l));
}
__device__ __forceinline__ int wave_read(const PL<int>& x, int l) { return __builtin_amdgcn_readlane(x.v, l); }
__device__ __forceinline__ int popc64(uint64_t x) { return __popcll(x); }
__device__ __forceinline__ int ffs64(uint64_t x) { return __ffsll((long long)x) - 1; }
__device__ __forceinline__ long long smj_clock() { return (long long)__builtin_readcyclecounter(); }
__device__ __forceinline__ float ld_coh(const float* p) { return __hip_atomic_load(p, __ATOMIC_RELAXED, __HIP_MEMORY_SCOPE_AGENT); }
__device__ __forceinline__ int ld_coh(const int* p) { return __hip_atomic_load(p, __ATOMIC_RELAXED, __HIP_MEMORY_SCOPE_AGENT); }
__device__ __forceinline__ void st_coh(float* p, float v) { __hip_atomic_store(p, v, __ATOMIC_RELAXED, __HIP_MEMORY_SCOPE_AGENT); }
__device__ __forceinline__ void st_coh(int* p, int v) { __hip_atomic_store(p, v, __ATOMIC_RELAXED, __HIP_MEMORY_SCOPE_AGENT); }
__device__ __forceinline__ void coh_release() { __builtin_amdgcn_fence(__ATOMIC_RELEASE, "wavefront"); asm volatile("s_waitcnt vmcnt(0)" ::: "memory"); }
__device__ __forceinline__ void coh_acquire() { __builtin_amdgcn_fence(__ATOMIC_ACQUIRE, "wavefront"); }
__device__ __forceinline__ int opaque(int x) { asm volatile("" : "+v"(x)); return x; }
__device__ __forceinline__ int uni(int x) { return __builtin_amdgcn_readfirstlane(x); }
__device__ __forceinline__ float uni(float x) { return __builtin_bit_cast(float, __builtin_amdgcn_readfirstlane(__builtin_bit_cast(int, x))); }
__device__ __forceinline__ int lds_atomic_inc(int* p) { return atomicAdd(p, 1); }
__device__ __forceinline__ int lds_atomic_add(int* p, int n) { return atomicAdd(p, n); }
__device__ __forceinline__ float fast_rcp(float x) { return __builtin_amdgcn_rcpf(x); }
__device__ __forceinline__ float fast_rsqrt(float x) { return __builtin_amdgcn_rsqf(x); }
#endif

struct alignas(16) Vec4 { float x, y, z, w; };
struct F3 { float x, y, z; };
struct F4 { float w, x, y, z; };
struct F6 { float a[6]; };
struct M3 { float m[9]; };

SMJ_DEV float dot3(const float* a, const float* b) { return a[0] * b[0] + a[1] * b[1] + a[2] * b[2]; }
SMJ_DEV void cross3(float* r, const float* a, const float* b) {
  float x = a[1] * b[2] - a[2] * b[1], y = a[2] * b[0] - a[0] * b[2], z = a[0] * b[1] - a[1] * b[0];
  r[0] = x; r[1] = y; r[2] = z;
}
SMJ_DEV float normalize3(float* a) {
  float n = sqrtf(dot3(a, a));
  if (n < 1e-15f) { a[0] = 1; a[1] = 0; a[2] = 0; return 0; }
  float i = 1.0f / n;
  a[0] *= i; a[1] *= i; a[2] *= i;
  return n;
}
SMJ_DEV void quat_mul(float* r, const float* a, const float* b) {
  float w = a[0] * b[0] - a[1] * b[1] - a[2] * b[2] - a[3] * b[3], x = a[0] * b[1] + a[1] * b[0] + a[2] * b[3] - a[3] * b[2],
        y = a[0] * b[2] - a[1] * b[3] + a[2] * b[0] + a[3] * b[1], z = a[0] * b[3] + a[1] * b[2] - a[2] * b[1] + a[3] * b[0];
  r[0] = w; r[1] = x; r[2] = y; r[3] = z;
}
SMJ_DEV void quat_normalize(float* q) {
  float n = sqrtf(q[0] * q[0] + q[1] * q[1] + q[2] * q[2] + q[3] * q[3]);
  if (n < 1e-15f) { q[0] = 1; q[1] = q[2] = q[3] = 0; return; }
  float i = 1.0f / n;
  q[0] *= i; q[1] *= i; q[2] *= i; q[3] *= i;
}
SMJ_DEV void quat2mat(float* R, const float* q) {
  float w = q[0], x = q[1], y = q[2], z = q[3];
  R[0] = w * w + x * x - y * y - z * z; R[1] = 2 * (x * y - w * z); R[2] = 2 * (x * z + w * y);
  R[3] = 2 * (x * y + w * z); R[4] = w * w - x * x + y * y - z * z; R[5] = 2 * (y * z - w * x);
  R[6] = 2 * (x * z - w * y); R[7] = 2 * (y * z + w * x); R[8] = w * w - x * x - y * y + z * z;
}
SMJ_DEV void mulmat3vec(float* r, const float* R, const float* v) {
  float x = R[0] * v[0] + R[1] * v[1] + R[2] * v[2], y = R[3] * v[0] + R[4] * v[1] + R[5] * v[2],
        z = R[6] * v[0] + R[7] * v[1] + R[8] * v[2];
  r[0] = x; r[1] = y; r[2] = z;
}
SMJ_DEV void mulmat3Tvec(float* r, const float* R, const float* v) {
  float x = R[0] * v[0] + R[3] * v[1] + R[6] * v[2], y = R[1] * v[0] + R[4] * v[1] + R[7] * v[2],
        z = R[2] * v[0] + R[5] * v[1] + R[8] * v[2];
  r[0] = x; r[1] = y; r[2] = z;
}
SMJ_DEV void mulmat3(float* r, const float* A, const float* B) {
  float t[9];
#pragma unroll
  for (int i = 0; i < 3; i++)
#pragma unroll
    for (int j = 0; j < 3; j++) t[3 * i + j] = A[3 * i] * B[j] + A[3 * i + 1] * B[3 + j] + A[3 * i + 2] * B[6 + j];
#pragma unroll
  for (int i = 0; i < 9; i++) r[i] = t[i];
}
SMJ_DEV void mul_inert_vec(float* r, const float* i, const float* v) {
  r[0] = i[0] * v[0] + i[3] * v[1] + i[4] * v[2] - i[8] * v[4] + i[7] * v[5];
  r[1] = i[3] * v[0] + i[1] * v[1] + i[5] * v[2] + i[8] * v[3] - i[6] * v[5];
  r[2] = i[4] * v[0] + i[5] * v[1] + i[2] * v[2] - i[7] * v[3] + i[6] * v[4];
  r[3] = i[8] * v[1] - i[7] * v[2] + i[9] * v[3];
  r[4] = i[6] * v[2] - i[8] * v[0] + i[9] * v[4];
  r[5] = i[7] * v[0] - i[6] * v[1] + i[9] * v[5];
}
SMJ_DEV void cross_motion(float* r, const float* vel, const float* v) {
  float a[3], b[3], c[3];
  cross3(a, vel, v); cross3(b, vel, v + 3); cross3(c, vel + 3, v);
  r[0] = a[0]; r[1] = a[1]; r[2] = a[2]; r[3] = b[0] + c[0]; r[4] = b[1] + c[1]; r[5] = b[2] + c[2];
}
SMJ_DEV void cross_force(float* r, const float* vel, const float* f) {
  float a[3], b[3], c[3];
  cross3(a, vel, f); cross3(b, vel + 3, f + 3); cross3(c, vel, f + 3);
  r[0] = a[0] + b[0]; r[1] = a[1] + b[1]; r[2] = a[2] + b[2]; r[3] = c[0]; r[4] = c[1]; r[5] = c[2];
}
```

Measured before the change: 13.16 million.

## Prefetch model lane records ahead of use and hoist narrow-phase pair words

Splits each model-table load into an issue step and a use step so that body, dof, entry, collision-pair and joint records can be fetched earlier and overlap with preceding work (enabled only under SMJ_LEAN). Under the new SMJ_NARROW_AHEAD flag, which both build units now define, the narrow phase gathers per-pair shape and pair words with one wide per-lane load before the serial pair loop, and loads both shapes' vertices before their frames. SYNC in the single-wave path is changed from a workgroup __syncthreads to a wavefront fence plus wave barrier, which is cheaper but is only correct if the block is exactly one wave. The prefetches raise register pressure in exchange for hiding memory latency.

```diff
diff --git a/stretch_mujoco_amd/csrc/smj_kernels.hip b/stretch_mujoco_amd/csrc/smj_kernels.hip
--- a/stretch_mujoco_amd/csrc/smj_kernels.hip
+++ b/stretch_mujoco_amd/csrc/smj_kernels.hip
@@ -1,4 +1,5 @@
 #define SMJ_BUILD_TAG step
+#define SMJ_NARROW_AHEAD 1
 #include "smj_step_tu.h"
 
 __global__ __launch_bounds__(256) void smj_reset_kernel(const DevModel M, const DevState S, const uint8_t* mask) {
diff --git a/stretch_mujoco_amd/csrc/smj_kernels_mid.hip b/stretch_mujoco_amd/csrc/smj_kernels_mid.hip
--- a/stretch_mujoco_amd/csrc/smj_kernels_mid.hip
+++ b/stretch_mujoco_amd/csrc/smj_kernels_mid.hip
@@ -1,2 +1,3 @@
 #define SMJ_BUILD_TAG mid
+#define SMJ_NARROW_AHEAD 1
 #include "smj_step_tu.h"
diff --git a/stretch_mujoco_amd/csrc/smj_step_impl.h b/stretch_mujoco_amd/csrc/smj_step_impl.h
--- a/stretch_mujoco_amd/csrc/smj_step_impl.h
+++ b/stretch_mujoco_amd/csrc/smj_step_impl.h
@@ -325,11 +325,25 @@
     return static_cast<const int*>(__builtin_assume_aligned(M.k_lanerec + ol * SMJ_LR_STRIDE + off, 16));
   }
   SMJ_DEV static float asf(int b) { return __builtin_bit_cast(float, b); }
-  SMJ_DEV void load(KinTab& t) {
-    LANES {
-      const int* r = lanerec(opaque(lane), SMJ_LR_KIN);
-      int v[35];
-      for (int k = 0; k < 35; k++) v[k] = r[k];
+  template <int OFF, int N>
+  struct Rec { PL<int[N]> w; };
+  template <int OFF, int N>
+  SMJ_DEV void issue(Rec<OFF, N>& rec) {
+    LANES {
+      const int* r = lanerec(opaque(lane), OFF);
+      for (int k = 0; k < N; k++) rec.w[lane][k] = r[k];
+    }
+  }
+  typedef Rec<SMJ_LR_KIN, 35> KinRec;
+  typedef Rec<SMJ_LR_BODY, 23> BodyRec;
+  typedef Rec<SMJ_LR_DOF, 14> DofRec;
+  typedef Rec<SMJ_LR_ENT, 3 * NENT> EntRec;
+  typedef Rec<SMJ_LR_ENT, 7 * NENT> EntRecImpl;
+  typedef Rec<SMJ_LR_ACT, 28> ActRec;
+  SMJ_DEV void load(KinTab& t) { KinRec rec; issue(rec); use(t, rec); }
+  SMJ_DEV void use(KinTab& t, const KinRec& rec) {
+    LANES {
+      const int* v = rec.w[lane];
       t.parent[lane] = v[0]; t.level[lane] = v[1];
       for (int q = 0; q < 6; q++) t.jump[lane][q] = v[2 + q];
       for (int k = 0; k < 3; k++) t.pos[lane][k] = asf(v[8 + k]);
@@ -346,11 +360,10 @@
     PL<uint64_t> dofmask;
     PL<float[10]> inl;
   };
-  SMJ_DEV void load(BodyTab& t) {
-    LANES {
-      const int* r = lanerec(opaque(lane), SMJ_LR_BODY);
-      int v[23];
-      for (int k = 0; k < 23; k++) v[k] = r[k];
+  SMJ_DEV void load(BodyTab& t) { BodyRec rec; issue(rec); use(t, rec); }
+  SMJ_DEV void use(BodyTab& t, const BodyRec& rec) {
+    LANES {
+      const int* v = rec.w[lane];
       t.root[lane] = v[0]; t.subsize[lane] = v[1]; t.parent[lane] = v[2]; t.dofadr[lane] = v[3]; t.dofnum[lane] = v[4];
       for (int q = 0; q < 6; q++) t.jump[lane][q] = v[5 + q];
       t.dofmask[lane] = mk64(v[11], v[12]);
@@ -364,11 +377,10 @@
     PL<int[2]> act;
     PL<float[2]> actmom;
   };
-  SMJ_DEV void load(DofTab& t) {
-    LANES {
-      const int* r = lanerec(opaque(lane), SMJ_LR_DOF);
-      int v[14];
-      for (int k = 0; k < 14; k++) v[k] = r[k];
+  SMJ_DEV void load(DofTab& t) { DofRec rec; issue(rec); use(t, rec); }
+  SMJ_DEV void use(DofTab& t, const DofRec& rec) {
+    LANES {
+      const int* v = rec.w[lane];
       t.body[lane] = v[0]; t.jtype[lane] = v[1]; t.qadr[lane] = v[2]; t.first[lane] = v[3]; t.bsub[lane] = v[4];
       t.velmask[lane] = mk64(v[5], v[6]);
       t.damp[lane] = asf(v[7]); t.stiff[lane] = asf(v[8]); t.spring[lane] = asf(v[9]);
@@ -380,10 +392,15 @@
     PL<float[NENT]> arm, damp, dcoef, lcoef;
   };
   SMJ_DEV void load(EntryTab& t, bool implicit) {
-    LANES {
-      const int* r = lanerec(opaque(lane), SMJ_LR_ENT);
+    if (implicit) { EntRecImpl rec; issue(rec); use(t, rec); }
+    else { EntRec rec; issue(rec); use(t, rec); }
+  }
+  template <int N>
+  SMJ_DEV void use(EntryTab& t, const Rec<SMJ_LR_ENT, N>& rec) {
+    LANES {
+      const int* r = rec.w[lane];
       for (int u = 0; u < NENT; u++) { t.i[lane][u] = r[u]; t.j[lane][u] = r[NENT + u]; t.arm[lane][u] = asf(r[2 * NENT + u]); }
-      if (implicit)
+      if constexpr (N == 7 * NENT)
         for (int u = 0; u < NENT; u++) {
           t.lact[lane][u] = r[3 * NENT + u]; t.damp[lane][u] = asf(r[4 * NENT + u]); t.dcoef[lane][u] = asf(r[5 * NENT + u]);
           t.lcoef[lane][u] = asf(r[6 * NENT + u]);
@@ -398,15 +415,55 @@
     PL<int> gc_body, gc_mlo, gc_mhi;
     PL<float> gc_mass, gc_x, gc_y, gc_z;
   };
-  SMJ_DEV void load(ActTab& t) {
-    LANES {
-      const int* r = lanerec(opaque(lane), SMJ_LR_ACT);
-      int v[28];
-      for (int k = 0; k < 28; k++) v[k] = r[k];
+  SMJ_DEV void load(ActTab& t) { ActRec rec; issue(rec); use(t, rec); }
+  SMJ_DEV void use(ActTab& t, const ActRec& rec) {
+    LANES {
+      const int* v = rec.w[lane];
       for (int u = 0; u < 4; u++) { t.dof[lane][u] = v[u]; t.qadr[lane][u] = v[4 + u]; t.mom[lane][u] = asf(v[8 + u]); }
       for (int k = 0; k < 8; k++) t.prm[lane][k] = asf(v[12 + k]);
       t.flags[lane] = v[20]; t.gc_body[lane] = v[21]; t.gc_mlo[lane] = v[22]; t.gc_mhi[lane] = v[23];
       t.gc_mass[lane] = asf(v[24]); t.gc_x[lane] = asf(v[25]); t.gc_y[lane] = asf(v[26]); t.gc_z[lane] = asf(v[27]);
+    }
+  }
+#if defined(SMJ_LEAN) && !defined(SMJ_EMUL)
+  static constexpr bool kAhead = true;
+#else
+  static constexpr bool kAhead = false;
+#endif
+#if defined(SMJ_NARROW_AHEAD) || defined(SMJ_LEAN) || defined(SMJ_EMUL)
+  static constexpr bool kNarrowAhead = true;
+#else
+  static constexpr bool kNarrowAhead = false;
+#endif
+  struct Ahead {
+    BodyRec body; DofRec dof; EntRec ent;
+    PL<int[SMJ_PP_CONDIM]> pp;
+    PL<int> ss[8]; PL<float> rr[8];
+    EntRecImpl enti; PL<int> jqadr, jdadr, jtype;
+  };
+  SMJ_DEV void issue_collision(Ahead& ah) {
+    const int ncp = M.nconvpair;
+    LANES {
+      if (lane < M.nplanepair) {
+        const int* r = static_cast<const int*>(__builtin_assume_aligned(M.k_pprec + opaque(lane) * SMJ_PP_STRIDE, 16));
+        for (int k = 0; k < SMJ_PP_CONDIM; k++) ah.pp[lane][k] = r[k];
+      }
+#pragma unroll
+      for (int j = 0; j < 8; j++) {
+        int t = 64 * j + opaque(lane);
+        t = t < ncp ? t : ncp;
+        ah.ss[j][lane] = M.k_convpair_ss[t];
+        ah.rr[j][lane] = M.k_convpair_rsum[t];
+      }
+    }
+  }
+  SMJ_DEV void issue_integrate(Ahead& ah) {
+    issue(ah.enti);
+    LANES {
+      if (lane < M.njnt) {
+        const int j = opaque(lane);
+        ah.jqadr[lane] = M.jnt_qposadr[j]; ah.jdadr[lane] = M.jnt_dofadr[j]; ah.jtype[lane] = M.jnt_type[j];
+      }
     }
   }
 
@@ -544,10 +601,12 @@
     SYNC();
   }
 
-  SMJ_DEV void kinematics() {
+  SMJ_DEV void kinematics(const KinRec& kin, Ahead& ah) {
     const int nb = M.nbody;
     KinTab kt;
-    load(kt);
+    if (kAhead) use(kt, kin);
+    else load(kt);
+    if (kAhead) { issue(ah.body); issue(ah.dof); issue(ah.ent); }
     PL<float[3]> pl;
     PL<float[4]> ql;
     PL<float[6]> al, xl;
@@ -657,12 +716,13 @@
     SYNC();
   }
 
-  SMJ_DEV void com_crb() {
+  SMJ_DEV void com_crb(const Ahead& ah) {
     const int nb = M.nbody, nv = M.nv;
     BodyTab bt;
     DofTab dt;
     EntryTab et;
-    load(bt); load(dt); load(et, false);
+    if (kAhead) { use(bt, ah.body); use(dt, ah.dof); use(et, ah.ent); }
+    else { load(bt); load(dt); load(et, false); }
     PL<float> mx, my, mz;
     PL<float[3]> xip;
     LANES {
@@ -863,12 +923,13 @@
     }
   }
 
-  SMJ_DEV void smooth_forces(bool dbg) {
+  SMJ_DEV void smooth_forces(bool dbg, Ahead& ah) {
     const int nb = M.nbody, nv = M.nv, nu = M.nu;
     PL<float> frc_passive, frc_bias, frc_act;
     DofTab dt;
     ActTab at;
     load(dt); load(at);
+    if (kAhead) issue_collision(ah);
     LANES {
       float f = 0;
       if (lane < nv) {
@@ -1096,7 +1157,7 @@
     LANES { if (lane == 0) write_contact(c, r, dist, pos, n); }
   }
 
-  SMJ_DEV void collision() {
+  SMJ_DEV void collision(const Ahead& ah) {
     ncon = 0;
     for (int base = 0; base < M.nplanepair; base += 64) {
       PL<int> hull, cv;
@@ -1106,7 +1167,8 @@
         if (t < M.nplanepair) {
           const int* r = static_cast<const int*>(__builtin_assume_aligned(M.k_pprec + opaque(t) * SMJ_PP_STRIDE, 16));
           int v[SMJ_PP_CONDIM];
-          for (int k = 0; k < SMJ_PP_CONDIM; k++) v[k] = r[k];
+          if (kAhead && base == 0) { for (int k = 0; k < SMJ_PP_CONDIM; k++) v[k] = ah.pp[lane][k]; }
+          else { for (int k = 0; k < SMJ_PP_CONDIM; k++) v[k] = r[k]; }
           const int b1 = v[SMJ_PP_B1], b2 = v[SMJ_PP_B2];
           float lp1[3], lm1[9], pp[3], pm[9];
           for (int k = 0; k < 3; k++) lp1[k] = asf(v[SMJ_PP_POS1 + k]);
@@ -1793,13 +1855,12 @@
       if (sphere_sphere(v1, A.size[0], v2, Bs.size[0], margin, depth, dir, pos)) { add_contact(r, depth, pos, dir); n++; }
     }
   }
-  SMJ_DEV void load_shape(Shape& sh, int g, int slot, float* cen) {
-    (void)g;
+  SMJ_DEV void shape_meta(Shape& sh, int slot) {
     const unsigned meta = (unsigned)uni(s.u.c.meta[slot]);
     sh.type = (int)(meta & 15u); sh.nvert = (int)((meta >> 4) & 4095u);
     sh.verts = M.k_hull_vert4 + 4 * (int)(meta >> 16);
-    for (int k = 0; k < 3; k++) { sh.pos[k] = uni(s.u.c.pos[slot][k]); sh.size[k] = uni(s.u.c.size[slot][k]); cen[k] = uni(s.u.c.ccen[slot][k]); }
-    for (int k = 0; k < 9; k++) sh.mat[k] = uni(s.u.c.mat[slot][k]);
+  }
+  SMJ_DEV void shape_verts(Shape& sh) {
     if (sh.type == GT_MESH) {
       const Vec4* verts = reinterpret_cast<const Vec4*>(sh.verts);
       const int nvert = sh.nvert;
@@ -1811,6 +1872,20 @@
           sh.vc[lane][3 * u] = v.x; sh.vc[lane][3 * u + 1] = v.y; sh.vc[lane][3 * u + 2] = v.z;
         }
       }
+    }
+  }
+  SMJ_DEV void shape_frame(Shape& sh, int slot, float* cen) {
+    for (int k = 0; k < 3; k++) { sh.pos[k] = uni(s.u.c.pos[slot][k]); sh.size[k] = uni(s.u.c.size[slot][k]); cen[k] = uni(s.u.c.ccen[slot][k]); }
+    for (int k = 0; k < 9; k++) sh.mat[k] = uni(s.u.c.mat[slot][k]);
+  }
+  SMJ_DEV void load_shapes(Shape& A, Shape& Bs, int s1, int s2, float* c0, float* c1) {
+    if (kNarrowAhead) {
+      shape_meta(A, s1); shape_meta(Bs, s2);
+      shape_verts(A); shape_verts(Bs);
+      shape_frame(A, s1, c0); shape_frame(Bs, s2, c1);
+    } else {
+      shape_meta(A, s1); shape_frame(A, s1, c0); shape_verts(A);
+      shape_meta(Bs, s2); shape_frame(Bs, s2, c1); shape_verts(Bs);
     }
   }
 
@@ -2351,14 +2426,14 @@
     const unsigned slot = (((unsigned)tag >> 30) & 1u) << SMJ_MC_LOG2 | (((unsigned)tag * 2654435761u) >> (32 - SMJ_MC_LOG2));
     return S.mcache + ((size_t)env * SMJ_MC_SLOTS + slot) * SMJ_MC_WORDS;
   }
-  SMJ_DEV void narrow_pair(const int* r, int s1, int s2, float* sepslot, int septag, bool sep_hit, const float* sd, float* pc, bool prof, bool lookup = true) {
-    const int g1 = uni(r[SMJ_CP_G1]), g2 = uni(r[SMJ_CP_G2]);
+  struct PairWords { int b1, b2; float margin, rbmin; };
+  SMJ_DEV void narrow_pair(const int* r, int s1, int s2, float* sepslot, int septag, bool sep_hit, const float* sd, float* pc, bool prof, bool lookup = true, const PairWords* pw = nullptr) {
     const int ta0 = uni(s.u.c.meta[s1]) & 15, tb0 = uni(s.u.c.meta[s2]) & 15;
     float* mc = nullptr;
     const int ncon0 = ncon;
     if (mcache_bound() && manifold_cache() && ta0 != GT_SPHERE && tb0 != GT_SPHERE && !(ta0 == GT_CAPSULE && tb0 == GT_CAPSULE)) {
       mc = mc_entry(septag);
-      const int b1 = uni(r[SMJ_CP_B1]), b2 = uni(r[SMJ_CP_B2]);
+      const int b1 = pw ? pw->b1 : uni(r[SMJ_CP_B1]), b2 = pw ? pw->b2 : uni(r[SMJ_CP_B2]);
       PL<float> w;
       PL<int> moved;
       if (lookup) LANES {
@@ -2390,9 +2465,9 @@
         return;
       }
     }
-    narrow_pair_run(r, g1, g2, s1, s2, sepslot, septag, sep_hit, sd, pc, prof);
+    narrow_pair_run(r, pw, s1, s2, sepslot, septag, sep_hit, sd, pc, prof);
     if (mc && ncon > ncon0 && ncon - ncon0 <= 5 && !(flags & SMJ_FLAG_CON_OVERFLOW)) {
-      const int b1 = uni(r[SMJ_CP_B1]), b2 = uni(r[SMJ_CP_B2]), n = ncon - ncon0;
+      const int b1 = pw ? pw->b1 : uni(r[SMJ_CP_B1]), b2 = pw ? pw->b2 : uni(r[SMJ_CP_B2]), n = ncon - ncon0;
       SYNC();
       LANES {
         if (lane < SMJ_MC_WORDS) {
@@ -2407,12 +2482,11 @@
       }
     }
   }
-  SMJ_DEV void narrow_pair_run(const int* r, int g1, int g2, int s1, int s2, float* sepslot, int septag, bool sep_hit, const float* sd, float* pc, bool prof) {
+  SMJ_DEV void narrow_pair_run(const int* r, const PairWords* pw, int s1, int s2, float* sepslot, int septag, bool sep_hit, const float* sd, float* pc, bool prof) {
     Shape A, Bs;
     float c0[3], c1[3], depth, dir[3], pos[3];
-    load_shape(A, g1, s1, c0);
-    load_shape(Bs, g2, s2, c1);
-    const float margin = asf(uni(r[SMJ_CP_MARGIN]));
+    load_shapes(A, Bs, s1, s2, c0, c1);
+    const float margin = pw ? pw->margin : asf(uni(r[SMJ_CP_MARGIN]));
     if (A.type == GT_SPHERE && Bs.type == GT_SPHERE) {
       if (sphere_sphere(A.pos, A.size[0], Bs.pos, Bs.size[0], margin, depth, dir, pos)) add_contact(r, depth, pos, dir);
       return;
@@ -2478,15 +2552,15 @@
     if (prof && M.multiccd && A.type != GT_SPHERE && Bs.type != GT_SPHERE) pc[SMJ_PROF_C_NMULTI] += 1.f;
     if (M.multiccd && A.type != GT_SPHERE && Bs.type != GT_SPHERE) {
 #ifdef SMJ_EMUL
-      if (M.multi_serial) { convex_multi(r, A, Bs, s1, s2, pos, dir, margin, 1e-3f * asf(uni(r[SMJ_CP_RBMIN])), org); return; }
+      if (M.multi_serial) { convex_multi(r, A, Bs, s1, s2, pos, dir, margin, 1e-3f * (pw ? pw->rbmin : asf(uni(r[SMJ_CP_RBMIN]))), org); return; }
 #endif
       const long long t4 = prof ? smj_clock() : 0;
-      const int rounds = convex_multi4(r, A, Bs, s1, s2, pos, dir, margin, 1e-3f * asf(uni(r[SMJ_CP_RBMIN])), org);
+      const int rounds = convex_multi4(r, A, Bs, s1, s2, pos, dir, margin, 1e-3f * (pw ? pw->rbmin : asf(uni(r[SMJ_CP_RBMIN]))), org);
       if (prof) { pc[SMJ_PROF_C_TMULTI] += (float)(smj_clock() - t4); pc[SMJ_PROF_C_ROUNDS] += (float)rounds; }
     }
   }
 
-  SMJ_DEV void collision_convex(float* pc, bool prof) {
+  SMJ_DEV void collision_convex(float* pc, bool prof, const Ahead& ah) {
     if (!M.convex_pairs || (M.nconvpair == 0 && (NSAT == 0 || M.nsgeom == 0))) return;
     long long tc = prof ? smj_clock() : 0;
 #define CTICK(slot) if (prof) { const long long t1 = smj_clock(); pc[slot] += (float)(t1 - tc); tc = t1; }
@@ -2527,7 +2601,7 @@
     split_on = false;
     CTICK(SMJ_PROF_C_NARROW)
     if (serial_redo) {
-      collision_moving(pc, prof);
+      collision_moving(pc, prof, ah);
       SYNC();
       return;
     }
@@ -2581,7 +2655,8 @@
       if (cmd == W2_COLLIDE) {
         ncon = 0;
         flags = 0;
-        collision_moving(nullptr, false);
+        Ahead none;
+        collision_moving(nullptr, false, none);
         LANES { if (lane == 0) { s.mbox[2] = ncon; s.mbox[3] = flags; } }
       } else if (cmd == W2_SAT_NEWTON) {
         const uint64_t conemask = mk64(uni(s.mbox[1]), uni(s.mbox[2]));
@@ -2608,7 +2683,7 @@
     LANES { if (lane == 0) { s.mbox[0] = cmd; s.mbox[1] = w1; s.mbox[2] = w2; } }
     WG_BARRIER();
   }
-  SMJ_DEV void collision_moving(float* pc, bool prof) {
+  SMJ_DEV void collision_moving(float* pc, bool prof, const Ahead& ah) {
     long long tc = prof ? smj_clock() : 0;
 #define CTICK(slot) if (prof) { const long long t1 = smj_clock(); pc[slot] += (float)(t1 - tc); tc = t1; }
 #else
@@ -2624,7 +2699,12 @@
     for (int g0 = 0; g0 < ncp; g0 += 512) {
       PL<int> ssv[8];
       PL<float> rrv[8];
-      LANES {
+      if (kAhead && g0 == 0) {
+        LANES {
+#pragma unroll
+          for (int j = 0; j < 8; j++) { ssv[j][lane] = ah.ss[j][lane]; rrv[j][lane] = ah.rr[j][lane]; }
+        }
+      } else LANES {
 #pragma unroll
         for (int j = 0; j < 8; j++) {
           int t = g0 + 64 * j + lane;
@@ -2702,6 +2782,17 @@
         if (sepbase && hit[lane]) e = *reinterpret_cast<const Vec4*>(sepbase + 4 * (tt[lane] & (SMJ_SEP_SLOTS / 2 - 1)));
         sdx[lane] = e.x; sdy[lane] = e.y; sdz[lane] = e.z; stag[lane] = __builtin_bit_cast(int, e.w);
       }
+      PL<int> ws1, ws2, wb1, wb2, wmar, wrb;
+      if constexpr (kNarrowAhead) {
+        LANES {
+          int q[6] = {0, 0, 0, 0, 0, 0};
+          if (hit[lane]) {
+            const int* r = static_cast<const int*>(__builtin_assume_aligned(M.k_cprec + tt[lane] * SMJ_CP_STRIDE, 16));
+            q[0] = r[SMJ_CP_S1]; q[1] = r[SMJ_CP_S2]; q[2] = r[SMJ_CP_B1]; q[3] = r[SMJ_CP_B2]; q[4] = r[SMJ_CP_MARGIN]; q[5] = r[SMJ_CP_RBMIN];
+          }
+          ws1[lane] = q[0]; ws2[lane] = q[1]; wb1[lane] = q[2]; wb2[lane] = q[3]; wmar[lane] = q[4]; wrb[lane] = q[5];
+        }
+      }
       CTICK(SMJ_PROF_C_OBB)
       if (prof) pc[SMJ_PROF_C_NOBB] += (float)popc64(mask);
       while (mask) {
@@ -2710,8 +2801,13 @@
         const int t = wave_read(tt, l);
         const int* r = static_cast<const int*>(__builtin_assume_aligned(M.k_cprec + t * SMJ_CP_STRIDE, 16));
         const float sd[3] = {wave_read(sdx, l), wave_read(sdy, l), wave_read(sdz, l)};
-        narrow_pair(r, uni(r[SMJ_CP_S1]), uni(r[SMJ_CP_S2]), sepbase ? sepbase + 4 * (t & (SMJ_SEP_SLOTS / 2 - 1)) : nullptr, t + 1,
-                    sepbase && wave_read(stag, l) == t + 1, sd, pc, prof);
+        float* const sepslot = sepbase ? sepbase + 4 * (t & (SMJ_SEP_SLOTS / 2 - 1)) : nullptr;
+        if constexpr (kNarrowAhead) {
+          const PairWords w = {wave_read(wb1, l), wave_read(wb2, l), asf(wave_read(wmar, l)), asf(wave_read(wrb, l))};
+          narrow_pair(r, wave_read(ws1, l), wave_read(ws2, l), sepslot, t + 1, sepbase && wave_read(stag, l) == t + 1, sd, pc, prof, true, &w);
+        } else {
+          narrow_pair(r, uni(r[SMJ_CP_S1]), uni(r[SMJ_CP_S2]), sepslot, t + 1, sepbase && wave_read(stag, l) == t + 1, sd, pc, prof);
+        }
       }
       CTICK(SMJ_PROF_C_NARROW)
     }
@@ -3801,9 +3897,10 @@
     return a * a * q2 + a * q1 + q0;
   }
 
-  SMJ_DEV void solve_newton(bool dbg, float* pc, long long& t0, bool prof) {
+  SMJ_DEV void solve_newton(bool dbg, float* pc, long long& t0, bool prof, Ahead& ah) {
 #define TICK(slot) if (prof) { const long long t1 = smj_clock(); pc[slot] += (float)(t1 - t0); t0 = t1; }
     const int nv = M.nv, ne = nefc;
+    if (kAhead) issue_integrate(ah);
     NRow nr0;
     PL<float> qacc, Ma, Mv, grad, search, tmpv;
     if (ne == 0) {
@@ -4229,10 +4326,11 @@
 #undef TICK
   }
 
-  SMJ_DEV void build_dense(bool implicit) {
+  SMJ_DEV void build_dense(bool implicit, const EntRecImpl* ahead = nullptr) {
     const float h = M.timestep;
     EntryTab et;
-    load(et, implicit);
+    if (kAhead && ahead) use(et, *ahead);
+    else load(et, implicit);
     LANES {
       for (int k = lane; k < NVS * (NVS + 1); k += 64) {
         const int r = k / (NVS + 1), c = k - r * (NVS + 1);
@@ -4262,13 +4360,14 @@
     SYNC();
   }
 
-  SMJ_DEV void integrate() {
+  SMJ_DEV void integrate(const Ahead& ah, KinRec* next_kin) {
     const int nv = M.nv;
     const float h = M.timestep;
 #if SMJ_W2_INTEGRATE
     fork2(W2_SAT_INTEGRATE);
 #endif
-    build_dense(true);
+    if (kAhead && next_kin) issue(*next_kin);
+    build_dense(true, kAhead ? &ah.enti : nullptr);
     PL<float> x;
     LANES { x[lane] = lane < nv ? s.tmp[lane] : 0.f; }
     solve_H(x);
@@ -4278,8 +4377,8 @@
     SYNC();
     LANES {
       if (lane < M.njnt) {
-        const int j = lane, qa = M.jnt_qposadr[j], da = M.jnt_dofadr[j];
-        if (M.jnt_type[j] == JT_FREE) {
+        const int j = lane, qa = kAhead ? ah.jqadr[lane] : M.jnt_qposadr[j], da = kAhead ? ah.jdadr[lane] : M.jnt_dofadr[j];
+        if ((kAhead ? ah.jtype[lane] : M.jnt_type[j]) == JT_FREE) {
           for (int k = 0; k < 3; k++) s.qpos[qa + k] += h * s.qvel[da + k];
           float wv[3] = {s.qvel[da + 3], s.qvel[da + 4], s.qvel[da + 5]};
           const float nrm = sqrtf(dot3(wv, wv)), ang = nrm * h;
@@ -4466,35 +4565,38 @@
     setup();
     load_state();
     TICK(SMJ_PROF_SETUP)
+    KinRec kin;
+    if (kAhead) issue(kin);
     for (int st = 0; st < nsteps; st++) {
       const bool last = st == nsteps - 1;
+      Ahead ah;
 #if SMJ_W2_FORWARD
       fork2(W2_SAT_FORWARD, env);
-      kinematics();
+      kinematics(kin, ah);
       WG_BARRIER();
 #else
-      kinematics();
+      kinematics(kin, ah);
 #if NSAT > 0
       sat_forward();
 #endif
 #endif
       if (last && (read_flags & 4)) dump_poses();
       TICK(SMJ_PROF_KIN)
-      com_crb();
+      com_crb(ah);
       if (last) dump_debug();
       TICK(SMJ_PROF_COMCRB)
-      smooth_forces(last);
+      smooth_forces(last, ah);
       TICK(SMJ_PROF_SMOOTH)
       if (!newton()) factor();
       TICK(SMJ_PROF_FACTOR)
 
-      collision();
+      collision(ah);
       {
         const int ncon_planes = ncon;
         const unsigned flags_planes = flags;
 #pragma nounroll
         for (int pass = 0; pass < 2; pass++) {
-          collision_convex(pc, prof && pass == 0);
+          collision_convex(pc, prof && pass == 0, ah);
           if (pass || !((flags & ~flags_planes) & SMJ_FLAG_CON_OVERFLOW) || !(SMJ_SPLIT_COLLIDE || (mcache_bound() && manifold_cache()))) break;
           static_assert(SMJ_MC_SLOTS <= 64, "the redo clears the env's kept manifolds in ONE pass of the 64 lanes (SMJ_MC_LOG2 above 5 needs a loop here)");
           if (S.mcache) {
@@ -4522,7 +4624,7 @@
         return;
       }
 #if NSAT > 0
-      if (newton()) solve_newton(last, pc, t0, prof);
+      if (newton()) solve_newton(last, pc, t0, prof, ah);
       else solve_pgs_sat(last, pc, t0, prof);
       if (last && debug_bound()) {
         LANES {
@@ -4531,13 +4633,13 @@
         }
       }
 #else
-      if (newton()) solve_newton(last, pc, t0, prof);
+      if (newton()) solve_newton(last, pc, t0, prof, ah);
       else if (nefc > NEFP) solve<true>(last, pc, t0, prof);
       else solve<false>(last, pc, t0, prof);
 #endif
       if (last && want_imu) imu();
       TICK(SMJ_PROF_POST)
-      integrate();
+      integrate(ah, last ? nullptr : &kin);
       base_controller();
       TICK(SMJ_PROF_INTEGRATE)
       pc[SMJ_PROF_PGS_SWEEPS] += (float)niter;
diff --git a/stretch_mujoco_amd/csrc/smj_wave.h b/stretch_mujoco_amd/csrc/smj_wave.h
--- a/stretch_mujoco_amd/csrc/smj_wave.h
+++ b/stretch_mujoco_amd/csrc/smj_wave.h
@@ -77,7 +77,7 @@
 #define WG_BARRIER() do { __builtin_amdgcn_fence(__ATOMIC_RELEASE, "workgroup"); __builtin_amdgcn_s_barrier(); __builtin_amdgcn_fence(__ATOMIC_ACQUIRE, "workgroup"); } while (0)
 #else
 #define LANES for (int lane = (int)threadIdx.x, _k = 0; _k < 1; ++_k)
-#define SYNC() __syncthreads()
+#define SYNC() do { __builtin_amdgcn_fence(__ATOMIC_ACQ_REL, "wavefront"); __builtin_amdgcn_wave_barrier(); } while (0)
 #endif
 template <class T>
 struct PL {
```

Result: no change. 13.16 million, median of 2 (+0.1%).
